# WilliamVenner/squad-mortar-helper

Measured on AMD Instinct MI355X. Metric: map frames/sec (1920x1080 full CV pipeline), whole job, higher is better.
Workload: dtype u8/f32

## Files before the change

include/smh_vision_hip_debug.h:

```cpp
#ifndef SMH_VISION_HIP_DEBUG_H
#define SMH_VISION_HIP_DEBUG_H

#include "smh_vision_hip.h"

#ifdef __cplusplus
extern "C" {
#endif

SMHV_API int smhv_debug_lsd_classic(int on);
SMHV_API int smhv_debug_lsd_tile_cap(uint32_t cap);
SMHV_API int smhv_debug_lsd_threads(uint32_t threads);
SMHV_API int smhv_debug_pattern_copy(smhv_batch *b, const void *d_frames, uint32_t n, uint32_t rows_in_flight, void *stream);
SMHV_API int smhv_debug_heightmap_color_map_device(smhv_heightmap *hm, void *d_rgba, float *ms);
SMHV_API int smhv_debug_skip_line_search(int on);
SMHV_API int smhv_debug_lsd_spin_limit(uint32_t polls);
SMHV_API int smhv_debug_no_host_atomics(int on);
SMHV_API int smhv_debug_side_kernel(smhv_ctx *ctx, uint32_t workgroups, void *stream);

SMHV_API int smhv_debug_pipeline_stats(smhv_pipeline *p, uint64_t out[32]);
SMHV_API int smhv_debug_pipeline_peek(smhv_pipeline *p, uint64_t out[16]);

SMHV_API int smhv_debug_marker_table(smhv_ctx *ctx, uint32_t *bits);

SMHV_API int smhv_debug_crc32_host_level(const void *data, uint64_t nbytes, int level, uint32_t *crc);
SMHV_API int smhv_debug_band_rows(uint32_t frame_w, uint32_t frame_h, uint32_t n, int fused, uint32_t *rows, uint32_t *bands, int *tiles);
SMHV_API int smhv_debug_map_band_rows(uint32_t rows);
SMHV_API int smhv_debug_render_form(uint32_t form);
SMHV_API int smhv_debug_render_rule(uint32_t map_w, uint32_t map_h, float sw, float sh, uint32_t hm_w, uint32_t hm_h, float *ratio, float *switch_ratio,
                                    uint32_t *lds_texels, uint32_t *form);
SMHV_API int smhv_debug_feed_rows(uint32_t rows);
SMHV_API int smhv_debug_feed_gray_form(uint32_t form);
SMHV_API int smhv_debug_batch_mask_state(smhv_batch *b, uint32_t *stale_frames, int *eager);
SMHV_API int smhv_debug_batch_ui_state(smhv_batch *b, uint32_t *stale_frames, int *eager);
SMHV_API int smhv_debug_batch_materialize_ui(smhv_batch *b, void *stream);
SMHV_API int smhv_debug_mask_expand(smhv_batch *b, uint32_t n, void *stream);
SMHV_API int smhv_debug_ingest_feed(smhv_ingest *q, uint32_t n, uint32_t *counter);
SMHV_API int smhv_debug_ingest_feed_pixels(smhv_ingest *q, uint32_t n, uint32_t *counter, uint32_t pixels);

#ifdef __cplusplus
}
#endif

#endif
```

squad-mortar-helper_amd/_lib.py:

```python
import ctypes as C
import os

_HERE = os.path.dirname(os.path.abspath(__file__))
LIB_PATH = os.environ.get("SMH_VISION_HIP_LIB") or os.path.join(_HERE, "libsmh_vision_hip.so")

MAX_LINES = 32
MAX_SCALES = 3

STAGE_MARKERS, STAGE_UI_MAP, STAGE_OCR, STAGE_SCALES, STAGE_ALL = 0x1, 0x2, 0x4, 0x8, 0xF
STAGE_MINIMAP = 0x10
STAGE_EXACT_STATS = 0x20
STAGE_LSD_HELPERS = 0x40
STAGE_FIRING = 0x80
STAGE_HEIGHTMAP_OVERLAY = 0x100
FIRING_BOUNDS_OFFSET = 1
FIRING_NONE, FIRING_SCALES, FIRING_HEIGHTMAP = 0, 1, 2
VIEW_NONE, VIEW_OCR_INPUT, VIEW_FIND_SCALES_INPUT, VIEW_LSD_PREPROCESS, VIEW_LSD_INPUT, VIEW_CROPPED_BRQ = range(6)
IMAGE_UI_MAP = 100
IMAGE_HEIGHTMAP_OVERLAY = 101
RENDER_HEIGHTMAP, RENDER_MARKERS, RENDER_BOUNDS_OFFSET = 1, 2, 4
RENDER_MAX_LINES = 256
PRIM_LINE, PRIM_RECT, PRIM_FOREGROUND, PRIM_SHIFT1 = 0, 1, 0x100, 0x200
RENDER_MAX_PRIMS = 256
LAYER_MINIMAP_BOUNDS = 1
# ... 288 lines not shown
    "smhv_lsd_stats": (C.c_int, [C.c_void_p, C.c_uint32, C.c_int, C.POINTER(C.c_uint32), C.POINTER(C.c_uint64)]),
    "smhv_calc_meters_to_px_ratio": (C.c_int, [C.c_void_p, C.POINTER(C.c_uint32), C.c_uint32, C.POINTER(C.c_double), C.POINTER(C.c_int), C.POINTER(C.c_uint32)]),
    "smhv_find_minimap": (C.c_int, [C.c_void_p, C.POINTER(C.c_uint32), C.POINTER(C.c_int)]),
    "smhv_get_debug_view": (C.c_int, [C.c_void_p, C.c_int, C.c_void_p, C.POINTER(C.c_uint32), C.POINTER(C.c_uint32)]),
    "smhv_batch_create": (C.c_int, [C.c_void_p, C.c_uint32, C.c_uint32, C.c_uint32, C.POINTER(C.c_void_p)]),
    "smhv_batch_destroy": (None, [C.c_void_p]),
    "smhv_batch_layout_get": (C.c_int, [C.c_void_p, C.POINTER(BatchLayout)]),
    "smhv_batch_run": (C.c_int, [C.c_void_p, C.c_void_p, C.c_uint32, C.c_uint32, C.c_int, C.c_uint32, C.c_void_p, C.c_void_p]),
    "smhv_batch_device_ptrs": (C.c_int, [C.c_void_p] + [C.POINTER(C.c_void_p)] * 6),
    "smhv_batch_tile_mask": (C.c_int, [C.c_void_p, C.POINTER(C.c_void_p), C.POINTER(C.c_void_p), C.POINTER(C.c_uint32)]),
    "smhv_batch_read_tile_mask": (C.c_int, [C.c_void_p, C.c_uint32, C.c_void_p, C.c_void_p, C.c_void_p, C.POINTER(C.c_int)]),
    "smhv_batch_read_results": (C.c_int, [C.c_void_p, C.c_uint32, C.c_uint32, C.POINTER(FrameResult)]),
    "smhv_batch_read_image": (C.c_int, [C.c_void_p, C.c_int, C.c_uint32, C.c_void_p]),
    "smhv_batch_set_scales_stream": (C.c_int, [C.c_void_p, C.c_void_p]),
    "smhv_batch_wait_map_pass": (C.c_int, [C.c_void_p, C.c_void_p]),
    "smhv_batch_enable_timing": (C.c_int, [C.c_void_p, C.c_int]),
    "smhv_batch_lsd_coop_stats": (C.c_int, [C.c_void_p, C.c_uint32, C.c_uint32, C.POINTER(C.c_uint32)]),
    "smhv_batch_stage_ms": (C.c_int, [C.c_void_p, C.POINTER(C.c_float)]),
    "smhv_pipeline_create": (C.c_int, [C.c_void_p, C.c_uint32, C.c_uint32, C.c_uint32, C.c_uint32, C.POINTER(C.c_void_p)]),
    "smhv_pipeline_create_ex": (C.c_int, [C.c_void_p, C.c_uint32, C.c_uint32, C.c_uint32, C.c_uint32, C.c_void_p, C.POINTER(C.c_void_p)]),
    "smhv_pipeline_hold": (C.c_int, [C.c_void_p, C.c_uint32, C.c_void_p]),
    "smhv_debug_pipeline_stats": (C.c_int, [C.c_void_p, C.POINTER(C.c_uint64)]),
    "smhv_debug_pipeline_peek": (C.c_int, [C.c_void_p, C.POINTER(C.c_uint64)]),
    "smhv_pipeline_destroy": (None, [C.c_void_p]),
    "smhv_pipeline_submit": (C.c_int, [C.c_void_p, C.c_void_p, C.c_uint32, C.c_uint32, C.c_int, C.c_uint32, C.c_void_p, C.c_void_p, C.POINTER(C.c_uint32)]),
    "smhv_pipeline_wait": (C.c_int, [C.c_void_p, C.c_uint32]),
    "smhv_pipeline_wait_all": (C.c_int, [C.c_void_p]),
    "smhv_pipeline_slot": (C.c_int, [C.c_void_p, C.c_uint32, C.POINTER(C.c_void_p), C.POINTER(C.c_void_p)]),
    "smhv_shard_range": (None, [C.c_uint64, C.c_uint32, C.c_uint32, C.POINTER(C.c_uint64), C.POINTER(C.c_uint64)]),
    "smhv_node_create": (C.c_int, [C.POINTER(C.c_int), C.c_uint32, C.c_uint32, C.c_uint32, C.c_uint32, C.c_uint32, LOG_FN, C.POINTER(C.c_void_p)]),
    "smhv_node_destroy": (None, [C.c_void_p]),
    "smhv_node_ctx": (C.c_int, [C.c_void_p, C.c_uint32, C.POINTER(C.c_void_p), C.POINTER(C.c_void_p)]),
    "smhv_node_run": (C.c_int, [C.c_void_p, C.POINTER(C.c_void_p), C.POINTER(C.c_uint32), C.c_uint32, C.c_int, C.c_uint32, C.POINTER(C.c_void_p)]),
    "smhv_node_gather": (C.c_int, [C.c_void_p, C.POINTER(FrameResult), C.POINTER(C.c_uint32)]),
    "smhv_debug_lsd_classic": (C.c_int, [C.c_int]),
    "smhv_debug_lsd_tile_cap": (C.c_int, [C.c_uint32]),
    "smhv_debug_lsd_spin_limit": (C.c_int, [C.c_uint32]),
    "smhv_debug_lsd_threads": (C.c_int, [C.c_uint32]),
    "smhv_debug_skip_line_search": (C.c_int, [C.c_int]),
    "smhv_debug_no_host_atomics": (C.c_int, [C.c_int]),
    "smhv_debug_side_kernel": (C.c_int, [C.c_void_p, C.c_uint32, C.c_void_p]),
    "smhv_trait_times": (C.c_int, [C.c_void_p, C.POINTER(C.c_uint64), C.POINTER(C.c_uint64), C.c_int]),
    "smhv_ui_map": (C.c_int, [C.c_void_p, C.POINTER(C.c_void_p), C.POINTER(C.c_uint32), C.POINTER(C.c_uint32)]),
    "smhv_debug_pattern_copy": (C.c_int, [C.c_void_p, C.c_void_p, C.c_uint32, C.c_uint32, C.c_void_p]),
    "smhv_debug_batch_mask_state": (C.c_int, [C.c_void_p, C.POINTER(C.c_uint32), C.POINTER(C.c_int)]),
    "smhv_debug_batch_ui_state": (C.c_int, [C.c_void_p, C.POINTER(C.c_uint32), C.POINTER(C.c_int)]),
    "smhv_debug_batch_materialize_ui": (C.c_int, [C.c_void_p, C.c_void_p]),
    "smhv_debug_mask_expand": (C.c_int, [C.c_void_p, C.c_uint32, C.c_void_p]),
    "smhv_debug_marker_table": (C.c_int, [C.c_void_p, C.c_void_p]),
    "smhv_ingest_create": (C.c_int, [C.c_void_p, C.c_uint32, C.c_uint32, C.c_uint32, C.c_uint32, C.POINTER(C.c_void_p)]),
    "smhv_ingest_create_ex": (C.c_int, [C.c_void_p, C.c_uint32, C.c_uint32, C.c_uint32, C.c_uint32, C.c_uint32, C.POINTER(C.c_void_p)]),
    "smhv_crc32_host": (C.c_uint32, [C.c_void_p, C.c_uint64]),
    "smhv_debug_map_band_rows": (C.c_int, [C.c_uint32]),
    "smhv_debug_band_rows": (C.c_int, [C.c_uint32, C.c_uint32, C.c_uint32, C.c_int, C.POINTER(C.c_uint32), C.POINTER(C.c_uint32), C.POINTER(C.c_int)]),
    "smhv_debug_ingest_feed": (C.c_int, [C.c_void_p, C.c_uint32, C.POINTER(C.c_uint32)]),
    "smhv_debug_ingest_feed_pixels": (C.c_int, [C.c_void_p, C.c_uint32, C.POINTER(C.c_uint32), C.c_uint32]),
    "smhv_debug_crc32_host_level": (C.c_int, [C.c_void_p, C.c_uint64, C.c_int, C.POINTER(C.c_uint32)]),
    "smhv_ingest_destroy": (None, [C.c_void_p]),
    "smhv_ingest_local_cpus": (C.c_int, [C.c_void_p, C.c_char_p, C.c_size_t]),
    "smhv_ingest_bind_thread": (C.c_int, [C.c_void_p]),
    "smhv_ingest_acquire": (C.c_int, [C.c_void_p, C.POINTER(C.c_void_p)]),
    "smhv_ingest_commit": (C.c_int, [C.c_void_p]),
    "smhv_ingest_push": (C.c_int, [C.c_void_p, C.c_void_p]),
    "smhv_ingest_commit_pixels": (C.c_int, [C.c_void_p, C.c_uint32]),
    "smhv_ingest_push_pixels": (C.c_int, [C.c_void_p, C.c_void_p, C.c_uint32]),
    "smhv_ingest_staging_bytes": (C.c_uint64, [C.c_uint32, C.c_uint32, C.c_uint32]),
    "smhv_yuv_to_bgra_device": (C.c_int, [C.c_void_p, C.c_void_p, C.POINTER(YuvLayout), C.c_uint32, C.c_uint32, C.c_uint32, C.c_uint32, C.c_void_p, C.c_uint64,
                                          C.c_uint32, C.c_void_p]),
    "smhv_bgra_to_yuv_device": (C.c_int, [C.c_void_p, C.c_void_p, C.c_uint64, C.c_uint64, C.c_uint32, C.c_uint32, C.c_uint32, C.c_uint32, C.c_uint32, C.c_void_p,
                                          C.POINTER(YuvLayout), C.c_void_p]),
    "smhv_batch_video": (C.c_int, [C.c_void_p, C.c_uint32, C.c_uint32, C.c_uint32, C.c_uint32, C.c_void_p, C.POINTER(YuvLayout), C.c_void_p]),
    "smhv_video_bytes": (C.c_uint64, [C.c_uint32, C.c_uint32, C.c_uint32]),
    "smhv_ingest_batch": (C.c_int, [C.c_void_p, C.POINTER(C.c_void_p), C.POINTER(C.c_uint32), C.POINTER(C.c_uint32)]),
    "smhv_ingest_reset": (C.c_int, [C.c_void_p]),
    "smhv_ingest_counts": (C.c_int, [C.c_void_p, C.POINTER(C.c_uint64), C.POINTER(C.c_uint64)]),
    "smhv_crc32_device": (C.c_int, [C.c_void_p, C.c_void_p, C.c_uint64, C.POINTER(C.c_uint32)]),
    "smhv_heightmap_create": (C.c_int, [C.c_void_p, C.c_void_p, C.c_uint32, C.c_uint32, C.POINTER(C.c_int32), C.POINTER(C.c_float), C.POINTER(C.c_void_p)]),
    "smhv_heightmap_destroy": (None, [C.c_void_p]),
    "smhv_heightmap_color_map": (C.c_int, [C.c_void_p, C.c_void_p]),
    "smhv_debug_heightmap_color_map_device": (C.c_int, [C.c_void_p, C.c_void_p, C.POINTER(C.c_float)]),
    "smhv_batch_set_firing": (C.c_int, [C.c_void_p, C.c_void_p, C.POINTER(FiringOptions)]),
    "smhv_pipeline_set_firing": (C.c_int, [C.c_void_p, C.c_void_p, C.POINTER(FiringOptions)]),
    "smhv_batch_read_firing": (C.c_int, [C.c_void_p, C.c_uint32, C.c_uint32, C.POINTER(FiringResult)]),
    "smhv_batch_firing_ptr": (C.c_int, [C.c_void_p, C.POINTER(C.c_void_p)]),
    "smhv_firing_solutions": (C.c_int, [C.c_void_p, C.c_void_p, C.c_uint32, C.POINTER(C.c_double), C.POINTER(C.c_uint32), C.c_void_p,
                                        C.POINTER(FiringOptions), C.POINTER(Firing)]),
    "smhv_batch_overlay_ptr": (C.c_int, [C.c_void_p, C.POINTER(C.c_void_p)]),
    "smhv_heightmap_overlay": (C.c_int, [C.c_void_p, C.c_void_p, C.POINTER(FiringOptions), C.c_void_p]),
    "smhv_map_viewport_calc": (C.c_int, [C.c_float, C.c_float, C.c_float, C.c_float, C.c_uint32, C.POINTER(C.c_float), C.POINTER(C.c_float),
                                         C.POINTER(RenderOptions)]),
    "smhv_batch_render": (C.c_int, [C.c_void_p, C.c_uint32, C.c_uint32, C.c_void_p, C.POINTER(RenderOptions), C.c_void_p]),
    "smhv_batch_render_ptr": (C.c_int, [C.c_void_p, C.POINTER(C.c_void_p), C.POINTER(C.c_uint64)]),
    "smhv_batch_render_size": (C.c_int, [C.c_void_p, C.POINTER(C.c_uint32), C.POINTER(C.c_uint32)]),
    "smhv_batch_read_render": (C.c_int, [C.c_void_p, C.c_uint32, C.c_void_p]),
    "smhv_batch_render_layers": (C.c_int, [C.c_void_p, C.c_uint32, C.c_uint32, C.c_void_p, C.POINTER(RenderOptions), C.POINTER(RenderLayersStruct), C.c_void_p]),
    "smhv_render_map_layers": (C.c_int, [C.c_void_p, C.c_void_p, C.POINTER(RenderOptions), C.POINTER(RenderLayersStruct), C.c_void_p, C.c_uint32, C.c_void_p]),
    "smhv_render_map": (C.c_int, [C.c_void_p, C.c_void_p, C.POINTER(RenderOptions), C.c_void_p, C.c_uint32, C.c_void_p]),
    "smhv_label_font": (C.c_int, [C.c_uint8, C.POINTER(C.c_uint8)]),
    "smhv_batch_render_labels": (C.c_int, [C.c_void_p, C.c_uint32, C.c_uint32, C.c_void_p, C.POINTER(RenderOptions), C.POINTER(LabelOptionsStruct), C.c_void_p]),
    "smhv_batch_read_labels": (C.c_int, [C.c_void_p, C.c_uint32, C.c_uint32, C.POINTER(LabelResult)]),
    "smhv_batch_labels_ptr": (C.c_int, [C.c_void_p, C.POINTER(C.c_void_p)]),
    "smhv_render_map_labeled": (C.c_int, [C.c_void_p, C.c_void_p, C.POINTER(RenderOptions), C.POINTER(RenderLayersStruct), C.c_void_p, C.c_uint32,
                                          C.POINTER(LabelOptionsStruct), C.c_void_p, C.POINTER(LabelResult)]),
    "smhv_text_font": (C.c_int, [C.c_uint8, C.POINTER(C.c_uint8)]),
    "smhv_probe_text": (C.c_int, [C.POINTER(Probe), C.c_char_p, C.c_size_t]),
    "smhv_batch_probe": (C.c_int, [C.c_void_p, C.c_uint32, C.c_uint32, C.POINTER(RenderOptions), C.POINTER(ProbePoint), C.c_uint32, C.c_void_p]),
# ... 62 lines not shown
    "smhv_relief_map": (C.c_int, [C.c_void_p, C.c_void_p, C.POINTER(RenderOptions), C.POINTER(ReliefOptionsStruct), C.POINTER(C.c_uint32), C.c_void_p,
                                  C.c_void_p, C.c_void_p, C.c_void_p, C.POINTER(ReliefResult)]),
    "smhv_batch_scale_labels": (C.c_int, [C.c_void_p, C.c_void_p, C.c_uint32, C.c_void_p]),
    "smhv_batch_read_scale_labels": (C.c_int, [C.c_void_p, C.c_uint32, C.c_uint32, C.POINTER(ScaleLabelFrame), C.c_void_p]),
    "smhv_batch_scale_labels_ptr": (C.c_int, [C.c_void_p, C.POINTER(C.c_void_p), C.POINTER(C.c_void_p)]),
    "smhv_scale_labels": (C.c_int, [C.c_void_p, C.POINTER(ScaleLabelFrame), C.c_void_p]),
    "smhv_glyph_templates_check": (C.c_int, [C.POINTER(GlyphTemplate), C.c_uint32]),
    "smhv_glyph_templates_from_label": (C.c_int, [C.c_void_p, C.POINTER(ScaleLabel), C.c_char_p, C.POINTER(GlyphTemplate), C.POINTER(C.c_uint32)]),
    "smhv_glyph_atlas_create": (C.c_int, [C.c_void_p, C.POINTER(GlyphTemplate), C.c_uint32, C.POINTER(GlyphAtlasOptions), C.POINTER(C.c_void_p)]),
    "smhv_glyph_atlas_destroy": (None, [C.c_void_p]),
    "smhv_batch_label_text": (C.c_int, [C.c_void_p, C.c_void_p, C.c_uint32, C.c_void_p]),
    "smhv_batch_read_label_text": (C.c_int, [C.c_void_p, C.c_uint32, C.c_uint32, C.POINTER(LabelTextFrame)]),
    "smhv_batch_label_text_ptr": (C.c_int, [C.c_void_p, C.POINTER(C.c_void_p), C.POINTER(C.c_void_p)]),
    "smhv_label_text": (C.c_int, [C.c_void_p, C.c_void_p, C.POINTER(LabelTextFrame)]),
    "smhv_batch_run_label_anchors": (C.c_int, [C.c_void_p, C.c_void_p, C.c_uint32, C.c_uint32, C.c_int, C.c_uint32, C.c_void_p]),
    "smhv_scale_labels_anchors": (C.c_int, [C.POINTER(ScaleLabel), C.c_uint32, C.POINTER(C.c_uint32), C.POINTER(Anchors), C.POINTER(C.c_double),
                                            C.POINTER(C.c_int)]),
    "smhv_debug_render_form": (C.c_int, [C.c_uint32]),
    "smhv_debug_render_rule": (C.c_int, [C.c_uint32, C.c_uint32, C.c_float, C.c_float, C.c_uint32, C.c_uint32, C.POINTER(C.c_float), C.POINTER(C.c_float),
                                         C.POINTER(C.c_uint32), C.POINTER(C.c_uint32)]),
}


def firing_options(fit_to_minimap=True, viewport=None):
    o = FiringOptions()
    o.size = C.sizeof(FiringOptions)
    o.flags = 0 if fit_to_minimap else FIRING_BOUNDS_OFFSET
    if viewport is not None:
        sw, sh, tx, ty = viewport
        o.viewport_scale[0], o.viewport_scale[1] = sw, sh
        o.viewport_top_left[0], o.viewport_top_left[1] = tx, ty
    return o


FIRING_DTYPE = None


def firing_dtype():
    import numpy as np
    global FIRING_DTYPE
    if FIRING_DTYPE is None:
        FIRING_DTYPE = np.dtype([("meters", "<f8"), ("alt_delta", "<f8"), ("mils", "<f8", (2,)), ("bearing", "<f4", (2,)),
                                 ("source", "<u4"), ("reserved", "<u4")], align=True)
        assert FIRING_DTYPE.itemsize == C.sizeof(Firing)
    return FIRING_DTYPE


class PipelineOptions(C.Structure):
    _fields_ = [("size", C.c_uint32), ("search", C.c_uint32), ("streams", C.c_uint32), ("idle_close_us", C.c_uint32), ("occupancy_policy", C.c_uint32),
                ("late_helpers", C.c_uint32), ("service_workgroups", C.c_uint32), ("flags", C.c_uint32), ("remote_after", C.c_uint32), ("remote_tickets", C.c_uint32), ("remote_last", C.c_uint32), ("room_for_others", C.c_uint32)]


SEARCH_AUTO, SEARCH_BATCH, SEARCH_FRAME = 0, 1, 2
PIPE_NO_TEAM_HELP, PIPE_NO_STREAM_PRIORITY, PIPE_NO_PROLOGUE, PIPE_NO_REMOTE_HELP, PIPE_HELP_FIRST, PIPE_WALK_BIT_ROWS, PIPE_THREE_LOAD_SETS = 1, 2, 4, 8, 16, 32, 64


class VisionError(RuntimeError):

    def __init__(self, code, msg):
        super().__init__("smh_vision_hip error %d: %s" % (code, msg))
        self.code = code
        self.records = None


_lib = None


def load():
    global _lib
    if _lib is None:
        if not os.path.exists(LIB_PATH):
            raise ImportError(
                "%s not found: the HIP extension is not built (run __graft_entry__.build() or "
                "`make -C squad-mortar-helper_amd/csrc`). There is no CPU fallback." % LIB_PATH)
        try:
            import torch
        except ImportError:
            pass
        lib = C.CDLL(LIB_PATH)
        for name, (res, args) in SIGNATURES.items():
            fn = getattr(lib, name)
            fn.restype = res
            fn.argtypes = args
        _lib = lib
    return _lib


def _hm(heightmap):
    return heightmap._hm if heightmap is not None else None


def check(rc):
    if rc != 0:
        raise VisionError(rc, load().smhv_last_error().decode("utf-8", "replace"))
```

squad-mortar-helper_amd/batch.py:

```python
import ctypes as C
from collections.abc import Mapping

import numpy as np

from . import _lib as L

STAGE_NAMES = ("button", "map_pass", "brq_pass", "lsd", "scale_ratio")


def make_anchors(per_frame):
    arr = (L.Anchors * len(per_frame))()
    for i, (start_y, scales) in enumerate(per_frame):
        arr[i].n = min(len(scales), L.MAX_SCALES)
        arr[i].scales_start_y = start_y
        for j, (m, x, y) in enumerate(scales[:L.MAX_SCALES]):
            arr[i].scales[j][0], arr[i].scales[j][1], arr[i].scales[j][2] = m, x, y
    return arr


def results_to_dicts(recs):
    out = []
    for r in recs:
        n = r.n_lines
        out.append(dict(
# ... 428 lines not shown
        for i in range(depth):
            b = C.c_void_p()
            L.check(self._lib.smhv_pipeline_slot(self._p, i, C.byref(b), None))
            self.slots.append(FrameBatch(vision, frame_w, frame_h, max_frames, _handle=b))

    def stream_of(self, slot):
        st = C.c_void_p()
        L.check(self._lib.smhv_pipeline_slot(self._p, slot, None, C.byref(st)))
        return st.value or 0

    def hold(self, slot, stream):
        L.check(self._lib.smhv_pipeline_hold(self._p, slot, C.c_void_p(stream)))

    def submit(self, frames_ptr, n, stages=L.STAGE_ALL, grayscale=True, max_gap=15, anchors=None, after_stream=0):
        if anchors is not None and len(anchors) < n:
            raise ValueError("anchors holds %d entries, the submission covers %d frames" % (len(anchors), n))
        a = C.cast(anchors, C.c_void_p) if anchors is not None else None
        slot = C.c_uint32(0)
        L.check(self._lib.smhv_pipeline_submit(self._p, C.c_void_p(frames_ptr), n, stages, int(bool(grayscale)), max_gap, a, C.c_void_p(after_stream), C.byref(slot)))
        return int(slot.value)

    def set_firing(self, heightmap=None, fit_to_minimap=True, viewport=None):
        opt = L.firing_options(fit_to_minimap, viewport)
        L.check(self._lib.smhv_pipeline_set_firing(self._p, L._hm(heightmap), C.byref(opt)))

    def search_stats(self):
        out = (C.c_uint64 * 32)()
        L.check(self._lib.smhv_debug_pipeline_stats(self._p, out))
        if not out[0]:
            return None
        keys = ("launches", "frames", "waves", "busy_cycles", "resident_cycles", "waves_per_launch", "submissions")
        d = dict(zip(keys, [int(v) for v in out[1:8]]))
        d["cycles_per_frame_by_phase"] = dict(zip(("acquire", "search", "record", "release"), [int(v) / max(d["frames"], 1) for v in out[8:12]]))
        d["help_cycles_per_frame"] = int(out[12]) / max(d["frames"], 1)
        d["remote_help"] = {"requests": int(out[16]), "helpers_attached": int(out[17]), "candidates_cast": int(out[18]), "tickets_left": int(out[19]) - (1 << 64) if int(out[19]) >= (1 << 63) else int(out[19])}
        d["cycles_per_frame"] = d["busy_cycles"] / max(d["frames"], 1)
        d["busy_fraction"] = d["busy_cycles"] / max(d["resident_cycles"], 1)
        d["remote_help"].update({"polls": int(out[23]), "polls_empty": int(out[24]), "claims_lost": int(out[25]), "exits_idle": int(out[26]), "exits_closed": int(out[27]),
                                 "cycles_attached_per_helper": int(out[28]) / max(int(out[17]), 1), "cast_fraction_of_attached": int(out[29]) / max(int(out[28]), 1)})
        d["timeline_ms"] = {"frame_wait": int(out[20]) / max(d["frames"], 1) / 1e5, "submission_search": int(out[21]) / max(d["submissions"], 1) / 1e5,
                            "last_frame_at_work": int(out[22]) / max(d["submissions"], 1) / 1e5}
        d["adaptive"] = bool(int(out[13]) & 2)
        d["settled"] = bool(int(out[13]) & 4) or not d["adaptive"]
        d["mode"] = "frame-granular" if int(out[13]) & 1 else "batch-granular"
        d["measured_frames_per_s"] = {"frame-granular": int(out[14]), "batch-granular": int(out[15])}
        return d

    def peek(self):
        out = (C.c_uint64 * 16)()
        L.check(self._lib.smhv_debug_pipeline_peek(self._p, out))
        keys = ("submissions", "alive_epoch", "launches", "last_seq", "avail", "head", "reserved", "closing_epoch", "completed", "busy")
        d = dict(zip(keys, [int(v) for v in out[:10]]))
        d["avail"] = d["avail"] - (1 << 64) if d["avail"] >= (1 << 63) else d["avail"]
        d["slots"] = [(int(v) >> 32, int(v) & 0xFFFFFFFF) for v in out[10:14]]
        d["service_workgroups"], d["waves_per_workgroup"] = int(out[14]) >> 32, int(out[14]) & 0xFFFFFFFF
        d["lds_words_per_wave"], d["lds_bytes_dynamic"] = int(out[15]) >> 32, int(out[15]) & 0xFFFFFFFF
        return d

    def wait(self, slot=None):
        if slot is None:
            L.check(self._lib.smhv_pipeline_wait_all(self._p))
        else:
            L.check(self._lib.smhv_pipeline_wait(self._p, slot))

    def close(self):
        if self._p:
            for b in self.slots:
                b.close()
            self._lib.smhv_pipeline_destroy(self._p)
            self._p = None

    def __del__(self):
        try:
            self.close()
        except Exception:
            pass
```

squad-mortar-helper_amd/csrc/smh_kernels.h:

```cpp
#pragma once
#include <hip/hip_runtime.h>
#include <stdint.h>

#include "../../include/smh_vision_hip.h"
#include "../../include/smh_vision_hip_debug.h"

namespace smh {

struct Geom {
	uint32_t W, H;
	uint32_t rx, ry, rw, rh;
	uint32_t bx, by, bw, bh;
	uint32_t qx, qy, qw, qh;
	uint32_t m_ax, m_xoff, m_quads, m_block;
	uint32_t q_ax, q_xoff, q_quads, q_block;
	uint64_t frame_bytes;
	uint64_t ui_pitch, ui_stride;
	uint64_t mask_pitch, mask_stride;
	uint32_t bits_pitch_w; uint64_t bits_stride_w;
	uint64_t ocr_pitch, ocr_stride;
};

struct FrameAux {
	uint32_t open;
// ... 332 lines not shown
	uint32_t closing;
	int32_t help_avail;
	uint32_t help_head, help_reserve;
	uint32_t stat_remote;
	uint32_t head;
	uint32_t reserve;
	uint32_t completed;
	uint32_t busy;
	uint32_t stat_items, stat_waves;
	unsigned long long stat_busy, stat_life;
	unsigned long long stat_phase[4];
	unsigned long long stat_help;
	uint32_t stat_requests, stat_attached;
	unsigned long long stat_t_wait, stat_t_sub, stat_t_last;
	uint32_t stat_h_polls, stat_h_empty, stat_h_lost, stat_h_idle_exit, stat_h_closed_exit, stat_h_pad;
	unsigned long long stat_h_cycles, stat_h_cast_cycles;
	unsigned long long help_ring[SVC_HELP_RING];
};
struct SvcHost {
	unsigned long long state;
	uint32_t launches;
	uint32_t pad0;
	uint32_t done_seq[SVC_MAX_SLOTS];
	uint32_t pad[12];
};
struct SvcParams {
	SvcCtl *ctl;
	unsigned long long *ring;
	SvcSlot *slots;
	SvcHost *host;
	const uint32_t *cull_tab;
	const float *ray_off;
	float max_gap;
	uint32_t tile_cap, list_cap;
	uint32_t part_words;
	uint32_t ring_log2;
	uint32_t epoch;
	uint32_t idle_short, idle_long;
	uint32_t flags;
	SvcRemote *remote;
	uint32_t *remote_store;
	uint32_t remote_store_words;
	uint32_t remote_after;
	uint32_t remote_tickets;
	uint32_t remote_last_div;
	uint32_t compact;
};
uint32_t svc_waves_for(const Geom &g, uint32_t tile_limit, uint32_t *part_words, uint32_t *tile_cap, uint32_t *list_cap, uint32_t *lds_bytes, uint32_t *compact = nullptr);
uint32_t svc_store_words_for(const Geom &g, uint32_t tile_cap, uint32_t compact);
hipError_t svc_probe_host_atomics(SvcHost *h, SvcHost *d_h, bool *ok);
hipError_t launch_svc_publish(SvcCtl *ctl, unsigned long long *ring, SvcSlot *slots, uint32_t slot, const Buffers &b, uint32_t n, uint32_t seq, uint32_t ring_log2, hipStream_t s);
hipError_t launch_lsd_service(const Geom &g, const SvcParams &p, uint32_t workgroups, uint32_t waves, uint32_t lds_bytes, hipStream_t s);

enum : uint32_t { MAP_UI = 1u, MAP_MASK = 2u, MAP_BYTES = 4u, MAP_PRIO = 0x100u, MAP_BAND_MAJOR = 0x200u };
enum : uint32_t { BRQ_OCR = 1u, BRQ_SCALES = 2u };

enum : uint32_t { UI_FORM_RGBA = 0u, UI_FORM_LUMA = 1u, UI_FORM_KEEP = 2u };
hipError_t launch_button(const Geom &g, const Buffers &b, uint32_t n, int force_open, hipStream_t s, uint8_t *ui_form = nullptr, uint32_t ui_luma = UI_FORM_KEEP);
hipError_t launch_ui_expand(const Geom &g, const uint8_t *d_luma, uint8_t *d_ui, uint8_t *ui_form, uint32_t n, hipStream_t s);
hipError_t launch_map_pass(const Geom &g, const Buffers &b, uint32_t n, uint32_t flags, int grayscale, hipStream_t s, bool tiles_wanted = false, bool overlapped = false);
struct LaunchTuning {
	uint32_t map_lds_total;
	uint32_t map_grid_cap;
	uint32_t lsd_tile_limit;
	uint32_t map_prio;
	uint32_t map_deep;
	uint32_t map_overlapped;
};
uint32_t map_brq_lds_bytes(const Geom &g);
uint32_t lsd_tile_lds_bytes(const Geom &g, uint32_t tile_limit);
hipError_t launch_map_brq_pass(const Geom &g, const Buffers &b, uint32_t n, uint32_t flags, uint32_t qflags, int grayscale, uint32_t fixed_start_y, int use_anchor_start, hipStream_t s,
                               const LaunchTuning *tune = nullptr);
hipError_t launch_pattern_copy(const Geom &g, const Buffers &b, uint32_t n, uint32_t rows_in_flight, hipStream_t s);
void map_band_rows(uint32_t rh, uint32_t n, int fused, uint32_t *rows, int *tiles);
hipError_t launch_brq_pass(const Geom &g, const Buffers &b, uint32_t n, uint32_t flags, uint32_t fixed_start_y, int use_anchor_start, hipStream_t s);
struct LsdFork { hipStream_t s1, s2; hipEvent_t fork, join1, join2; };
bool lsd_rows_only(const Geom &g);
hipError_t launch_lsd(const Geom &g, const Buffers &b, uint32_t n, float max_gap, int mode, float px, float py, hipStream_t s, const LsdFork *fk, uint32_t tile_bs = 0,
                      bool prefer_classic = false, uint32_t tile_limit = 0, bool *record_fused = nullptr);
size_t lsd_coop_ctl_bytes(uint32_t n);
hipError_t launch_scale_ratio(const Geom &g, const Buffers &b, uint32_t n, uint32_t *d_bars, hipStream_t s);
hipError_t launch_find_minimap(const Geom &g, const Buffers &b, uint32_t n, hipStream_t s);
hipError_t launch_finalize(const Geom &g, const Buffers &b, uint32_t n, uint32_t stages, hipStream_t s);
hipError_t launch_scales_finalize(const Geom &g, const Buffers &b, uint32_t n, uint32_t stages, uint32_t *d_bars, hipStream_t s);
hipError_t launch_firing_lines(const FiringRun &r, const smhv_line *lines, uint32_t n, uint32_t has_mpx, double mpx, uint32_t has_minimap,
                               const uint32_t minimap[4], smhv_firing *out, hipStream_t s);
hipError_t launch_heightmap_color_map(const uint16_t *hm, uint64_t n, uint32_t *mm, uint32_t *rgba, hipStream_t s);
#define SMH_HM_LUT_ENTRIES 65536u
hipError_t launch_heightmap_lut(const uint16_t *hm, uint64_t n, uint32_t *mm, uint32_t *lut, hipStream_t s);
hipError_t launch_hm_overlay(const Geom &g, const OverlayRun &r, uint32_t n, hipStream_t s);
hipError_t launch_render_map(const Geom &g, const RenderRun &r, uint32_t n, hipStream_t s);
hipError_t launch_render_map_layers(const Geom &g, const RenderRun &r, const RenderLayersRun &y, uint32_t n, hipStream_t s);
hipError_t launch_heightmap_lut16(const uint32_t *lut, uint16_t *lut16, uint32_t *vr, hipStream_t s);
#define SMH_HM_LUT_WORDS (SMH_HM_LUT_ENTRIES + 4u + SMH_HM_LUT_ENTRIES / 2u)
hipError_t launch_labels(const LabelRun &r, uint32_t n, hipStream_t s);
hipError_t launch_reach(const ReachRun &r, uint32_t n, bool paint, bool classes, hipStream_t s);
hipError_t launch_relief(const ReliefRun &r, uint32_t n, bool paint, hipStream_t s);
hipError_t launch_clear_lines(const ClearLinesRun &r, uint32_t n, hipStream_t s);
hipError_t launch_clear_map(const ClearMapRun &r, uint32_t n, bool paint, bool bytes, hipStream_t s);
hipError_t launch_scale_labels(const ScaleLabelsRun &r, uint32_t n, hipStream_t s);
uint32_t scale_labels_gap(uint32_t qw);
hipError_t launch_label_text(const LabelTextRun &r, uint32_t n, hipStream_t s);
hipError_t launch_debug_text(const Geom &g, const DebugRun &r, uint32_t n, hipStream_t s);
void render_set_form(uint32_t form);
uint32_t render_rule(const Geom &g, const RenderRun &r, uint32_t *texels, float *ratio);
float render_switch_ratio();
hipError_t launch_debug_view(const Geom &g, const Buffers &b, uint32_t frame, int which, int isolated, uint8_t *d_rgba, hipStream_t s);
hipError_t launch_marker_table(uint32_t *d_bits, hipStream_t s);
hipError_t launch_mask_expand(const Geom &g, const uint32_t *d_bits, uint8_t *d_mask, uint32_t n, hipStream_t s);
hipError_t launch_pack_rows(const void *d_src, uint32_t src_pitch_bytes, void *d_dst, uint32_t row_bytes, uint32_t rows, hipStream_t s);
hipError_t launch_side_probe(uint32_t *d_out, uint32_t workgroups, uint32_t spin, hipStream_t s);
hipError_t launch_build_sector_table(unsigned long long *d_tab, uint32_t T, hipStream_t s);
hipError_t launch_build_ray_offsets(float *d_off, hipStream_t s);
size_t lsd_lds_bytes();
void lsd_set_classic(bool on);
void lsd_set_tile_cap(uint32_t cap);
void lsd_set_threads(uint32_t threads);
void lsd_set_spin_limit(uint32_t polls);
hipError_t set_ray_table(const float *dx, const float *dy);
#define SMH_CRC_BS 1024
// ... 86 lines not shown
```

squad-mortar-helper_amd/csrc/smh_lsd_seq.inc:

```

template <int MODE>
__device__ __forceinline__ uint32_t seq_build_list(const Win &m, WShared &ws, uint32_t *list, uint32_t *survw, uint32_t list_cap, uint32_t wy0, uint32_t wrows, uint32_t wwords, uint32_t wi_min,
                                                   uint32_t WT, uint32_t *wi_next) {
	const uint32_t lane = threadIdx.x & 63u;
	uint32_t o = 0, next = WT;
	auto append = [&](uint32_t w, uint32_t wi) {
		const unsigned long long nz = __ballot(w != 0u);
		if (!nz) return;
		const uint32_t pos = o + (uint32_t)__popcll(nz & ((1ull << lane) - 1ull));
		if (w != 0u && pos < list_cap) { list[pos] = wi; survw[pos] = w; ws.stag[pos] = 0; }
		const uint32_t cnt = (uint32_t)__popcll(nz);
		if (o + cnt > list_cap) {
			unsigned long long rest = nz;
			for (uint32_t k = o; k < list_cap; ++k) rest &= rest - 1ull;
			next = (uint32_t)__builtin_amdgcn_readlane((int)wi, (int)__builtin_ctzll(rest));
			o = list_cap;
		} else o += cnt;
	};
	if constexpr (MODE == LSD_MODE_TILE || MODE == LSD_MODE_TILEC) {
		auto tile_at = [&](uint32_t ty, uint32_t c) -> uint32_t {
			if constexpr (MODE == LSD_MODE_TILEC) return tilec_number(m, (int)c, (int)ty);
			else return (uint32_t)m.t_idx[__mul24((int)ty, (int)m.t_pitch) + (int)c];
		};
		const bool two = wwords <= 32u;
// ... 150 lines not shown
		const rem_u32x4 z = {0u, 0u, 0u, 0u};
		g_st64(&r->ring[lane].post, 0ull); g_st64(&r->ring[lane].claim, 0ull); g_st128(r->ring[lane].res_a, z); g_st128(r->ring[lane].res_b, z);
	}
	if (lane == 0) g_st64(&r->info, (unsigned long long)ntiles);
	asm volatile("s_waitcnt vmcnt(0)" ::: "memory");
	__builtin_amdgcn_fence(__ATOMIC_RELEASE, "agent");
	asm volatile("s_waitcnt vmcnt(0)" ::: "memory");
	uint32_t gen = st_hi + 1u;
	if ((gen & 0xFFFFu) == 0u) ++gen;
	if (lane == 0) {
		g_st64(&r->state, ((unsigned long long)gen << 32) | SVC_REMOTE_OPEN);
		__hip_atomic_fetch_add(&ctl->stat_requests, 1u, __ATOMIC_RELAXED, __HIP_MEMORY_SCOPE_AGENT);
		ws.rem_open = 1u; ws.rem_gen = gen; ws.rem_k = 0u; ws.rem_nr = 0u;
	}
	wave_lds_sync();
	(void)remote_issue_tickets(ws, ctl, gen, tickets);
	return true;
}

__device__ __forceinline__ void tile_win(Win &m, uint32_t rw, uint32_t rh, uint32_t *smem, uint32_t tile_cap) {
	const uint32_t TWP = tile_idx_pitch(rw);
	m.w = rw; m.h = rh; m.wf = (float)rw; m.hf = (float)rh;
	m.p = smem; m.pitch4 = 0u; m.y_lo = 0; m.xbias = 0; m.rows_hi = 0u; m.cols_hi = 0u;
	m.rows0 = nullptr; m.ylo_f = 0.0f; m.yhi_f = 0.0f;
	m.c_p = (const LdsWord *)smem; m.c_y0 = 0u; m.c_rows = 0u; m.c_pitch4 = 0u;
	m.t_idx = (const LdsU16 *)(smem + (tile_cap + 1u) * 8u) + TWP + 2u; m.t_tiles = (const LdsWord *)smem; m.t_pitch = TWP; m.tiled = true;
	m.tc_rows = nullptr; m.tc_groups = 0u; m.compact = false;
	m.w2 = nullptr;
}

__device__ __forceinline__ void tilec_win(Win &m, uint32_t rw, uint32_t rh, uint32_t *smem, uint32_t tile_cap) {
	tile_win(m, rw, rh, smem, tile_cap);
	const uint32_t G = tilec_groups(rw);
	m.t_idx = nullptr;
	m.tc_rows = (const LdsWord *)(smem + (tile_cap + 1u) * 8u + G * 4u); m.tc_groups = G; m.compact = true;
}

#ifndef SVC_WIN_EXTRA
#define SVC_WIN_EXTRA 24u
#endif
#ifdef SMH_NO_WINDOW_REUSE
#define SVC_WIN_REUSE(compact) false
#else
#define SVC_WIN_REUSE(compact) (!(compact))
#endif
#define SVC_WIN_ROWS(compact) (SVC_WIN_REUSE(compact) ? W_WIN_ROWS + SVC_WIN_EXTRA : W_WIN_ROWS)
#define SVC_WIN_STRIDE(compact) (SVC_WIN_ROWS(compact) * LSD_W2_PITCH + 2u)
#ifdef SMH_NO_LEAN_SAMPLER
#define SVC_LEAN_SAMPLER(compact) false
#else
#define SVC_LEAN_SAMPLER(compact) (!(compact))
#endif

template <int MODE, bool REUSE = false, bool LEAN = false>
__device__ __forceinline__ void seq_cast_candidate(const Win &m, uint32_t *wwin, WinTag *tag, const uint32_t *cull_tab, uint32_t cull, const RayDir *dirs, const float *ray_off, float max_gap,
                                                   uint32_t px, uint32_t py, float &xs, float &ys, unsigned long long &wkey, float &ex0, float &ey0, uint32_t &steps_sum
#ifdef SMH_LSD_WDEBUG
                                                   , unsigned long long *sprof, unsigned long long &slast, unsigned long long *uprof, uint32_t &n_units
#endif
                                                   ) {
	const uint32_t lane = opaque_lane();
	unsigned long long live;
#ifdef SMH_LSD_WDEBUG
	cand_setup<MODE == LSD_MODE_TILEC, (REUSE ? W_WIN_ROWS + SVC_WIN_EXTRA : W_WIN_ROWS), REUSE>(m, wwin, cull_tab, cull, px, py, xs, ys, live, tag, uprof);
	{ const unsigned long long _n = __builtin_amdgcn_s_memtime(); sprof[2] += _n - slast; slast = _n; }
#else
	cand_setup<MODE == LSD_MODE_TILEC, (REUSE ? W_WIN_ROWS + SVC_WIN_EXTRA : W_WIN_ROWS), REUSE>(m, wwin, cull_tab, cull, px, py, xs, ys, live, tag);
#endif
	unsigned long long bkey = 0ull;
	float bxe = xs, bye = ys;
	uint32_t st = 0;
	auto unit_dirs_lds = [&](uint32_t u) -> RayDir { return dirs[min(u * 64u + lane, (uint32_t)SMH_LSD_RAYS - 1u)]; };
	RayDir dn = unit_dirs_lds(live ? (uint32_t)__builtin_ctzll(live) : 0u);
	for (unsigned long long todo = live; todo; todo &= todo - 1ull) {
		const uint32_t u = (uint32_t)__builtin_ctzll(todo);
		const RayDir d = dn;
		const unsigned long long rest = todo & (todo - 1ull);
		if (rest) dn = unit_dirs_lds((uint32_t)__builtin_ctzll(rest));
		unsigned long long key;
		float xe, ye;
#ifdef SMH_LSD_WDEBUG
		unit_rays<MODE, (MODE == LSD_MODE_TILEC ? SEQ_RAY_GROUP_C : SEQ_RAY_GROUP), REUSE, LEAN>(m, wwin, ray_off, px, py, xs, ys, u, d, max_gap, key, xe, ye, st, uprof, tag);
		++n_units;
#else
		unit_rays<MODE, (MODE == LSD_MODE_TILEC ? SEQ_RAY_GROUP_C : SEQ_RAY_GROUP), REUSE, LEAN>(m, wwin, ray_off, px, py, xs, ys, u, d, max_gap, key, xe, ye, st, tag);
#endif
		if (key > bkey) { bkey = key; bxe = xe; bye = ye; }
	}
	steps_sum = wave_sum32_dpp(st);
	wkey = 0ull; ex0 = xs; ey0 = ys;
	if (__any(bkey != 0ull)) {
		const uint32_t hi = (uint32_t)(bkey >> 32), lo = (uint32_t)bkey;
		const uint32_t mhi = wave_max32_dpp(hi);
		const uint32_t mlo = wave_max32_dpp(hi == mhi ? lo : 0u);
		wkey = ((unsigned long long)mhi << 32) | mlo;
		if (wkey != 0ull) {
			const uint32_t src = (uint32_t)__builtin_ctzll(__ballot(bkey == wkey));
			ex0 = bcast_f(bxe, src); ey0 = bcast_f(bye, src);
		}
	}
#ifdef SMH_LSD_WDEBUG
	{ const unsigned long long _n = __builtin_amdgcn_s_memtime(); sprof[3] += _n - slast; slast = _n; }
#endif
}

__device__ __forceinline__ bool desk_take(WShared &ws, uint32_t px, uint32_t py, float &xs, float &ys, unsigned long long &wkey, float &ex0, float &ey0, uint32_t &steps_sum) {
	const uint32_t lane = opaque_lane();
	bool match = false;
	if (lane < SEQ_DESK_ENTRIES) {
		const uint32_t st = W_LD_ACQ(&ws.rob[lane].state);
		match = st != (uint32_t)H_FREE && st != (uint32_t)H_RZOMBIE && ws.rob[lane].px == px && ws.rob[lane].py == py;
	}
	const unsigned long long hit = __ballot(match);
	if (!hit) return false;
	const uint32_t e = (uint32_t)__builtin_ctzll(hit);
	WSlot &sl = ws.rob[e];
	if (e >= SEQ_HELP_SLOTS) {
		if (uniform_u32(sl.state) == (uint32_t)H_RPOSTED) remote_harvest(ws);
		WDBG(0, 1u);
		if (uniform_u32(sl.state) == (uint32_t)H_RPOSTED) {
			const uint32_t k = uniform_u32(sl.lines_seen);
			uint32_t old = 0;
			if (lane == 0) old = (uint32_t)__hip_atomic_fetch_max(&rem_of(ws)->ring[e - SEQ_HELP_SLOTS].claim, (unsigned long long)k, __ATOMIC_RELAXED, __HIP_MEMORY_SCOPE_AGENT);
			if (uniform_u32(old) < k) {
				if (lane == 0) sl.state = H_FREE;
				wave_lds_sync();
				WDBG(1, 1u);
				return false;
			}
			WDBG(2, 1u);
#ifdef SMH_LSD_WDEBUG
			const unsigned long long t_w = __builtin_amdgcn_s_memtime();
#endif
			while (uniform_u32(sl.state) != (uint32_t)H_DONE) { __builtin_amdgcn_s_sleep(16); remote_harvest(ws); }
#ifdef SMH_LSD_WDEBUG
			if (lane == 0) ws.prof[0] += __builtin_amdgcn_s_memtime() - t_w;
#endif
		}
		xs = sl.ptx; ys = sl.pty; wkey = sl.best; ex0 = sl.ex; ey0 = sl.ey; steps_sum = sl.steps;
		__builtin_amdgcn_wave_barrier();
		if (lane == 0) sl.state = H_FREE;
		wave_lds_sync();
		return true;
	}
	if (uniform_u32(W_LD_ACQ(&sl.state)) == (uint32_t)H_POSTED) {
		uint32_t ok = 0;
		if (lane == 0) { uint32_t expect = H_POSTED; ok = __hip_atomic_compare_exchange_strong(&sl.state, &expect, (uint32_t)H_FREE, __ATOMIC_ACQ_REL, __ATOMIC_RELAXED, __HIP_MEMORY_SCOPE_WORKGROUP) ? 1u : 0u; }
		if (uniform_u32(ok)) return false;
	}
	while (uniform_u32(W_LD_ACQ(&sl.state)) != (uint32_t)H_DONE) __builtin_amdgcn_s_sleep(2);
	xs = sl.ptx; ys = sl.pty; wkey = sl.best; ex0 = sl.ex; ey0 = sl.ey; steps_sum = sl.steps;
	__builtin_amdgcn_wave_barrier();
	if (lane == 0) W_ST_REL(&sl.state, (uint32_t)H_FREE);
	return true;
}

__device__ __forceinline__ uint32_t disp_entry(WShared &ws, const uint32_t *list, uint32_t *survw, uint32_t e, uint32_t first, uint32_t end, uint32_t n_lines, uint32_t wy0, uint32_t wwords,
                                               int xorg, float &fpx0, float &fpy) {
	uint32_t w = 0;
	fpx0 = 0.0f; fpy = 0.0f;
	if (e < end && e >= first) {
		w = survw[e];
		const uint32_t wi = list[e], r = wi / wwords, c = wi - r * wwords;
		fpy = (float)(wy0 + r); fpx0 = (float)(xorg + (int)(c * 32u));
		const uint32_t tag = ws.stag[e];
		if (w && tag < n_lines) {
			for (uint32_t l = tag; l < n_lines && w; ++l) {
				ProxLine L;
				L.x0 = ws.lines[l][0]; L.y0 = ws.lines[l][1]; L.x1 = ws.lines[l][2]; L.y1 = ws.lines[l][3];
				L.a = ws.prox_a[l]; L.dxl = ws.prox_d[l][0]; L.dyl = ws.prox_d[l][1];
				L.degenerate = L.dxl == 0.0 && L.dyl == 0.0;
				w = prox_filter_word(w, fpx0, fpy, L);
			}
			survw[e] = w;
			ws.stag[e] = (unsigned char)n_lines;
		}
	}
	return w;
}

__device__ __forceinline__ void desk_post_remote(WShared &ws, uint32_t slot, uint32_t qx, uint32_t qy, uint32_t &st, uint32_t &spx, uint32_t &spy) {
	const uint32_t k = uniform_u32(ws.rem_k) + 1u;
	if (opaque_lane() == slot) {
		ws.rob[slot].px = qx; ws.rob[slot].py = qy; ws.rob[slot].lines_seen = k; ws.rob[slot].state = H_RPOSTED;
		ws.rem_k = k;
		g_st64(&rem_of(ws)->ring[slot - SEQ_HELP_SLOTS].post, ((unsigned long long)k << 32) | ((qy & 0xFFFFu) << 16) | (qx & 0xFFFFu));
		st = H_RPOSTED; spx = qx; spy = qy;
	}
	RDBG(0, 1ull);
	wave_lds_sync();
}
__device__ __forceinline__ void desk_refresh(WShared &ws, const uint32_t *list, uint32_t *survw, uint32_t wy0, uint32_t wwords, int xorg, uint32_t cap_local, uint32_t cap_remote, uint32_t &post_seq,
                                             uint32_t &cur_e, int &cur_bit, uint32_t &ahead) {
	const uint32_t lane = opaque_lane();
	const uint32_t n_lines = W_LD(&ws.n_lines), end = ws.disp_end, first = W_LD(&ws.disp_e);
	const uint32_t want = 1u + cap_local + cap_remote;
	cur_e = end; cur_bit = -1;
	uint32_t mpx = 0xFFFFFFFFu, mpy = 0xFFFFFFFFu, np = 0;
	for (uint32_t e0 = first & ~63u; e0 < end && np < want; e0 += 64u) {
		float fpx0, fpy;
		const uint32_t w = disp_entry(ws, list, survw, e0 + lane, first, end, n_lines, wy0, wwords, xorg, fpx0, fpy);
		unsigned long long any = __ballot(w != 0u);
		while (any && np < want) {
// ... 89 lines not shown
		const uint32_t ww = (uint32_t)__builtin_amdgcn_readlane((int)w, (int)src);
		const uint32_t bit = (uint32_t)__builtin_ctz(ww);
		const uint32_t ppx = (uint32_t)((int)bcast_f(fpx0, src) + (int)bit), ppy = (uint32_t)bcast_f(fpy, src);
		cur_e = e0 + src; cur_bit = (int)bit;
		if (ahead++ == 0u) continue;
		if (room_l) {
			const uint32_t slot = (uint32_t)__builtin_ctzll(free_l);
			free_l &= free_l - 1ull;
			if (lane == slot) {
				ws.rob[slot].px = ppx; ws.rob[slot].py = ppy; ws.rob[slot].lines_seen = post_seq;
				W_ST_REL(&ws.rob[slot].state, (uint32_t)H_POSTED);
			}
			++post_seq; ++busy_l;
		} else {
			uint32_t d0 = 0, d1 = 0, d2 = 0;
			desk_post_remote(ws, (uint32_t)__builtin_ctzll(free_r), ppx, ppy, d0, d1, d2);
			free_r &= free_r - 1ull;
			++busy_r;
		}
		room_l = busy_l < cap_local && free_l; room_r = busy_r < cap_remote && free_r;
	}
}

template <int MODE, bool WAVE = false, bool TEAM = false, bool REUSE = false, bool LEAN = false>
__device__ void lsd_frame_seq(const Geom &g, const Buffers &b, uint32_t f, float max_gap, const FrameAux &aux, uint32_t *smem, WShared &ws, const uint32_t *cull_tab, const RayDir *dirs,
                              uint32_t win_cap, uint32_t list_cap, const FrameView *tile_view = nullptr) {
	static_assert(!TEAM || (WAVE && (MODE == LSD_MODE_TILE || MODE == LSD_MODE_TILEC)), "helpers read the owner's tile store in LDS");
	const uint32_t lane = threadIdx.x & 63u;
	FrameView v;
	if constexpr (MODE == LSD_MODE_TILE || MODE == LSD_MODE_TILEC) v = *tile_view;
	else frame_setup<MODE, WAVE>(g, b, f, aux, smem, v);
	const Win &m = v.m;
	uint32_t *list = smem + win_cap, *survw = list + list_cap, *wwin = survw + list_cap;
	const uint32_t wy0 = v.wy0, wrows = v.wrows, wwords = v.wwords;
	const int xorg = v.xorg;
	const uint32_t WT = wrows * wwords;
	const uint32_t cull = cull_mode_for(b.cull_tab, max_gap);
	if (lane == 0) { ws.n_lines = 0u; ws.rounds = 0u; ws.steps = 0ull; }
	if (TEAM && lane < SEQ_DESK_ENTRIES) ws.rob[lane].state = H_FREE;
	if (TEAM && lane == 0) { ws.rem_open = 0u; ws.rem_nr = 0u; if (REUSE) ws.frame_no += 1u; }
#ifdef SMH_LSD_WDEBUG
	if (lane < 8u) ws.dbg[lane] = 0u;
	if (lane < 10u) ws.rdbg[lane] = 0ull;
	if (lane == 0) ws.prof[0] = 0ull;
#endif
	const bool remote_ok = TEAM && ws.rem_r != 0ull;
	bool rem_open = false;
	uint32_t rem_nr = 0, rem_asked = 0;
	uint32_t rounds = 0, n_lines = 0, post_seq = 0;
	uint32_t seg_start = 0, cur_e = 0, ahead = 0;
	int cur_bit = -1;
	bool done = false, want = false, desk_valid = false;
	WinTag wtag = {0, 0, false};
#ifdef SMH_LSD_WDEBUG
	unsigned long long sprof[8] = {0, 0, 0, 0, 0, 0, 0, 0}, slast = __builtin_amdgcn_s_memtime(), uprof[12] = {0, 0, 0, 0, 0, 0, 0, 0, 0, 0, 0, 0};
	uint32_t n_units = 0, n_taken = 0;
#define SPROF(i) do { const unsigned long long _n = __builtin_amdgcn_s_memtime(); sprof[i] += _n - slast; slast = _n; } while (0)
#else
#define SPROF(i)
#endif
	while (!done) {
		uint32_t segnext;
		const uint32_t n_list = seq_build_list<MODE>(m, ws, list, survw, list_cap, wy0, wrows, wwords, seg_start, WT, &segnext);
		if (lane == 0) { ws.disp_e = 0u; ws.disp_end = n_list; }
		desk_valid = false;
		__builtin_amdgcn_fence(__ATOMIC_RELEASE, "workgroup");
		__builtin_amdgcn_wave_barrier();
		__builtin_amdgcn_fence(__ATOMIC_ACQUIRE, "workgroup");
		SPROF(0);
		while (true) {
			uint32_t px = 0, py = 0;
			if (!wave_dispatch(ws, list, survw, wy0, wwords, xorg, px, py)) break;
			__builtin_amdgcn_fence(__ATOMIC_RELEASE, "workgroup");
			__builtin_amdgcn_wave_barrier();
			SPROF(1);
			float xs = 0.0f, ys = 0.0f, ex0 = 0.0f, ey0 = 0.0f;
			unsigned long long wkey = 0ull;
			uint32_t st_sum = 0u;
			++rounds;
			if (ahead) --ahead;
			bool have = false;
#ifdef SMH_LSD_WDEBUG
			const unsigned long long t_tk = __builtin_amdgcn_s_memtime();
#endif
			if (TEAM && want) have = desk_take(ws, px, py, xs, ys, wkey, ex0, ey0, st_sum);
#ifdef SMH_LSD_WDEBUG
			if (rem_open) RDBG(7, __builtin_amdgcn_s_memtime() - t_tk);
#endif
#ifdef SMH_LSD_WDEBUG
			if (have) ++n_taken;
			if (!have) seq_cast_candidate<MODE, REUSE, LEAN>(m, wwin, &wtag, cull_tab, cull, dirs, b.ray_off, max_gap, px, py, xs, ys, wkey, ex0, ey0, st_sum, sprof, slast, uprof, n_units);
#else
			if (!have) seq_cast_candidate<MODE, REUSE, LEAN>(m, wwin, &wtag, cull_tab, cull, dirs, b.ray_off, max_gap, px, py, xs, ys, wkey, ex0, ey0, st_sum);
#endif
			if (lane == 0) ws.steps += st_sum;
			if (wkey != 0ull && __uint_as_float((uint32_t)(wkey >> 32)) > SMH_LSD_ACCEPT_LEN_SQ) {
				float ex, ey;
				get_centre(m, ex0, ey0, ex, ey);
				if (lane == 0) {
					ws.lines[n_lines][0] = xs; ws.lines[n_lines][1] = ys; ws.lines[n_lines][2] = ex; ws.lines[n_lines][3] = ey;
					const ProxLine pl = prox_line(xs, ys, ex, ey);
					ws.prox_a[n_lines] = pl.a; ws.prox_d[n_lines][0] = pl.dxl; ws.prox_d[n_lines][1] = pl.dyl;
					W_ST_REL(&ws.n_lines, n_lines + 1u);
				}
				++n_lines;
				desk_valid = false;
				__builtin_amdgcn_fence(__ATOMIC_RELEASE, "workgroup");
				__builtin_amdgcn_wave_barrier();
				__builtin_amdgcn_fence(__ATOMIC_ACQUIRE, "workgroup");
				if (n_lines == SMH_LSD_MAX_LINES) { done = true; break; }
			}
			if (TEAM) {
				if (!want && rounds >= SEQ_HELP_AFTER) {
					want = true;
					if (lane == 0) W_ST_REL(&ws.want_set, 1u);
				}
				if (want) {
					if (remote_ok && (rounds & (rem_open ? 7u : 1u)) == 0u) {
						if (rem_open) {
							rem_nr = remote_helpers(ws);
							const uint32_t want_h = uniform_u32(ws.rem_tickets);
							if (rem_nr * 2u < want_h && rounds - rem_asked >= 8u) {
								if ((ws.rem_flags & 1u) || (int32_t)uniform_u32((uint32_t)__hip_atomic_load(&rem_ctl_of(ws)->avail, __ATOMIC_RELAXED, __HIP_MEMORY_SCOPE_AGENT)) <= 0)
									(void)remote_issue_tickets(ws, rem_ctl_of(ws), uniform_u32(ws.rem_gen), want_h - rem_nr);
								rem_asked = rounds;
							}
						}
						else if (rounds >= uniform_u32(ws.rem_after) && ws.disp_end - min(W_LD(&ws.disp_e), ws.disp_end) >= SEQ_REMOTE_MIN_LEFT) {
							const uint32_t *dp = (const uint32_t *)(uintptr_t)(((unsigned long long)uniform_u32((uint32_t)(ws.rem_done >> 32)) << 32) | uniform_u32((uint32_t)ws.rem_done));
							const uint32_t n_sub = uniform_u32(ws.rem_n), fin = uniform_u32(__hip_atomic_load(dp, __ATOMIC_RELAXED, __HIP_MEMORY_SCOPE_AGENT));
							const bool free_waves = (ws.rem_flags & 1u) || (int32_t)uniform_u32((uint32_t)__hip_atomic_load(&rem_ctl_of(ws)->avail, __ATOMIC_RELAXED, __HIP_MEMORY_SCOPE_AGENT)) <= 0;
							if (free_waves && (n_sub - min(fin, n_sub)) * uniform_u32(ws.rem_last_div) <= n_sub) rem_asked = rounds;
#ifdef SMH_LSD_WDEBUG
							if (rem_asked == rounds && lane == 0) { ws.dbg[3] += 1u; if (ws.dbg[4] == 0u) ws.dbg[4] = rounds; }
#endif
							if (rem_asked == rounds)
								rem_open = remote_open<MODE == LSD_MODE_TILEC>((uint32_t)(uintptr_t)(const LdsByte *)&ws, (uint32_t)(uintptr_t)(const LdsByte *)smem, MODE == LSD_MODE_TILEC ? tilec_idx_words(g.rw, g.rh) : tile_idx_words(g.rw, g.rh));
						}
					}
					const uint32_t nh = uniform_u32(W_LD(&ws.late));
					const uint32_t cap_l = min(nh, SEQ_HELP_SLOTS - 1u), cap_r = rem_open ? min(2u + 2u * rem_nr, SVC_REMOTE_RING) : 0u;
					if (!cap_l && !cap_r) desk_valid = false;
					else if (!desk_valid) {
#ifdef SMH_LSD_WDEBUG
						const unsigned long long t_r = __builtin_amdgcn_s_memtime();
#endif
						desk_refresh(ws, list, survw, wy0, wwords, xorg, cap_l, cap_r, post_seq, cur_e, cur_bit, ahead);
						desk_valid = true;
#ifdef SMH_LSD_WDEBUG
						if (rem_open) { RDBG(3, 1ull); RDBG(5, __builtin_amdgcn_s_memtime() - t_r); }
#endif
					} else {
#ifdef SMH_LSD_WDEBUG
						const unsigned long long t_r = __builtin_amdgcn_s_memtime();
#endif
						desk_post_more(ws, list, survw, wy0, wwords, xorg, cap_l, cap_r, post_seq, cur_e, cur_bit, ahead);
#ifdef SMH_LSD_WDEBUG
						if (rem_open) RDBG(6, __builtin_amdgcn_s_memtime() - t_r);
#endif
					}
#ifdef SMH_LSD_WDEBUG
					if (rem_open) { RDBG(8, 1ull); if (lane == 0 && ws.rdbg[9] == 0ull) ws.rdbg[9] = __builtin_amdgcn_s_memtime(); }
#endif
				}
			}
			SPROF(4);
		}
		if (segnext >= WT) break;
		seg_start = segnext;
	}
	if (TEAM) {
		if (lane == 0) W_ST_REL(&ws.want_set, 0u);
		if (rem_open) remote_close(ws);
		while (uniform_u32(W_LD_ACQ(&ws.late)) != 0u) __builtin_amdgcn_s_sleep(2);
	}
	smhv_frame_result *res = &b.results[f];
	if (lane < n_lines) {
		res->lines[lane].x0 = ws.lines[lane][0]; res->lines[lane].y0 = ws.lines[lane][1];
		res->lines[lane].x1 = ws.lines[lane][2]; res->lines[lane].y1 = ws.lines[lane][3];
	}
	if (lane == 0) { res->n_lines = n_lines; res->rounds = rounds; res->ray_steps = ws.steps; res->status = SMHV_FRAME_OK; }
#ifdef SMH_LSD_WDEBUG
	if (lane == 0) {
		for (int k = 0; k < 5; ++k) res->meters[20 + k] = (double)sprof[k];
		for (int k = 0; k < 3; ++k) res->meters[25 + k] = (double)uprof[8 + k];
		res->meters[30] = (double)uprof[0]; res->meters[31] = (double)uprof[1];
		res->length_px[28] = (double)uprof[2];
		res->meters[28] = (double)n_units;
		res->meters[29] = (double)n_taken;
		res->length_px[22] = (double)ws.dbg[0]; res->length_px[23] = (double)ws.dbg[1]; res->length_px[24] = (double)ws.dbg[2]; res->length_px[25] = (double)ws.prof[0];
		res->length_px[26] = (double)ws.dbg[3]; res->length_px[27] = (double)ws.dbg[4];
		for (int k = 0; k < 9; ++k) res->angle[16 + k] = (float)ws.rdbg[k];
		res->angle[25] = ws.rdbg[9] ? (float)(__builtin_amdgcn_s_memtime() - ws.rdbg[9]) : 0.0f;
	}
#endif
}
```

squad-mortar-helper_amd/csrc/smh_map_pass.inc:

```
	const uint32_t f = blockIdx.y;
	if (!b.aux[f].open) return;
	const uint32_t q = threadIdx.x, lane = q & 63u, wave = q >> 6, nwave = blockDim.x >> 6;
	const int r0 = (int)(blockIdx.x * RB);
	const int r1 = min(r0 + (int)RB, (int)g.rh);
	const bool qact = q < g.m_quads;
	uint32_t vmask = 0;
#pragma unroll
	for (int c = 0; c < 4; ++c)
		if ((uint32_t)(4 * q + c - g.m_xoff) < g.rw) vmask |= 1u << c;
	if (!qact) vmask = 0;

	const uint8_t *fp = b.frames + (size_t)f * g.frame_bytes + ((size_t)g.ry * g.W + g.m_ax + 4 * q) * 4;
	uint8_t *uip = GRAYF == 2 ? b.ui + (size_t)f * (g.ui_stride >> 2) + (size_t)q * 4 : b.ui + (size_t)f * g.ui_stride + (size_t)q * 16;
	const size_t row_bytes = (size_t)g.W * 4;

	uint64_t P[4] = {0, 0, 0, 0};
	const int rs = max(r0 - 1, 0), re = min(r1, (int)g.rh - 1);
	const bool do_ui = (flags & MAP_UI) != 0, do_mask = (flags & MAP_MASK) != 0;

	const uint8_t *lp = qact ? fp : fp - (size_t)q * 16;
	uint4 nx[4];
#pragma unroll
	for (int k = 0; k < 4; ++k) nx[k] = *(const uint4 *)(lp + (size_t)min(rs + k, re) * row_bytes);
	extern __shared__ __attribute__((aligned(16))) uint32_t s_hits[];
	for (int r = rs; r <= re; r += 4) {
		uint4 px[4];
		uint32_t prehits = 0;
#pragma unroll
		for (int k = 0; k < 4; ++k) px[k] = nx[k];
		if (r + 4 <= re) {
#pragma unroll
			for (int k = 0; k < 4; ++k) nx[k] = *(const uint4 *)(lp + (size_t)min(r + 4 + k, re) * row_bytes);
		}
#pragma unroll
		for (int k = 0; k < 4; ++k) {
			const int row = r + k;
			if (row > re) break;
			const uint32_t pv[4] = {px[k].x, px[k].y, px[k].z, px[k].w};
			if (do_ui && row >= r0 && row < r1 && qact) {
				uint32_t ov[4];
#pragma unroll
				for (int c = 0; c < 4; ++c) {
					const uint32_t p = pv[c], bb = p & 255u, gg = (p >> 8) & 255u, rr8 = (p >> 16) & 255u;
					if (GRAYF == 2) ov[c] = luma8(rr8, gg, bb);
					else if (GRAYF) ov[c] = luma8(rr8, gg, bb) * 0x00010101u | 0xFF000000u;
					else ov[c] = rr8 | (gg << 8) | (bb << 16) | 0xFF000000u;
				}
				if constexpr (GRAYF == 2) *(uint32_t *)(uip + (size_t)row * (g.ui_pitch >> 2)) = ov[0] | (ov[1] << 8) | (ov[2] << 16) | (ov[3] << 24);
				else {
					uint4 o;
					o.x = ov[0]; o.y = ov[1]; o.z = ov[2]; o.w = ov[3];
					*(uint4 *)(uip + (size_t)row * g.ui_pitch) = o;
				}
			}
			if (do_mask) {
				uint32_t pre = 0;
#pragma unroll
				for (int c = 0; c < 4; ++c) pre |= marker_prefilter(pv[c]) ? (1u << c) : 0u;
				prehits |= (pre & vmask) << (4 * k);
			}
		}
		if (do_mask && __any(prehits != 0u)) {
			uint32_t *hpx = s_hits + wave * 160u;
			uint32_t *hres = hpx + 64;
			unsigned short *hid = (unsigned short *)(hres + 64);
			const uint32_t cnt = (uint32_t)__popc(prehits);
			uint32_t incl = cnt;
			for (int o = 1; o < 64; o <<= 1) { const uint32_t t = __shfl_up(incl, o); if (lane >= (uint32_t)o) incl += t; }
			const uint32_t total = __shfl(incl, 63);
			const uint32_t off = incl - cnt;
			hres[lane] = 0u;
			for (uint32_t base = 0; base < total; base += 64u) {
				uint32_t o = off - base;
#pragma unroll
				for (int k = 0; k < 4; ++k) {
					const uint32_t pk[4] = {px[k].x, px[k].y, px[k].z, px[k].w};
#pragma unroll
					for (int c = 0; c < 4; ++c)
						if ((prehits >> (4 * k + c)) & 1u) {
							if (o < 64u) { hpx[o] = pk[c]; hid[o] = (unsigned short)((lane << 4) | (uint32_t)(4 * k + c)); }
							++o;
						}
				}
				__builtin_amdgcn_wave_barrier();
				const uint32_t e = base + lane;
				if (e < total) {
					const uint32_t p = hpx[lane];
					if (marker_exact((p >> 16) & 255u, (p >> 8) & 255u, p & 255u)) {
						const uint32_t id = hid[lane];
						atomicOr(&hres[id >> 4], 1u << (id & 15u));
					}
				}
				__builtin_amdgcn_wave_barrier();
			}
			const uint32_t res = hres[lane];
			if (res) {
				const int sh = r - (r0 - 1);
#pragma unroll
				for (int c = 0; c < 4; ++c) {
					uint32_t y = (res >> c) & 0x1111u;
					y = (y | (y >> 3) | (y >> 6) | (y >> 9)) & 0xFu;
					P[c] |= (uint64_t)y << sh;
				}
			}
		}
	}
	if (!do_mask) return;

	__shared__ uint64_t s_edge_first[16], s_edge_last[16];
	if (lane == 0) s_edge_first[wave] = P[0];
	if (lane == 63) s_edge_last[wave] = P[3];
	__syncthreads();
	uint64_t left = __shfl_up(P[3], 1), right = __shfl_down(P[0], 1);
	if (lane == 0) left = wave > 0 ? s_edge_last[wave - 1] : 0ull;
	if (lane == 63) right = wave + 1 < nwave ? s_edge_first[wave + 1] : 0ull;
	const int nrows = r1 - r0;
	const uint64_t rowmask = ((nrows >= 63 ? ~0ull : ((1ull << nrows) - 1ull)) << 1);
	uint64_t D[4];
#define SMH_VERT(p) ((p) | ((p) << 1) | ((p) >> 1))
	D[0] = SMH_VERT(P[0]) | left | P[1];
	D[1] = SMH_VERT(P[1]) | P[0] | P[2];
	D[2] = SMH_VERT(P[2]) | P[1] | P[3];
	D[3] = SMH_VERT(P[3]) | P[2] | right;
#undef SMH_VERT
#pragma unroll
	for (int c = 0; c < 4; ++c) D[c] = ((vmask >> c) & 1u) ? (D[c] & rowmask) : 0ull;

	const bool do_bytes = (flags & MAP_BYTES) != 0;
	const uint32_t quads_padded = (g.m_quads + 15u) & ~15u;
	const uint64_t any = D[0] | D[1] | D[2] | D[3];
	const uint64_t lanes_set = __ballot(any != 0ull);
	uint32_t occ7 = 0;
	if constexpr (TILES) {
		const uint32_t ntr = ((uint32_t)nrows + 7u) >> 3, op = occ_pitch(g);
		uint8_t *occp = b.occ + (size_t)f * occ_stride(g) + (size_t)((uint32_t)r0 >> 3) * op + wave;
		if (lanes_set) occ7 = tile_occupancy(any >> 1, lane, ntr, occp, op);
		else if (lane < ntr) occp[(size_t)lane * op] = 0;
		if (blockIdx.x == 0 && q == 0) b.aux[f].tiles = 1u;
	}
	if (q < quads_padded) {
		uint8_t *mp = b.mask + (size_t)f * g.mask_stride + (size_t)q * 4;
		uint32_t *bp = b.bits + (size_t)f * g.bits_stride_w + (q >> 3);
		uint32_t *tp = nullptr;
		if constexpr (TILES) tp = b.tiled + (size_t)f * tiled_stride_w(g) + ((size_t)((uint32_t)r0 >> 3) * g.bits_pitch_w + (q >> 3)) * 8u;
		for (int row = r0; row < r1; ++row) {
			const int bit = row - r0 + 1;
			const uint32_t nib = (uint32_t)((D[0] >> bit) & 1ull) | ((uint32_t)((D[1] >> bit) & 1ull) << 1) |
			                     ((uint32_t)((D[2] >> bit) & 1ull) << 2) | ((uint32_t)((D[3] >> bit) & 1ull) << 3);
			if (do_bytes) *(uint32_t *)(mp + (size_t)row * g.mask_pitch) = ((nib * 0x00204081u) & 0x01010101u) * 0xFFu;
			uint32_t v = nib;
			v |= __shfl_down(v, 1) << 4;
			v |= __shfl_down(v, 2) << 8;
			v |= __shfl_down(v, 4) << 16;
			if ((lane & 7u) == 0) bp[(size_t)row * g.bits_pitch_w] = v;
			if constexpr (TILES) {
				const uint32_t i = (uint32_t)(row - r0);
				if ((occ7 >> (i >> 3)) & 1u) tp[(size_t)(i >> 3) * g.bits_pitch_w * 8u + (i & 7u)] = v;
			}
		}
	}
	if (lanes_set) {
		const uint64_t rows_set = wave_or64(any);
		const uint32_t cnt = wave_sum32(__popcll(D[0]) + __popcll(D[1]) + __popcll(D[2]) + __popcll(D[3]));
		if (lane == 0) {
			FrameAux *a = &b.aux[f];
			atomicMin(&a->y_min, (uint32_t)(r0 - 1 + __builtin_ctzll(rows_set)));
			atomicMax(&a->y_max, (uint32_t)(r0 - 1 + 63 - __builtin_clzll(rows_set)));
			atomicMin(&a->w_min, (wave * 64u + (uint32_t)__builtin_ctzll(lanes_set)) >> 3);
			atomicMax(&a->w_max, (wave * 64u + 63u - (uint32_t)__builtin_clzll(lanes_set)) >> 3);
			atomicAdd(&a->n_mask_px, cnt);
		}
	}
```

squad-mortar-helper_amd/csrc/smh_runtime.cpp:

```cpp
#include <hip/hip_runtime.h>

#include <atomic>
#include <condition_variable>
#include <deque>
#include <thread>
#include <cmath>
#include <cstdarg>
#include <cstdio>
#include <cstdlib>
#include <cstring>
#include <ctime>
#include <initializer_list>
#include <sched.h>
#include <pthread.h>
#include <cctype>
#include <mutex>
#include <vector>
#include <new>
#include <string>

#include "smh_consts.h"
#include "smh_kernels.h"
#include "smh_glyph_rule.h"
#include "smh_grid.h"
// ... 995 lines not shown
		if (rc) return rc;
	}
	const bool scales = (stages & SMHV_STAGE_SCALES) && (anchors || d_anchors_src);
	const hipStream_t sb = (svc && svc->s_pro) ? svc->s_pro : s;
	if (scales && d_anchors_src) HIPCHK(hipMemcpyAsync(b->d_anchors, d_anchors_src, sizeof(smhv_anchors) * n, hipMemcpyDeviceToDevice, sb));
	else if (scales) {
		smhv_batch::AnchorStage *st = nullptr;
		for (auto &a : b->anchor_stage)
			if (hipEventQuery(a.done) == hipSuccess) { st = &a; break; }
		if (!st) {
			smhv_batch::AnchorStage a;
			hipError_t e = hipHostMalloc((void **)&a.h, sizeof(smhv_anchors) * b->max_frames);
			if (e == hipSuccess) e = hipEventCreateWithFlags(&a.done, hipEventDisableTiming);
			if (e != hipSuccess) { if (a.h) (void)hipHostFree(a.h); return fail(SMHV_E_HIP, "anchor staging: %s", hipGetErrorString(e)); }
			b->anchor_stage.push_back(a);
			st = &b->anchor_stage.back();
		}
		memcpy(st->h, anchors, sizeof(smhv_anchors) * n);
		HIPCHK(hipMemcpyAsync(b->d_anchors, st->h, sizeof(smhv_anchors) * n, hipMemcpyHostToDevice, sb));
		HIPCHK(hipEventRecord(st->done, sb));
	}
	if (stages & SMHV_STAGE_FIRING) {
		int rc = firing_upload(b, sb);
		if (rc) return rc;
		bf.firing = b->d_fire_run;
	}
	const bool t = b->timing;
	hipEvent_t *ev = t ? b->ev[b->timed_runs % smhv_batch::TIMING_RING] : nullptr;
#define STAGE_BEGIN(i, st) do { if (t) HIPCHK(hipEventRecord(ev[2 * (i)], (st))); } while (0)
#define STAGE_END(i, st) do { if (t) HIPCHK(hipEventRecord(ev[2 * (i) + 1], (st))); } while (0)
	const bool ui_stage = (stages & SMHV_STAGE_UI_MAP) != 0u;
	bool ui_lazy = false;
	if (ui_stage) {
		std::lock_guard<std::mutex> lk(b->ui_mu);
		ui_lazy = grayscale && !(stages & SMHV_STAGE_HEIGHTMAP_OVERLAY) && !b->ui_eager;
		if (ui_lazy) { b->ui_stale = std::max(b->ui_stale, n); bf.ui = b->d_ui_luma; }
	}
	const int pass_gray = ui_lazy ? 2 : (grayscale ? 1 : 0);
	STAGE_BEGIN(0, sb);
	HIPCHK(launch_button(g, bf, n, 0, sb, b->d_ui_form, ui_stage ? (ui_lazy ? UI_FORM_LUMA : UI_FORM_RGBA) : UI_FORM_KEEP));
	STAGE_END(0, sb);
	if (sb != s) {
		HIPCHK(hipEventRecord(svc->ev_pro, sb));
		HIPCHK(hipStreamWaitEvent(s, svc->ev_pro, 0));
	}
	uint32_t mflags = 0, qflags = 0;
	if (stages & SMHV_STAGE_MARKERS) mflags |= MAP_MASK;
	if (stages & SMHV_STAGE_UI_MAP) mflags |= MAP_UI;
	if (stages & SMHV_STAGE_OCR) qflags |= BRQ_OCR;
	if (scales) qflags |= BRQ_SCALES;
	if (b->probe) HIPCHK(hipEventRecord(b->ev_probe[0], s));
	STAGE_BEGIN(1, s);
	if (mflags && qflags) HIPCHK(launch_map_brq_pass(g, bf, n, mflags, qflags, pass_gray, 0, 1, s, &b->tune));
	else if (mflags) HIPCHK(launch_map_pass(g, bf, n, mflags, pass_gray, s, true, b->tune.map_overlapped != 0u));
	if (mflags & MAP_MASK) {
		std::lock_guard<std::mutex> lk(b->mask_mu);
		if (b->mask_eager) HIPCHK(launch_mask_expand(g, b->d_bits, b->d_mask, n, s));
		else b->mask_stale = std::max(b->mask_stale, n);
	}
	STAGE_END(1, s);
	if (mflags & MAP_UI) { b->ui_written = true; b->ui_gray = grayscale != 0; }
	if (mflags & MAP_MASK) b->mask_written = true;
	if (qflags & BRQ_OCR) b->ocr_written = true;
	if (qflags & BRQ_SCALES) b->scales_written = true;
	b->run_stages = stages; b->run_n = n;
	STAGE_BEGIN(2, s);
	if (qflags && !mflags) HIPCHK(launch_brq_pass(g, bf, n, qflags, 0, 1, s));
	STAGE_END(2, s);
	if (!svc) HIPCHK(hipEventRecord(b->ev_map_done, s));
	if (b->probe) HIPCHK(hipEventRecord(b->ev_probe[1], s));
	if (sl != s) HIPCHK(hipStreamWaitEvent(sl, b->ev_map_done, 0));
	const bool skip_lsd = g_skip_lsd.load(std::memory_order_relaxed);
	if (svc) {
		if (stages & SMHV_STAGE_MINIMAP) HIPCHK(launch_find_minimap(g, bf, n, s));
		if (stages & SMHV_STAGE_HEIGHTMAP_OVERLAY) HIPCHK(launch_hm_overlay(g, orun, n, s));
		bf.rec_stages = SMH_REC_ON | (scales ? stages : (stages & ~SMHV_STAGE_SCALES));
		bf.rec_bars = b->d_bars;
		STAGE_BEGIN(3, s);
		HIPCHK(launch_svc_publish(svc->ctl, svc->ring, svc->slots, svc->slot, bf, n, svc->seq, svc->ring_log2, s));
		if (svc->published) *svc->published = true;
		STAGE_END(3, s);
		STAGE_BEGIN(4, s);
		STAGE_END(4, s);
		if (t) b->timed_runs++;
		return SMHV_OK;
	}
	STAGE_BEGIN(3, sl);
	const uint32_t late_kc = b->lsd_late_kc;
	if (late_kc > 0u) { bf.lsd_flags |= SMH_LSD_LATE_HELP; bf.lsd_late_kc = late_kc; }
	bool record_fused = false;
	if (!(stages & SMHV_STAGE_MINIMAP)) {
		bf.rec_stages = SMH_REC_ON | (scales ? stages : (stages & ~SMHV_STAGE_SCALES));
		bf.rec_bars = b->d_bars;
	}
	if ((stages & SMHV_STAGE_MARKERS) && !skip_lsd) HIPCHK(launch_lsd(g, bf, n, (float)max_gap, 0, 0.0f, 0.0f, sl, b->lsd_fork.s1 ? &b->lsd_fork : nullptr, b->lsd_bs, b->lsd_prefer_classic,
	                                                      (mflags && qflags) ? b->tune.lsd_tile_limit : 0u,
	                                                      &record_fused));
	STAGE_END(3, sl);
	if (b->probe) { HIPCHK(hipEventRecord(b->ev_probe[2], sl)); b->probe_valid = (stages & SMHV_STAGE_MARKERS) && mflags; }
	if (stages & SMHV_STAGE_MINIMAP) HIPCHK(launch_find_minimap(g, bf, n, sl));
	if (stages & SMHV_STAGE_HEIGHTMAP_OVERLAY) HIPCHK(launch_hm_overlay(g, orun, n, sl));
	STAGE_BEGIN(4, sl);
	if (record_fused) {  }
	else if (scales) HIPCHK(launch_scales_finalize(g, bf, n, stages, b->d_bars, sl));
	else HIPCHK(launch_finalize(g, bf, n, stages & ~SMHV_STAGE_SCALES, sl));
	STAGE_END(4, sl);
#undef STAGE_BEGIN
// ... 139 lines not shown
	const Geom &g = b->g;
	HIPCHK(hipSetDevice(b->ctx->device));
	HIPCHK(hipDeviceSynchronize());
	if (which == SMHV_IMAGE_HEIGHTMAP_OVERLAY && !b->d_overlay) return fail(SMHV_E_STATE, "batch_read_image: no run of this batch had SMHV_STAGE_HEIGHTMAP_OVERLAY");
	switch (which) {
	case 100:
	case SMHV_IMAGE_HEIGHTMAP_OVERLAY:
		{
			int rc = batch_materialize_ui(b, b->ctx->s_main);
			if (rc) return rc;
			HIPCHK(wait_stream(b->ctx->s_main));
		}
		HIPCHK(hipMemcpy2D(out, (size_t)g.rw * 4, (which == 100 ? b->d_ui : b->d_overlay) + frame * g.ui_stride + (size_t)g.m_xoff * 4, g.ui_pitch, (size_t)g.rw * 4,
		                   g.rh, hipMemcpyDeviceToHost));
		break;
	case SMHV_VIEW_LSD_INPUT: {
		std::lock_guard<std::mutex> lk(b->ctx->mu);
		int rc = batch_materialize_mask(b, b->ctx->s_main);
		if (rc) return rc;
		return copy_image_d2h(b->ctx, 2, out, b->d_mask + frame * g.mask_stride, g.mask_pitch, g.m_xoff, g.rw, g.rh, b->ctx->s_main);
	}
	case SMHV_VIEW_OCR_INPUT: {
		std::lock_guard<std::mutex> lk(b->ctx->mu);
		return copy_image_d2h(b->ctx, 2, out, b->d_ocr + frame * g.ocr_stride, g.ocr_pitch, g.q_xoff, g.qw, g.qh, b->ctx->s_main);
	}
	case SMHV_VIEW_FIND_SCALES_INPUT: {
		std::lock_guard<std::mutex> lk(b->ctx->mu);
		return copy_image_d2h(b->ctx, 2, out, b->d_scales + frame * g.ocr_stride, g.ocr_pitch, g.q_xoff, g.qw, g.qh, b->ctx->s_main);
	}
	default:
		return fail(SMHV_E_INVALID, "unsupported image id %d", which);
	}
	return SMHV_OK;
}

static std::atomic<int> g_own_queues[64];
struct smhv_pipeline {
	smhv_ctx *ctx = nullptr;
	uint32_t depth = 0;
	smhv_pipeline_options opt{};
	std::vector<smhv_batch *> batch;
	std::vector<hipStream_t> stream;
	std::vector<hipEvent_t> done;
	std::vector<hipEvent_t> hold;
	std::vector<char> held;
	std::vector<hipStream_t> last_sl;
	hipEvent_t ev_after = nullptr;
	LaunchTuning tuning{0u, 0u, 0u, 0u};
	bool adapt = false, tune_on = true;
	float ratio_ema = 0.0f;
	uint64_t submitted = 0;
	uint64_t round_start = 0;
	bool svc = false;
	uint32_t svc_compact = 0;
	uint32_t svc_streams = 0, svc_waves = 0, svc_part_words = 0, svc_tile_cap = 0, svc_list_cap = 0, svc_lds = 0, svc_wgs = 0, svc_ring_log2 = 0;
	SvcCtl *d_svc_ctl = nullptr;
	unsigned long long *d_svc_ring = nullptr;
	SvcSlot *d_svc_slots = nullptr;
	SvcHost *h_svc = nullptr, *d_svc_host = nullptr;
	SvcRemote *d_svc_remote = nullptr;
	uint32_t *d_svc_store = nullptr;
	uint32_t svc_store_words = 0;
	hipStream_t s_search = nullptr, s_pro = nullptr;
	std::mutex peek_mu;
	hipStream_t s_peek = nullptr;
	SvcCtl *h_peek = nullptr;
	smhv_heightmap *fire_hm = nullptr;
	smhv_firing_options fire_opt{};
	std::vector<hipEvent_t> ev_pub;
	std::vector<hipEvent_t> ev_pro;
	std::vector<uint32_t> seq;
	std::vector<hipStream_t> slot_st;
	uint32_t seq_counter = 0, svc_epoch = 0;
	bool svc_key_valid = false;
	const uint32_t *svc_cull = nullptr;
	uint32_t svc_max_gap = 0;
	std::vector<hipStream_t> svc_stream;
	std::vector<uint8_t> slot_frame;
	bool adaptive = false, mode_frame = false;
	uint32_t own_queues = 0;
	struct ModeCtl {
		uint32_t phase = 0, count = 0, settle = 0, key_n = 0, key_stages = 0, key_gap = 0, decisions = 0;
		uint32_t cand_n = 0, cand_stages = 0, cand_gap = 0, cand_count = 0;
		uint32_t remeasured = 0;
		bool window_mixed = false;
		uint64_t frames = 0;
		struct timespec t0{};
		double rate[2] = {0.0, 0.0};
	} mc;
};
static int svc_wait_slot(smhv_pipeline *p, uint32_t slot);
static int slot_wait(smhv_pipeline *p, uint32_t slot) {
	if (p->svc && p->slot_frame[slot]) return svc_wait_slot(p, slot);
	HIPCHK(wait_event(p->done[slot]));
	return SMHV_OK;
}
static int svc_launch(smhv_pipeline *p, uint32_t slot);
static int svc_submit(smhv_pipeline *p, uint32_t slot, const void *d_frames, uint32_t n, uint32_t stages, int grayscale, uint32_t max_gap,
                      const smhv_anchors *anchors, void *after_stream, uint32_t *slot_out);

extern "C" SMHV_API void smhv_pipeline_destroy(smhv_pipeline *p) {
	if (!p) return;
	if (p->ctx) (void)hipSetDevice(p->ctx->device);
	if (p->svc) for (uint32_t i = 0; i < p->depth && i < p->slot_frame.size(); ++i) if (p->slot_frame[i]) (void)svc_wait_slot(p, i);
	(void)hipDeviceSynchronize();
	for (auto b : p->batch) if (b) smhv_batch_destroy(b);
	for (auto e : p->done) if (e) (void)hipEventDestroy(e);
	for (auto e : p->hold) if (e) (void)hipEventDestroy(e);
	if (p->ev_after) (void)hipEventDestroy(p->ev_after);
	for (auto st : p->stream) if (st) (void)hipStreamDestroy(st);
	for (auto st : p->svc_stream) if (st) (void)hipStreamDestroy(st);
	if (p->ctx) g_own_queues[(uint32_t)p->ctx->device & 63u].fetch_sub((int)p->own_queues, std::memory_order_relaxed);
	if (p->s_search) (void)hipStreamDestroy(p->s_search);
	if (p->s_pro) (void)hipStreamDestroy(p->s_pro);
	if (p->s_peek) (void)hipStreamDestroy(p->s_peek);
	if (p->h_peek) (void)hipHostFree(p->h_peek);
	for (auto e : p->ev_pub) if (e) (void)hipEventDestroy(e);
	for (auto e : p->ev_pro) if (e) (void)hipEventDestroy(e);
	if (p->d_svc_ctl) (void)hipFree(p->d_svc_ctl);
	if (p->d_svc_ring) (void)hipFree(p->d_svc_ring);
	if (p->d_svc_slots) (void)hipFree(p->d_svc_slots);
	if (p->d_svc_remote) (void)hipFree(p->d_svc_remote);
	if (p->d_svc_store) (void)hipFree(p->d_svc_store);
	if (p->h_svc) (void)hipHostFree(p->h_svc);
	hm_release(p->fire_hm);
	ctx_release(p->ctx);
	delete p;
}

#define SMH_PIPE_TILE_LIMIT(g) ((g).rh > 900u ? 320u : 200u)
#define SMH_SVC_TILE_LIMIT(g) ((g).rh > 900u ? 272u : 200u)
#define SMH_PIPE_MAP_GRID 1024u
#define SMH_LDS_PER_CU 163840u
#define SMH_ADAPT_OFF 3.5f
#define SMH_ADAPT_ON 1.6f
#define SMH_LATE_KC_SEARCH_BOUND 400u
static LaunchTuning pipeline_tuning(const Geom &g) {
	LaunchTuning t{0u, 0u, 0u, 0u, 0u};
	const uint32_t lsd = (lsd_tile_lds_bytes(g, SMH_PIPE_TILE_LIMIT(g)) + 1023u) & ~1023u;
	if (lsd + 2048u >= SMH_LDS_PER_CU) return t;
	const uint32_t r = ((SMH_LDS_PER_CU - lsd - 2048u) / 2u) & ~1023u;
	if (4u * r <= SMH_LDS_PER_CU || r <= map_brq_lds_bytes(g)) return t;
	t.map_lds_total = r; t.map_grid_cap = SMH_PIPE_MAP_GRID; t.lsd_tile_limit = SMH_PIPE_TILE_LIMIT(g);
	return t;
}

#define SMH_SVC_AUTO_DEPTH 6u
#define SMH_OWN_QUEUES 16u
#define SMH_OWN_QUEUES_PROCESS 20u
static int pipeline_create_impl(smhv_ctx *c, uint32_t W, uint32_t H, uint32_t max_frames, uint32_t depth, const smhv_pipeline_options *opt_in, smhv_pipeline **out) {
	if (!c || !out || max_frames == 0 || depth == 0 || depth > SVC_MAX_SLOTS) return fail(SMHV_E_INVALID, "pipeline_create: bad arguments (depth 1..%u)", SVC_MAX_SLOTS);
	*out = nullptr;
	smhv_pipeline_options opt;
	memset(&opt, 0, sizeof opt);
	if (opt_in) {
		if (opt_in->size < 2 * sizeof(uint32_t) || opt_in->size > 4096u) return fail(SMHV_E_INVALID, "pipeline_create_ex: options.size is not set");
		memcpy(&opt, opt_in, opt_in->size < sizeof opt ? opt_in->size : sizeof opt);
	}
	if (opt.search > SMHV_SEARCH_FRAME || opt.occupancy_policy > 2u || opt.late_helpers > 2u || opt.streams > 8u || opt.room_for_others > 2u)
		return fail(SMHV_E_INVALID, "pipeline_create_ex: bad option value");
	CTX_OPEN(c);
	HIPCHK(hipSetDevice(c->device));
	Geom g0;
	{ int rc = compute_geom(W, H, &g0); if (rc) return rc; }
	smhv_pipeline *p = new (std::nothrow) smhv_pipeline();
	if (!p) return fail(SMHV_E_INVALID, "out of host memory");
	c->refs.fetch_add(1, std::memory_order_relaxed);
	p->ctx = c; p->depth = depth; p->opt = opt;
	if (opt.search != SMHV_SEARCH_BATCH && depth >= 3 && (opt.search == SMHV_SEARCH_FRAME || depth >= SMH_SVC_AUTO_DEPTH) && max_frames < (1u << 24)) {
		p->svc_waves = svc_waves_for(g0, SMH_SVC_TILE_LIMIT(g0), &p->svc_part_words, &p->svc_tile_cap, &p->svc_list_cap, &p->svc_lds, &p->svc_compact);
		p->svc = p->svc_waves > 0u;
	}
	if (opt.search == SMHV_SEARCH_FRAME && !p->svc) {
		ctx_release(c);
		delete p;
		return fail(SMHV_E_INVALID, "pipeline_create_ex: the frame-granular search needs depth >= 3 and a frame size whose mask tiles fit the LDS beside the streaming pass (%ux%u, depth %u)", W, H, depth);
	}
	if (p->svc) {
		bool atomics_ok = false;
		int native = 0;
		hipError_t ea = hipHostMalloc((void **)&p->h_svc, sizeof(SvcHost), hipHostMallocMapped | hipHostMallocCoherent);
		if (ea == hipSuccess) { memset(p->h_svc, 0, sizeof(SvcHost)); ea = hipHostGetDevicePointer((void **)&p->d_svc_host, p->h_svc, 0); }
		if (ea == hipSuccess && hipDeviceGetAttribute(&native, hipDeviceAttributeHostNativeAtomicSupported, c->device) != hipSuccess) { native = -1; (void)hipGetLastError(); }
		if (ea == hipSuccess) ea = svc_probe_host_atomics(p->h_svc, p->d_svc_host, &atomics_ok);
		if (g_no_host_atomics.load(std::memory_order_relaxed)) atomics_ok = false;
		if (ea != hipSuccess || !atomics_ok) {
			(void)hipGetLastError();
			logf(c, 2, "pipeline: device-side atomics on mapped host memory %s (hipDeviceAttributeHostNativeAtomicSupported = %d): no frame-granular search",
			     ea != hipSuccess ? hipGetErrorString(ea) : "do not take effect", native);
// ... 12 lines not shown
		p->svc_streams = p->svc ? std::min<uint32_t>(depth, opt.streams ? opt.streams : 2u) : 0u;
		p->adaptive = p->svc && opt.search == SMHV_SEARCH_AUTO;
		p->mode_frame = p->svc;
		p->slot_frame.assign(depth, 0);
		const uint32_t ns = (!p->svc || p->adaptive) ? depth : 0u;
		const uint32_t full[8] = {~0u, ~0u, ~0u, ~0u, ~0u, ~0u, ~0u, ~0u};
		p->stream.assign(ns, nullptr);
		auto own_queue = [p]() {
			if (p->own_queues >= SMH_OWN_QUEUES) return false;
			std::atomic<int> &cnt = g_own_queues[(uint32_t)p->ctx->device & 63u];
			if (cnt.fetch_add(1, std::memory_order_relaxed) >= (int)SMH_OWN_QUEUES_PROCESS) { cnt.fetch_sub(1, std::memory_order_relaxed); return false; }
			p->own_queues++;
			return true;
		};
		if (p->svc) {
			p->svc_stream.assign(p->svc_streams, nullptr);
			(void)own_queue();
			e = create_stream(&p->s_search, full);
			for (uint32_t i = 0; i < p->svc_streams && e == hipSuccess; ++i) e = create_stream(&p->svc_stream[i], own_queue() ? full : nullptr);
			if (e == hipSuccess && !(opt.flags & SMHV_PIPE_NO_PROLOGUE)) e = create_stream(&p->s_pro, own_queue() ? full : nullptr);
		}
		for (uint32_t i = 0; i < ns && e == hipSuccess; ++i) e = create_stream(&p->stream[i], own_queue() ? full : nullptr);
	}
	if (e == hipSuccess) e = hipEventCreateWithFlags(&p->ev_after, hipEventDisableTiming);
	for (uint32_t i = 0; i < depth && e == hipSuccess; ++i) e = hipEventCreateWithFlags(&p->done[i], hipEventDisableTiming);
	for (uint32_t i = 0; i < depth && e == hipSuccess; ++i) e = hipEventCreateWithFlags(&p->hold[i], hipEventDisableTiming);
	if (p->svc && e == hipSuccess) {
		p->ev_pub.assign(depth, nullptr); p->ev_pro.assign(depth, nullptr); p->seq.assign(depth, 0u); p->slot_st.assign(depth, nullptr);
		for (uint32_t i = 0; i < depth && e == hipSuccess; ++i) e = hipEventCreateWithFlags(&p->ev_pub[i], hipEventDisableTiming);
		for (uint32_t i = 0; i < depth && e == hipSuccess; ++i) e = hipEventCreateWithFlags(&p->ev_pro[i], hipEventDisableTiming);
		uint32_t lg = 8;
		while ((1ull << lg) < (uint64_t)depth * max_frames) ++lg;
		p->svc_ring_log2 = lg;
		int cus = 0;
		if (e == hipSuccess) e = hipDeviceGetAttribute(&cus, hipDeviceAttributeMultiprocessorCount, c->device);
		const int svc_cus = opt.room_for_others == 1u ? cus - std::max(cus / 8, 1) : cus;
		const bool every_cu = p->svc_waves >= 4u && !p->svc_compact;
		p->svc_wgs = opt.service_workgroups ? opt.service_workgroups : (uint32_t)std::max(every_cu ? svc_cus : std::min(cus * 9 / 16, svc_cus), 1);
		if (e == hipSuccess) e = hipMalloc((void **)&p->d_svc_ctl, sizeof(SvcCtl));
		if (e == hipSuccess) e = hipMemset(p->d_svc_ctl, 0, sizeof(SvcCtl));
		if (e == hipSuccess) e = hipMalloc((void **)&p->d_svc_ring, sizeof(unsigned long long) << lg);
		if (e == hipSuccess) e = hipMemset(p->d_svc_ring, 0, sizeof(unsigned long long) << lg);
		if (e == hipSuccess) e = hipMalloc((void **)&p->d_svc_slots, sizeof(SvcSlot) * depth);
		if (e == hipSuccess) e = hipMemset(p->d_svc_slots, 0, sizeof(SvcSlot) * depth);
		if (!(opt.flags & (SMHV_PIPE_NO_REMOTE_HELP | SMHV_PIPE_NO_TEAM_HELP)) && (uint64_t)p->svc_wgs * p->svc_waves <= 0xFFFFu) {
			const size_t owners = (size_t)p->svc_wgs * p->svc_waves;
			p->svc_store_words = svc_store_words_for(g0, p->svc_tile_cap, p->svc_compact);
			if (e == hipSuccess) e = hipMalloc((void **)&p->d_svc_remote, sizeof(SvcRemote) * owners);
			if (e == hipSuccess) e = hipMemset(p->d_svc_remote, 0, sizeof(SvcRemote) * owners);
			if (e == hipSuccess) e = hipMalloc((void **)&p->d_svc_store, sizeof(uint32_t) * owners * p->svc_store_words);
		}
	}
	if (e != hipSuccess) { smhv_pipeline_destroy(p); return fail(SMHV_E_HIP, "pipeline streams / events: %s", hipGetErrorString(e)); }
	for (uint32_t i = 0; i < depth; ++i) {
		int rc = smhv_batch_create(c, W, H, max_frames, &p->batch[i]);
		if (rc) { smhv_pipeline_destroy(p); return rc; }
		p->batch[i]->lsd_bs = depth >= 2 ? 512u : 1024u;
		p->batch[i]->lsd_prefer_classic = depth == 2 && lsd_rows_only(p->batch[i]->g);
		if (p->svc && !p->adaptive) {
			p->batch[i]->tune.map_prio = (opt.flags & SMHV_PIPE_NO_STREAM_PRIORITY) ? 0u : 1u;
			p->batch[i]->tune.map_deep = (opt.flags & SMHV_PIPE_THREE_LOAD_SETS) ? 1u : 0u;
			p->batch[i]->tune.map_overlapped = 1u;
		} else if (depth >= 3) {
			if (opt.occupancy_policy != 2u) p->tuning = pipeline_tuning(p->batch[i]->g);
			p->batch[i]->tune = p->tuning;
			p->batch[i]->tune.map_overlapped = 1u;
			if (opt.late_helpers == 1u) p->batch[i]->lsd_late_kc = 20u;
			if (opt.occupancy_policy == 0u) {
				p->adapt = true;
				hipError_t e2 = hipSuccess;
				for (int k = 0; k < 3 && e2 == hipSuccess; ++k) e2 = hipEventCreate(&p->batch[i]->ev_probe[k]);
				if (e2 != hipSuccess) { smhv_pipeline_destroy(p); return fail(SMHV_E_HIP, "pipeline probe events: %s", hipGetErrorString(e2)); }
				p->batch[i]->probe = true;
			}
		}
	}
	*out = p;
	return SMHV_OK;
}

extern "C" SMHV_API int smhv_pipeline_create(smhv_ctx *c, uint32_t W, uint32_t H, uint32_t max_frames, uint32_t depth, smhv_pipeline **out) {
	return pipeline_create_impl(c, W, H, max_frames, depth, nullptr, out);
}

extern "C" SMHV_API int smhv_pipeline_create_ex(smhv_ctx *c, uint32_t W, uint32_t H, uint32_t max_frames, uint32_t depth, const smhv_pipeline_options *opt, smhv_pipeline **out) {
	return pipeline_create_impl(c, W, H, max_frames, depth, opt, out);
}

static inline bool svc_alive(smhv_pipeline *p) { return (uint32_t)__atomic_load_n(&p->h_svc->state, __ATOMIC_ACQUIRE) != 0u; }

static int svc_launch(smhv_pipeline *p, uint32_t slot) {
	SvcParams sp;
	sp.ctl = p->d_svc_ctl; sp.ring = p->d_svc_ring; sp.slots = p->d_svc_slots; sp.host = p->d_svc_host;
	sp.cull_tab = p->svc_cull; sp.ray_off = p->ctx->d_ray_off; sp.max_gap = (float)p->svc_max_gap;
	sp.tile_cap = p->svc_tile_cap; sp.list_cap = p->svc_list_cap; sp.part_words = p->svc_part_words; sp.ring_log2 = p->svc_ring_log2;
	sp.epoch = ++p->svc_epoch;
	if (sp.epoch == 0u) sp.epoch = ++p->svc_epoch;
	sp.idle_short = p->opt.idle_close_us ? p->opt.idle_close_us * 2u : 100u;
	sp.flags = (p->opt.flags & SMHV_PIPE_NO_TEAM_HELP) ? 8u : 0u;
	sp.idle_long = 50000u;
	if (p->opt.flags & SMHV_PIPE_HELP_FIRST) sp.flags |= 16u;
	if (p->opt.flags & SMHV_PIPE_WALK_BIT_ROWS) sp.flags |= 32u;

	sp.remote = p->d_svc_remote; sp.remote_store = p->d_svc_store; sp.remote_store_words = p->svc_store_words;
	sp.remote_after = p->opt.remote_after ? p->opt.remote_after : 24u;
	sp.remote_tickets = std::min<uint32_t>(p->opt.remote_tickets ? p->opt.remote_tickets : 3u, 16u);
	sp.remote_last_div = p->opt.remote_last ? p->opt.remote_last : 6u;
	sp.compact = p->svc_compact;
	__atomic_fetch_or(&p->h_svc->state, (unsigned long long)sp.epoch, __ATOMIC_ACQ_REL);
	hipError_t e = hipStreamWaitEvent(p->s_search, p->ev_pub[slot], 0);
	if (e == hipSuccess) e = launch_lsd_service(p->batch[slot]->g, sp, p->svc_wgs, p->svc_waves, p->svc_lds, p->s_search);
	if (e != hipSuccess) {
		__atomic_fetch_and(&p->h_svc->state, 0xFFFFFFFF00000000ull, __ATOMIC_ACQ_REL);
		return fail(SMHV_E_HIP, "launching the line-search service: %s", hipGetErrorString(e));
	}
	p->h_svc->launches++;
	return SMHV_OK;
}

static int svc_wait_slot(smhv_pipeline *p, uint32_t slot) {
	const uint32_t target = p->seq[slot];
	if (target == 0u) return SMHV_OK;
	volatile uint32_t *flag = &p->h_svc->done_seq[slot];
	uint64_t spins = 0;
	struct timespec t0;
	clock_gettime(CLOCK_MONOTONIC, &t0);
	auto reached = [flag, target]() { return (int32_t)(__atomic_load_n(flag, __ATOMIC_ACQUIRE) - target) >= 0; };
	while (!reached()) {
		if (!svc_alive(p)) {
			if (reached()) break;
			int rc = svc_launch(p, slot);
			if (rc) return rc;
		}
		if (++spins < 4000u) { __builtin_ia32_pause(); continue; }
		struct timespec ts = {0, 20000};
		nanosleep(&ts, nullptr);
		if ((spins & 1023u) == 0u) {
			struct timespec t1;
			clock_gettime(CLOCK_MONOTONIC, &t1);
			if (t1.tv_sec - t0.tv_sec > 60) {
				const unsigned long long st = __atomic_load_n(&p->h_svc->state, __ATOMIC_ACQUIRE);
				return fail(SMHV_E_STATE, "pipeline_wait: slot %u (sequence %u, last completed %u) did not complete within 60 s: line-search service stalled "
				            "(submissions %u, launch alive %u, launches %u)", slot, target, *flag, (uint32_t)(st >> 32), (uint32_t)st, p->h_svc->launches);
			}
		}
	}
	return SMHV_OK;
}

static int svc_submit(smhv_pipeline *p, uint32_t slot, const void *d_frames, uint32_t n, uint32_t stages, int grayscale, uint32_t max_gap,
                      const smhv_anchors *anchors, void *after_stream, uint32_t *slot_out) {
	smhv_batch *b = p->batch[slot];
	if (!d_frames || n == 0 || n > b->max_frames) return fail(SMHV_E_INVALID, "bad arguments (n=%u, capacity %u)", n, b->max_frames);
	int rc = slot_wait(p, slot);
	if (rc) return rc;
	if (batch_check_errors(b, "pipeline_submit (the slot's previous submission, never waited for)") != SMHV_OK) logf(p->ctx, 2, "%s", t_last_error.c_str());
	hipStream_t st = p->svc_stream[p->submitted % p->svc_streams];
	if (p->adaptive) { b->tune = LaunchTuning{0u, 0u, 0u, (p->opt.flags & SMHV_PIPE_NO_STREAM_PRIORITY) ? 0u : 1u, (p->opt.flags & SMHV_PIPE_THREE_LOAD_SETS) ? 1u : 0u, 1u}; b->probe = false; b->lsd_late_kc = 0u; }
	Buffers probe{};
	const bool want_cull = (stages & SMHV_STAGE_MARKERS) && !(stages & SMHV_STAGE_EXACT_STATS);
	if (want_cull) { rc = sector_table_for(p->ctx, max_gap, st, &probe); if (rc) return rc; }
	if (!p->svc_key_valid || p->svc_cull != probe.cull_tab || p->svc_max_gap != max_gap) {
		for (uint32_t i = 0; i < p->depth; ++i) { rc = svc_wait_slot(p, i); if (rc) return rc; }
		struct timespec td0;
		clock_gettime(CLOCK_MONOTONIC, &td0);
		for (uint64_t spins = 0; svc_alive(p); ++spins) {
			struct timespec ts = {0, 20000}, td1;
			nanosleep(&ts, nullptr);
			if ((spins & 1023u) == 1023u) {
				clock_gettime(CLOCK_MONOTONIC, &td1);
				if (td1.tv_sec - td0.tv_sec > 60) {
					const unsigned long long stw = __atomic_load_n(&p->h_svc->state, __ATOMIC_ACQUIRE);
					return fail(SMHV_E_STATE, "pipeline_submit: the line-search service did not close within 60 s of its last submission (another gap threshold needs a new launch; "
					            "submissions %u, launch alive %u, launches %u)", (uint32_t)(stw >> 32), (uint32_t)stw, p->h_svc->launches);
				}
			}
		}
		p->svc_key_valid = true; p->svc_cull = probe.cull_tab; p->svc_max_gap = max_gap;
	}
	const hipStream_t s_first = p->s_pro ? p->s_pro : st;
	if (after_stream) {
		HIPCHK(hipEventRecord(p->ev_after, (hipStream_t)after_stream));
		HIPCHK(hipStreamWaitEvent(s_first, p->ev_after, 0));
	}
	if (p->held[slot]) {
		HIPCHK(hipStreamWaitEvent(s_first, p->hold[slot], 0));
		p->held[slot] = 0;
	}
	uint32_t seq = ++p->seq_counter;
	if (seq == 0u) seq = ++p->seq_counter;
	bool published = false;
	SvcPublish pub{p->d_svc_ctl, p->d_svc_ring, p->d_svc_slots, slot, seq, p->svc_ring_log2, probe.cull_tab, true, p->s_pro, p->ev_pro[slot], &published};
	__atomic_fetch_add(&p->h_svc->state, 1ull << 32, __ATOMIC_ACQ_REL);
	rc = batch_run_impl(b, d_frames, n, stages, grayscale, max_gap, anchors, st, st, &pub);
	if (rc && !published) {
		__atomic_fetch_sub(&p->h_svc->state, 1ull << 32, __ATOMIC_ACQ_REL);
		return rc;
	}
	const int rc_late = rc;
	p->seq[slot] = seq;
	p->slot_st[slot] = st;
	p->last_sl[slot] = st;
	p->slot_frame[slot] = 1;
	if (!svc_alive(p)) {
		HIPCHK(hipEventRecord(p->ev_pub[slot], st));
		rc = svc_launch(p, slot);
		if (rc) return rc;
	}
	p->submitted++;
	if (slot_out) *slot_out = slot;
	return rc_late;
// ... 136 lines not shown
	p->slot_frame[slot] = 0;
	p->submitted++;
	if (p->adaptive) { p->mc.count++; p->mc.frames += n; }
	if (slot_out) *slot_out = slot;
	return SMHV_OK;
}

extern "C" SMHV_API int smhv_pipeline_wait(smhv_pipeline *p, uint32_t slot) {
	if (!p || slot >= p->depth) return fail(SMHV_E_INVALID, "pipeline_wait: bad arguments");
	HIPCHK(hipSetDevice(p->ctx->device));
	{ int rc = slot_wait(p, slot); if (rc) return rc; }
	return batch_check_errors(p->batch[slot], "pipeline_wait");
}

extern "C" SMHV_API int smhv_pipeline_wait_all(smhv_pipeline *p) {
	if (!p) return fail(SMHV_E_INVALID, "null pipeline");
	HIPCHK(hipSetDevice(p->ctx->device));
	for (uint32_t i = 0; i < p->depth; ++i) { int r = slot_wait(p, i); if (r) return r; }
	int rc = SMHV_OK;
	for (uint32_t i = 0; i < p->depth; ++i) {
		std::string keep = t_last_error;
		const int r = batch_check_errors(p->batch[i], "pipeline_wait_all");
		if (r && !rc) rc = r;
		else if (r) t_last_error = keep;
	}
	return rc;
}

extern "C" SMHV_API int smhv_debug_pipeline_stats(smhv_pipeline *p, uint64_t out[32]) {
	if (!p || !out) return fail(SMHV_E_INVALID, "bad arguments");
	memset(out, 0, sizeof(uint64_t) * 32);
	if (!p->svc) return SMHV_OK;
	HIPCHK(hipSetDevice(p->ctx->device));
	HIPCHK(hipDeviceSynchronize());
	SvcCtl c;
	HIPCHK(hipMemcpy(&c, p->d_svc_ctl, sizeof c, hipMemcpyDeviceToHost));
	out[0] = 1u; out[1] = p->h_svc->launches; out[2] = c.stat_items; out[3] = c.stat_waves; out[4] = c.stat_busy; out[5] = c.stat_life;
	out[6] = (uint64_t)p->svc_wgs * p->svc_waves; out[7] = c.completed;
	for (int k = 0; k < 4; ++k) out[8 + k] = c.stat_phase[k];
	out[12] = c.stat_help;
	out[16] = c.stat_requests; out[17] = c.stat_attached; out[18] = c.stat_remote; out[19] = (uint64_t)(int64_t)c.help_avail;
	out[20] = c.stat_t_wait; out[21] = c.stat_t_sub; out[22] = c.stat_t_last;
	out[23] = c.stat_h_polls; out[24] = c.stat_h_empty; out[25] = c.stat_h_lost; out[26] = c.stat_h_idle_exit; out[27] = c.stat_h_closed_exit; out[28] = c.stat_h_cycles; out[29] = c.stat_h_cast_cycles;
	out[13] = (p->adaptive ? 2u : 0u) | (p->mode_frame ? 1u : 0u) | (p->mc.phase == 4u ? 4u : 0u); out[14] = (uint64_t)p->mc.rate[1]; out[15] = (uint64_t)p->mc.rate[0];
	return SMHV_OK;
}

extern "C" SMHV_API int smhv_debug_pipeline_peek(smhv_pipeline *p, uint64_t out[16]) {
	if (!p || !out) return fail(SMHV_E_INVALID, "bad arguments");
	memset(out, 0, sizeof(uint64_t) * 16);
	if (!p->svc) return SMHV_OK;
	HIPCHK(hipSetDevice(p->ctx->device));
	const unsigned long long st = __atomic_load_n(&p->h_svc->state, __ATOMIC_ACQUIRE);
	out[0] = st >> 32; out[1] = (uint32_t)st; out[2] = p->h_svc->launches; out[3] = p->seq_counter;
	out[14] = ((uint64_t)p->svc_wgs << 32) | p->svc_waves; out[15] = ((uint64_t)p->svc_part_words << 32) | p->svc_lds;
	std::lock_guard<std::mutex> lk(p->peek_mu);
	if (!p->s_peek) HIPCHK(hipStreamCreateWithFlags(&p->s_peek, hipStreamNonBlocking));
	if (!p->h_peek) HIPCHK(hipHostMalloc((void **)&p->h_peek, sizeof(SvcCtl)));
	SvcCtl *h_ctl = p->h_peek;
	HIPCHK(hipMemcpyAsync(h_ctl, p->d_svc_ctl, sizeof(SvcCtl), hipMemcpyDeviceToHost, p->s_peek));
	HIPCHK(hipStreamSynchronize(p->s_peek));
	out[4] = (uint64_t)(int64_t)h_ctl->avail; out[5] = h_ctl->head; out[6] = h_ctl->reserve; out[7] = h_ctl->closing; out[8] = h_ctl->completed; out[9] = h_ctl->busy;
	for (uint32_t i = 0; i < 4 && i < p->depth; ++i) out[10 + i] = ((uint64_t)p->seq[i] << 32) | __atomic_load_n(&p->h_svc->done_seq[i], __ATOMIC_ACQUIRE);
	return SMHV_OK;
}

extern "C" SMHV_API int smhv_pipeline_hold(smhv_pipeline *p, uint32_t slot, void *stream) {
	if (!p || slot >= p->depth) return fail(SMHV_E_INVALID, "pipeline_hold: bad arguments");
	HIPCHK(hipSetDevice(p->ctx->device));
	HIPCHK(hipEventRecord(p->hold[slot], (hipStream_t)stream));
	p->held[slot] = 1;
	return SMHV_OK;
}

extern "C" SMHV_API int smhv_pipeline_slot(smhv_pipeline *p, uint32_t slot, smhv_batch **batch, void **stream) {
	if (!p || slot >= p->depth) return fail(SMHV_E_INVALID, "pipeline_slot: bad arguments");
	if (batch) *batch = p->batch[slot];
	if (stream && p->svc && (p->slot_frame[slot] || p->stream.empty())) {
		HIPCHK(hipSetDevice(p->ctx->device));
		int rc = svc_wait_slot(p, slot);
		if (rc) return rc;
		*stream = (void *)(p->slot_st[slot] ? p->slot_st[slot] : p->svc_stream[0]);
		return SMHV_OK;
	}
	if (stream) *stream = (void *)(p->last_sl[slot] ? p->last_sl[slot] : p->stream[slot]);
	return SMHV_OK;
}

static int ensure_frame_buffers(smhv_ctx *c, uint32_t w, uint32_t h) {
	if (c->fb && c->W == w && c->H == h) return SMHV_OK;
	std::lock_guard<std::mutex> lk(c->mu);
	Geom g;
	int rc = compute_geom(w, h, &g);
	if (rc) return rc;
	HIPCHK(hipDeviceSynchronize());
	if (c->fb) { smhv_batch_destroy(c->fb); c->fb = nullptr; }
	if (c->h_ocr) { (void)hipHostFree(c->h_ocr); c->h_ocr = nullptr; }
	if (c->h_scales) { (void)hipHostFree(c->h_scales); c->h_scales = nullptr; }
	rc = smhv_batch_create(c, w, h, 1, &c->fb);
	if (rc) return rc;
	HIPCHK(hipHostMalloc((void **)&c->h_ocr, (size_t)g.qw * g.qh));
	HIPCHK(hipHostMalloc((void **)&c->h_scales, (size_t)g.qw * g.qh));
	memset(c->h_scales, 0, (size_t)g.qw * g.qh);
	memset(c->h_ocr, 0, (size_t)g.qw * g.qh);
	c->W = w; c->H = h;
	logf(c, 3, "allocated buffers for %ux%u frames (map ROI %u,%u %ux%u)", w, h, g.rx, g.ry, g.rw, g.rh);
	return SMHV_OK;
// ... 833 lines not shown
		}
		q->cv_job.notify_one();
		q->head++;
		q->acquired = false;
		return SMHV_OK;
	}
	if (layout == SMHV_PIXELS_BGRA8) {
		HIPCHK(hipMemcpyAsync(q->d_stage[slot], q->h_stage[slot], q->frame_bytes, hipMemcpyHostToDevice, q->s));
	} else if (yuv) {
		if (!q->d_raw[slot]) HIPCHK(hipMalloc((void **)&q->d_raw[slot], q->frame_bytes));
		HIPCHK(hipMemcpyAsync(q->d_raw[slot], q->h_stage[slot], yuv_tight_bytes(q->W, q->H), hipMemcpyHostToDevice, q->s));
		YuvRun run{};
		run.src = q->d_raw[slot]; run.dst = q->d_stage[slot]; run.W = q->W; run.H = q->H; run.n = 1; run.k = yuv_coef(yd);
		run.r[0] = yuv_tight_rect(q->W, q->H, yd.layout);
		HIPCHK(launch_yuv_to_bgra(run, 1, yd.layout, yd.bilinear, q->s));
	} else {
		if (!q->d_raw[slot]) HIPCHK(hipMalloc((void **)&q->d_raw[slot], q->frame_bytes));
		HIPCHK(hipMemcpyAsync(q->d_raw[slot], q->h_stage[slot], q->frame_bytes / 4 * bpp, hipMemcpyHostToDevice, q->s));
		HIPCHK(launch_to_bgra(q->d_raw[slot], q->d_stage[slot], (uint64_t)q->W * q->H, layout, q->s));
	}
	HIPCHK(hipMemsetAsync(q->d_acc + slot, 0, sizeof(uint32_t), q->s));
	HIPCHK(launch_crc32(q->d_stage[slot], q->frame_bytes / 4, q->wgs, q->rounds, q->x_skip, q->d_x_local, q->d_x_wg, q->d_acc + slot, q->s));
	HIPCHK(hipMemcpyAsync(q->h_acc + slot, q->d_acc + slot, sizeof(uint32_t), hipMemcpyDeviceToHost, q->s));
	HIPCHK(hipEventRecord(q->done[slot], q->s));
	q->head++;
	q->acquired = false;
	return SMHV_OK;
}

extern "C" SMHV_API int smhv_ingest_commit(smhv_ingest *q) { return smhv_ingest_commit_pixels(q, SMHV_PIXELS_BGRA8); }

extern "C" SMHV_API int smhv_ingest_push_pixels(smhv_ingest *q, const uint8_t *pixels, uint32_t layout) {
	if (!q || !pixels) return fail(SMHV_E_INVALID, "ingest_push: null argument");
	const uint32_t bpp = pixel_layout_bytes(layout);
	YuvDesc yd;
	if (!bpp && !yuv_decode(layout, &yd)) return fail(SMHV_E_INVALID, "ingest_push_pixels: unknown pixel layout 0x%x", layout);
	if (q->roi && bpp && layout != SMHV_PIXELS_BGRA8) return fail(SMHV_E_INVALID, "ingest_push_pixels: a queue created with SMHV_INGEST_ROI_UPLOAD takes BGRA8, NV12 and I420 frames only");
	uint8_t *dst = nullptr;
	int rc = smhv_ingest_acquire(q, &dst);
	if (rc) return rc;
	memcpy(dst, pixels, bpp ? q->frame_bytes / 4 * bpp : (size_t)yuv_tight_bytes(q->W, q->H));
	return smhv_ingest_commit_pixels(q, layout);
}

namespace smh { extern std::atomic<uint32_t> g_map_band_rows, g_map_band_major; }
extern "C" SMHV_API int smhv_debug_map_band_rows(uint32_t rows) {
	g_map_band_major.store((rows >> 31) ? 1u : ((rows >> 30) & 1u) ? 2u : 0u, std::memory_order_relaxed);
	rows &= 0x3FFFFFFFu;
	if (rows & 7u) return fail(SMHV_E_INVALID, "debug_map_band_rows: a multiple of 8 (0: the library's rule)");
	g_map_band_rows.store(rows, std::memory_order_relaxed);
	return SMHV_OK;
}

extern "C" SMHV_API int smhv_debug_band_rows(uint32_t frame_w, uint32_t frame_h, uint32_t n, int fused, uint32_t *rows, uint32_t *bands, int *tiles) {
	Geom g;
	int rc = compute_geom(frame_w, frame_h, &g);
	if (rc) return rc;
	uint32_t rb = 0;
	map_band_rows(g.rh, n ? n : 1u, fused, &rb, tiles);
	if (rows) *rows = rb;
	if (bands) *bands = (g.rh + rb - 1) / rb;
	return SMHV_OK;
}

extern "C" SMHV_API int smhv_debug_batch_mask_state(smhv_batch *b, uint32_t *stale_frames, int *eager) {
	if (!b) return fail(SMHV_E_INVALID, "null batch");
	std::lock_guard<std::mutex> lk(b->mask_mu);
	if (stale_frames) *stale_frames = b->mask_stale;
	if (eager) *eager = b->mask_eager ? 1 : 0;
	return SMHV_OK;
}

extern "C" SMHV_API int smhv_debug_batch_ui_state(smhv_batch *b, uint32_t *stale_frames, int *eager) {
	if (!b) return fail(SMHV_E_INVALID, "null batch");
	std::lock_guard<std::mutex> lk(b->ui_mu);
	if (stale_frames) *stale_frames = b->ui_stale;
	if (eager) *eager = b->ui_eager ? 1 : 0;
	return SMHV_OK;
}

extern "C" SMHV_API int smhv_debug_batch_materialize_ui(smhv_batch *b, void *stream) {
	if (!b) return fail(SMHV_E_INVALID, "null batch");
	CTX_OPEN(b->ctx);
	HIPCHK(hipSetDevice(b->ctx->device));
	return batch_materialize_ui(b, (hipStream_t)stream);
}

extern "C" SMHV_API int smhv_debug_mask_expand(smhv_batch *b, uint32_t n, void *stream) {
	if (!b || n == 0 || n > b->max_frames) return fail(SMHV_E_INVALID, "debug_mask_expand: bad arguments");
	CTX_OPEN(b->ctx);
	HIPCHK(hipSetDevice(b->ctx->device));
	HIPCHK(launch_mask_expand(b->g, b->d_bits, b->d_mask, n, (hipStream_t)stream));
	return SMHV_OK;
}

extern "C" SMHV_API int smhv_debug_ingest_feed(smhv_ingest *q, uint32_t n, uint32_t *counter) { return smhv_debug_ingest_feed_pixels(q, n, counter, SMHV_PIXELS_BGRA8); }

extern "C" SMHV_API int smhv_debug_ingest_feed_pixels(smhv_ingest *q, uint32_t n, uint32_t *counter, uint32_t pixels) {
	if (!q || !counter) return fail(SMHV_E_INVALID, "ingest_feed: null argument");
	for (uint32_t i = 0; i < n; ++i) {
		uint8_t *buf = nullptr;
		int rc = smhv_ingest_acquire(q, &buf);
		if (rc) return rc;
		const uint32_t c = (*counter)++;
		buf[0] = (uint8_t)c; buf[1] = (uint8_t)(c >> 8); buf[2] = (uint8_t)(c >> 16); buf[3] = 255;
		rc = smhv_ingest_commit_pixels(q, pixels);
// ... 204 lines not shown
```

squad-mortar-helper_amd/csrc/smh_service.inc:

```
#pragma once

struct SvcKernelArgs { Geom g; SvcParams p; };
#ifdef __HIP_DEVICE_COMPILE__
typedef const __attribute__((address_space(4))) SvcSlot *SvcSlotPtr;
typedef const __attribute__((address_space(4))) SvcKernelArgs *SvcKernelArgsPtr;
#else
typedef const SvcSlot *SvcSlotPtr;
typedef const SvcKernelArgs *SvcKernelArgsPtr;
#endif
__device__ __forceinline__ SvcKernelArgsPtr svc_args(const void *ka) {
	const unsigned long long v = (unsigned long long)(uintptr_t)ka;
	const uint32_t lo = (uint32_t)__builtin_amdgcn_readfirstlane((int)(uint32_t)v), hi = (uint32_t)__builtin_amdgcn_readfirstlane((int)(uint32_t)(v >> 32));
	return (SvcKernelArgsPtr)(uintptr_t)(((unsigned long long)hi << 32) | lo);
}

#define SVC_WS_WORDS ((uint32_t)((sizeof(WShared) + 15u) / 16u * 4u))
#define SVC_POLL_SLEEP 64

__device__ __forceinline__ uint32_t svc_ld(const uint32_t *p) { return __hip_atomic_load(p, __ATOMIC_RELAXED, __HIP_MEMORY_SCOPE_AGENT); }

__device__ __forceinline__ uint32_t *lds_ptr(uint32_t byte_off) { return (uint32_t *)(LdsWord *)(uintptr_t)uniform_u32(byte_off); }
__device__ __forceinline__ uint32_t lds_off(const void *p) { return (uint32_t)(uintptr_t)(const LdsByte *)p; }

template <bool COMPACT>
__device__ __attribute__((noinline)) void svc_frame_global(const void *kargs, uint32_t slot, uint32_t f, uint32_t part_off, uint32_t cull_off, uint32_t dirs_off) {
	SvcKernelArgsPtr ka = svc_args(kargs);
	slot = uniform_u32(slot); f = uniform_u32(f);
	uint32_t *part = lds_ptr(part_off);
	const Geom g = ka->g;
	const Buffers b = ((SvcSlotPtr)(ka->p.slots + slot))->b;
	const FrameAux aux = b.aux[f];
	lsd_frame_seq<LSD_MODE_GLOBAL, true, false, SVC_WIN_REUSE(COMPACT), SVC_LEAN_SAMPLER(COMPACT)>(g, b, f, ka->p.max_gap, aux, part + SVC_WS_WORDS, *(WShared *)part, lds_ptr(cull_off), (const RayDir *)lds_ptr(dirs_off), 0u, ka->p.list_cap);
}

template <bool COMPACT>
__device__ __attribute__((noinline)) unsigned long long svc_frame(const void *kargs, uint32_t slot, uint32_t f, uint32_t part_off, uint32_t cull_off, uint32_t dirs_off) {
	SvcKernelArgsPtr ka = svc_args(kargs);
	slot = uniform_u32(slot); f = uniform_u32(f);
	uint32_t *part = lds_ptr(part_off);
	const Geom g = ka->g;
	const Buffers b = ((SvcSlotPtr)(ka->p.slots + slot))->b;
	const FrameAux aux = b.aux[f];
	WShared &ws = *(WShared *)part;
	uint32_t *smem = part + SVC_WS_WORDS;
	if (!aux.open || aux.n_mask_px == 0) {
		if ((threadIdx.x & 63u) == 0) { b.results[f].n_lines = 0; b.results[f].rounds = 0; b.results[f].ray_steps = 0; b.results[f].status = SMHV_FRAME_OK; }
	} else {
		const uint32_t tile_cap = ka->p.tile_cap;
		if ((threadIdx.x & 63u) == 0) {
			SvcSlot *sl = ka->p.slots + slot;
			ws.rem_done = (unsigned long long)(uintptr_t)&sl->done;
			ws.rem_n = __hip_atomic_load(&sl->n, __ATOMIC_RELAXED, __HIP_MEMORY_SCOPE_AGENT);
		}
		FrameView v;
		bool fits;
		if constexpr (COMPACT) {
			uint32_t rc = 2u;
			if (b.tiled && aux.tiles && !(ka->p.flags & 32u)) rc = frame_setup_tilec_occ(g, b, f, aux, smem, tile_cap, &ws.ntiles, v, smem + tilec_mask_words(g.rw, g.rh, tile_cap), 2u * ka->p.list_cap + SVC_WIN_STRIDE(true));
			fits = rc == 2u ? frame_setup_tilec(g, b, f, aux, smem, tile_cap, &ws.ntiles, v) : rc == 0u;
		} else {
			uint32_t rc = 2u;
			if (b.tiled && aux.tiles && !(ka->p.flags & 32u)) rc = frame_setup_tile_occ(g, b, f, aux, smem, tile_cap, &ws.ntiles, v, smem + tile_mask_words(g.rw, g.rh, tile_cap), 2u * ka->p.list_cap + SVC_WIN_STRIDE(false));
			fits = rc == 2u ? frame_setup_tile<true>(g, b, f, aux, smem, tile_cap, &ws.ntiles, v) : rc == 0u;
		}
		if (fits) {
			if constexpr (COMPACT) lsd_frame_seq<LSD_MODE_TILEC, true, true, SVC_WIN_REUSE(true)>(g, b, f, ka->p.max_gap, aux, smem, ws, lds_ptr(cull_off), (const RayDir *)lds_ptr(dirs_off), tilec_mask_words(g.rw, g.rh, tile_cap), ka->p.list_cap, &v);
			else lsd_frame_seq<LSD_MODE_TILE, true, true, SVC_WIN_REUSE(false), SVC_LEAN_SAMPLER(false)>(g, b, f, ka->p.max_gap, aux, smem, ws, lds_ptr(cull_off), (const RayDir *)lds_ptr(dirs_off), tile_mask_words(g.rw, g.rh, tile_cap), ka->p.list_cap, &v);
		} else svc_frame_global<COMPACT>(kargs, slot, f, part_off, cull_off, dirs_off);
	}
	const unsigned long long t_search_end = __builtin_amdgcn_s_memtime();
	if (b.rec_stages & SMH_REC_ON) frame_record_tail_wave(&((const SvcKernelArgs *)kargs)->g, &((const SvcSlot *)(ka->p.slots + slot))->b, f);
	return t_search_end;
}

#define SVC_HELP_IDLE_POLLS 160u
template <bool COMPACT>
__device__ __attribute__((noinline)) void svc_help(const void *kargs, uint32_t owner_off, uint32_t my_off, uint32_t cull_off, uint32_t dirs_off) {
	SvcKernelArgsPtr ka = svc_args(kargs);
	uint32_t *opart = lds_ptr(owner_off), *mpart = lds_ptr(my_off);
	WShared &wo = *(WShared *)opart;
	const uint32_t lane = threadIdx.x & 63u;
	uint32_t ok = 0;
	if (lane == 0 && W_LD_ACQ(&wo.want_set) && W_LD(&wo.late) < SEQ_MAX_HELPERS) {
		const uint32_t prev = __hip_atomic_fetch_add(&wo.late, 1u, __ATOMIC_ACQ_REL, __HIP_MEMORY_SCOPE_WORKGROUP);
		if (prev < SEQ_MAX_HELPERS && W_LD_ACQ(&wo.want_set)) ok = 1u;
		else __hip_atomic_fetch_sub(&wo.late, 1u, __ATOMIC_RELEASE, __HIP_MEMORY_SCOPE_WORKGROUP);
	}
	if (!uniform_u32(ok)) return;
	const uint32_t rw = ka->g.rw, rh = ka->g.rh, tile_cap = ka->p.tile_cap, list_cap = ka->p.list_cap;
	const float max_gap = ka->p.max_gap;
	const uint32_t cull = cull_mode_for(ka->p.cull_tab, max_gap);
	const float *ray_off = ka->p.ray_off;
	Win m;
	if constexpr (COMPACT) tilec_win(m, rw, rh, opart + SVC_WS_WORDS, tile_cap); else tile_win(m, rw, rh, opart + SVC_WS_WORDS, tile_cap);
	uint32_t *wwin = mpart + SVC_WS_WORDS + (COMPACT ? tilec_mask_words(rw, rh, tile_cap) : tile_mask_words(rw, rh, tile_cap)) + 2u * list_cap;
	const uint32_t *cull_tab = lds_ptr(cull_off);
	const RayDir *dirs = (const RayDir *)lds_ptr(dirs_off);
	uint32_t idle = 0;
	WinTag wtag = {0, 0, false};
	uint32_t wframe = 0u;
	while (uniform_u32(W_LD_ACQ(&wo.want_set))) {
		uint32_t key = 0u;
		if (lane < SEQ_HELP_SLOTS && W_LD_ACQ(&wo.rob[lane].state) == (uint32_t)H_POSTED) key = ~((wo.rob[lane].lines_seen << 2) | lane);
		key = wave_max32_dpp(key);
		if (!key) {
			if (++idle > SVC_HELP_IDLE_POLLS) break;
			__builtin_amdgcn_s_sleep(8);
			continue;
		}
		WSlot &sl = wo.rob[~key & 3u];
		uint32_t got = 0;
		if (lane == 0) { uint32_t expect = H_POSTED; got = __hip_atomic_compare_exchange_strong(&sl.state, &expect, (uint32_t)H_TAKEN, __ATOMIC_ACQ_REL, __ATOMIC_RELAXED, __HIP_MEMORY_SCOPE_WORKGROUP) ? 1u : 0u; }
		if (!uniform_u32(got)) continue;
		idle = 0;
		const uint32_t px = uniform_u32(sl.px), py = uniform_u32(sl.py);
		if (SVC_WIN_REUSE(COMPACT)) {
			const uint32_t oframe = uniform_u32(W_LD(&wo.frame_no));
			if (oframe != wframe) { wframe = oframe; wtag.valid = false; }
		}
		float xs, ys, ex0, ey0;
		unsigned long long wkey;
		uint32_t st_sum;
#ifdef SMH_LSD_WDEBUG
		unsigned long long sprof[8] = {0, 0, 0, 0, 0, 0, 0, 0}, slast = __builtin_amdgcn_s_memtime(), uprof[12] = {0, 0, 0, 0, 0, 0, 0, 0, 0, 0, 0, 0};
		uint32_t n_units = 0;
		seq_cast_candidate<COMPACT ? LSD_MODE_TILEC : LSD_MODE_TILE, SVC_WIN_REUSE(COMPACT), SVC_LEAN_SAMPLER(COMPACT)>(m, wwin, &wtag, cull_tab, cull, dirs, ray_off, max_gap, px, py, xs, ys, wkey, ex0, ey0, st_sum, sprof, slast, uprof, n_units);
#else
		seq_cast_candidate<COMPACT ? LSD_MODE_TILEC : LSD_MODE_TILE, SVC_WIN_REUSE(COMPACT), SVC_LEAN_SAMPLER(COMPACT)>(m, wwin, &wtag, cull_tab, cull, dirs, ray_off, max_gap, px, py, xs, ys, wkey, ex0, ey0, st_sum);
#endif
		if (lane == 0) {
			sl.ptx = xs; sl.pty = ys; sl.best = wkey; sl.ex = ex0; sl.ey = ey0; sl.steps = st_sum;
			W_ST_REL(&sl.state, (uint32_t)H_DONE);
		}
	}
	if (lane == 0) __hip_atomic_fetch_sub(&wo.late, 1u, __ATOMIC_RELEASE, __HIP_MEMORY_SCOPE_WORKGROUP);
}

#define SVC_REMOTE_IDLE_POLLS 12u
#define SVC_REMOTE_IDLE_POLLS_FREE 600u
#define SVC_REMOTE_MAX_HELPERS 12u
template <bool COMPACT>
__device__ __attribute__((noinline)) void svc_help_remote(const void *kargs, uint32_t ticket, uint32_t my_off, uint32_t cull_off, uint32_t dirs_off) {
	SvcKernelArgsPtr ka = svc_args(kargs);
	ticket = uniform_u32(ticket);
	const uint32_t owner = ticket & 0xFFFFu, gen16 = ticket >> 16;
	SvcRemote *r = ka->p.remote + owner;
	const uint32_t lane = threadIdx.x & 63u;
	uint32_t ok = 0, gen = 0;
	if (lane == 0) {
		unsigned long long st = g_ld64(&r->state);
		while ((st & SVC_REMOTE_OPEN) && ((uint32_t)(st >> 32) & 0xFFFFu) == gen16 && ((uint32_t)st & 0x7FFFFFFFu) < SVC_REMOTE_MAX_HELPERS) {
			if (__hip_atomic_compare_exchange_strong(&r->state, &st, st + 1ull, __ATOMIC_ACQ_REL, __ATOMIC_RELAXED, __HIP_MEMORY_SCOPE_AGENT)) { ok = 1u; gen = (uint32_t)(st >> 32); break; }
		}
	}
	if (!uniform_u32(ok)) return;
	gen = uniform_u32(gen);
	if (lane == 0) __hip_atomic_fetch_add(&ka->p.ctl->stat_attached, 1u, __ATOMIC_RELAXED, __HIP_MEMORY_SCOPE_AGENT);
	__builtin_amdgcn_fence(__ATOMIC_ACQUIRE, "agent");
	const uint32_t rw = ka->g.rw, rh = ka->g.rh, tile_cap = ka->p.tile_cap, list_cap = ka->p.list_cap;
	const uint32_t ntiles = min(uniform_u32((uint32_t)g_ld64(&r->info)), tile_cap);
	uint32_t *mpart = lds_ptr(my_off), *store = mpart + SVC_WS_WORDS;
	{
		const uint4 *src = (const uint4 *)(ka->p.remote_store + (size_t)owner * ka->p.remote_store_words);
		uint4 *dst = (uint4 *)store;
		for (uint32_t i = lane; i < (ntiles + 1u) * 2u; i += 64u) dst[i] = src[i];
		const uint32_t q0 = (tile_cap + 1u) * 2u, nq = ((COMPACT ? tilec_idx_words(rw, rh) : tile_idx_words(rw, rh)) + 3u) / 4u;
		for (uint32_t i = lane; i < nq; i += 64u) dst[q0 + i] = src[q0 + i];
	}
	wave_lds_sync();
	const float max_gap = ka->p.max_gap;
	const uint32_t cull = cull_mode_for(ka->p.cull_tab, max_gap);
	const float *ray_off = ka->p.ray_off;
	Win m;
	if constexpr (COMPACT) tilec_win(m, rw, rh, store, tile_cap); else tile_win(m, rw, rh, store, tile_cap);
	uint32_t *wwin = store + (COMPACT ? tilec_mask_words(rw, rh, tile_cap) : tile_mask_words(rw, rh, tile_cap)) + 2u * list_cap;
	const uint32_t *cull_tab = lds_ptr(cull_off);
	const RayDir *dirs = (const RayDir *)lds_ptr(dirs_off);
	WinTag wtag = {0, 0, false};
	uint32_t idle = 0, n_cast = 0, n_polls = 0, n_empty = 0, n_lost = 0, exit_idle = 0;
	unsigned long long t_cast = 0ull;
	const unsigned long long t_att = __builtin_amdgcn_s_memtime();
	while (true) {
		++n_polls;
		const unsigned long long st = g_ld64(&r->state);
		unsigned long long pw = 0ull, cw = 0ull;
		if (lane < SVC_REMOTE_RING) { pw = g_ld64(&r->ring[lane].post); cw = g_ld64(&r->ring[lane].claim); }
		if (!(uniform_u32((uint32_t)st) & (uint32_t)SVC_REMOTE_OPEN) || uniform_u32((uint32_t)(st >> 32)) != gen) break;
		const uint32_t pk = (uint32_t)(pw >> 32);
		const bool open_post = lane < SVC_REMOTE_RING && pk != 0u && (unsigned long long)pk > cw;
		const uint32_t key = wave_max32_dpp(open_post ? ~pk : 0u);
		if (!key) {
			const int32_t waiting = (int32_t)uniform_u32((uint32_t)__hip_atomic_load(&ka->p.ctl->avail, __ATOMIC_RELAXED, __HIP_MEMORY_SCOPE_AGENT));
			++n_empty;
			if (++idle > (waiting > 0 ? SVC_REMOTE_IDLE_POLLS : SVC_REMOTE_IDLE_POLLS_FREE)) { exit_idle = 1u; break; }
			if (idle < 4u) __builtin_amdgcn_s_sleep(24); else __builtin_amdgcn_s_sleep(72);
			continue;
		}
		const uint32_t k = ~key;
		const uint32_t e = (uint32_t)__builtin_ctzll(__ballot(open_post && pk == k));
		uint32_t mine = 0;
		if (lane == 0) mine = __hip_atomic_fetch_max(&r->ring[e].claim, (unsigned long long)k, __ATOMIC_RELAXED, __HIP_MEMORY_SCOPE_AGENT) < (unsigned long long)k ? 1u : 0u;
		if (!uniform_u32(mine)) { ++n_lost; continue; }
		idle = 0;
		const unsigned long long t_c0 = __builtin_amdgcn_s_memtime();
		const uint32_t pxy = (uint32_t)__builtin_amdgcn_readlane((int)(uint32_t)pw, (int)e);
		const uint32_t px = pxy & 0xFFFFu, py = pxy >> 16;
		float xs, ys, ex0, ey0;
		unsigned long long wkey;
		uint32_t st_sum;
#ifdef SMH_LSD_WDEBUG
		unsigned long long sprof[8] = {0, 0, 0, 0, 0, 0, 0, 0}, slast = __builtin_amdgcn_s_memtime(), uprof[12] = {0, 0, 0, 0, 0, 0, 0, 0, 0, 0, 0, 0};
		uint32_t n_units = 0;
		seq_cast_candidate<COMPACT ? LSD_MODE_TILEC : LSD_MODE_TILE, SVC_WIN_REUSE(COMPACT), SVC_LEAN_SAMPLER(COMPACT)>(m, wwin, &wtag, cull_tab, cull, dirs, ray_off, max_gap, px, py, xs, ys, wkey, ex0, ey0, st_sum, sprof, slast, uprof, n_units);
#else
		seq_cast_candidate<COMPACT ? LSD_MODE_TILEC : LSD_MODE_TILE, SVC_WIN_REUSE(COMPACT), SVC_LEAN_SAMPLER(COMPACT)>(m, wwin, &wtag, cull_tab, cull, dirs, ray_off, max_gap, px, py, xs, ys, wkey, ex0, ey0, st_sum);
#endif
		++n_cast;
		t_cast += __builtin_amdgcn_s_memtime() - t_c0;
		if (lane == 0) {
			SvcRemoteEntry *en = &r->ring[e];
			const rem_u32x4 a = {k, st_sum, (uint32_t)(wkey >> 32), (uint32_t)wkey};
			const rem_u32x4 b = {k, __float_as_uint(ex0), __float_as_uint(ey0), ((uint32_t)(ys * 2.0f) << 16) | ((uint32_t)(xs * 2.0f) & 0xFFFFu)};
			g_st128(en->res_a, a);
			g_st128(en->res_b, b);
		}
	}
	asm volatile("s_waitcnt vmcnt(0)" ::: "memory");
	if (lane == 0) {
		__hip_atomic_fetch_sub(&r->state, 1ull, __ATOMIC_RELEASE, __HIP_MEMORY_SCOPE_AGENT);
		SvcCtl *ctl = ka->p.ctl;
		__hip_atomic_fetch_add(&ctl->stat_remote, n_cast, __ATOMIC_RELAXED, __HIP_MEMORY_SCOPE_AGENT);
		__hip_atomic_fetch_add(&ctl->stat_h_polls, n_polls, __ATOMIC_RELAXED, __HIP_MEMORY_SCOPE_AGENT);
		__hip_atomic_fetch_add(&ctl->stat_h_empty, n_empty, __ATOMIC_RELAXED, __HIP_MEMORY_SCOPE_AGENT);
		__hip_atomic_fetch_add(&ctl->stat_h_lost, n_lost, __ATOMIC_RELAXED, __HIP_MEMORY_SCOPE_AGENT);
		__hip_atomic_fetch_add(exit_idle ? &ctl->stat_h_idle_exit : &ctl->stat_h_closed_exit, 1u, __ATOMIC_RELAXED, __HIP_MEMORY_SCOPE_AGENT);
		__hip_atomic_fetch_add(&ctl->stat_h_cycles, __builtin_amdgcn_s_memtime() - t_att, __ATOMIC_RELAXED, __HIP_MEMORY_SCOPE_AGENT);
		__hip_atomic_fetch_add(&ctl->stat_h_cast_cycles, t_cast, __ATOMIC_RELAXED, __HIP_MEMORY_SCOPE_AGENT);
	}
}

__device__ __forceinline__ uint32_t svc_sibling_in_need(uint32_t *smem, uint32_t part_words, uint32_t nw, uint32_t me) {
	for (uint32_t w = 0; w < nw; ++w) {
		if (w == me) continue;
		const WShared &wsib = *(const WShared *)(smem + w * part_words);
		if (uniform_u32(W_LD(&wsib.want_set)) && uniform_u32(W_LD(&wsib.late)) < SEQ_MAX_HELPERS) return lds_off(smem + w * part_words);
	}
	return 0xFFFFFFFFu;
}

__device__ __forceinline__ uint32_t svc_pop(const SvcParams &p, uint32_t *team_smem, uint32_t nw, uint32_t me, bool checker, uint32_t *help_ticket) {
	const uint32_t lane = threadIdx.x & 63u;
	SvcCtl *ctl = p.ctl;
	const unsigned long long t_idle0 = __builtin_amdgcn_s_memtime();
	uint32_t polls = 0;
	while (true) {
		const unsigned long long look = __hip_atomic_load((const unsigned long long *)&ctl->avail, __ATOMIC_RELAXED, __HIP_MEMORY_SCOPE_AGENT);
		if ((uint32_t)(look >> 32) == p.epoch) return 0xFFFFFFFFu;
		if (p.remote && ((p.flags & 16u) || (int32_t)(uint32_t)look <= 0)) {
			const unsigned long long hl = __hip_atomic_load((const unsigned long long *)&ctl->help_avail, __ATOMIC_RELAXED, __HIP_MEMORY_SCOPE_AGENT);
			if ((int32_t)(uint32_t)hl > 0) {
				uint32_t hgot = 0, ht = 0;
				if (lane == 0) {
					if (__hip_atomic_fetch_sub(&ctl->help_avail, 1, __ATOMIC_ACQUIRE, __HIP_MEMORY_SCOPE_AGENT) > 0) { ht = __hip_atomic_fetch_add(&ctl->help_head, 1u, __ATOMIC_RELAXED, __HIP_MEMORY_SCOPE_AGENT); hgot = 1u; }
					else __hip_atomic_fetch_add(&ctl->help_avail, 1, __ATOMIC_RELAXED, __HIP_MEMORY_SCOPE_AGENT);
				}
				if (uniform_u32(hgot)) {
					ht = uniform_u32(ht);
					const unsigned long long *he = &ctl->help_ring[ht & (SVC_HELP_RING - 1u)];
// ... 26 lines not shown
			if (team_smem && svc_sibling_in_need(team_smem, p.part_words, nw, me) != 0xFFFFFFFFu) return 0xFFFFFFFEu;
			if (polls < 8u) __builtin_amdgcn_s_sleep(SVC_POLL_SLEEP); else __builtin_amdgcn_s_sleep(127);
		}
		++polls;
		if (checker && polls >= 8u && (polls & 3u) == 0u) {
			const unsigned long long idle = (__builtin_amdgcn_s_memtime() - t_idle0) >> 10;
			if (idle >= p.idle_short) {
				uint32_t leave = 0;
				if (lane == 0) {
					unsigned long long st = __hip_atomic_load(&p.host->state, __ATOMIC_RELAXED, __HIP_MEMORY_SCOPE_SYSTEM);
					if ((uint32_t)st != p.epoch) {
						__hip_atomic_store(&ctl->closing, p.epoch, __ATOMIC_RELEASE, __HIP_MEMORY_SCOPE_AGENT);
						leave = 1u;
					} else {
						const uint32_t comp = __hip_atomic_load(&ctl->completed, __ATOMIC_RELAXED, __HIP_MEMORY_SCOPE_AGENT);
						const bool quiet = svc_ld(&ctl->busy) == 0u && __hip_atomic_load(&ctl->avail, __ATOMIC_RELAXED, __HIP_MEMORY_SCOPE_AGENT) <= 0;
						const bool drained = quiet && (int32_t)(comp - (uint32_t)(st >> 32)) >= 0;
						const bool stalled = quiet && idle >= p.idle_long;
						if ((drained || stalled) &&
						    __hip_atomic_compare_exchange_strong(&p.host->state, &st, st & 0xFFFFFFFF00000000ull, __ATOMIC_ACQ_REL, __ATOMIC_RELAXED, __HIP_MEMORY_SCOPE_SYSTEM)) {
							__hip_atomic_store(&ctl->closing, p.epoch, __ATOMIC_RELEASE, __HIP_MEMORY_SCOPE_AGENT);
							leave = 1u;
						}
					}
				}
				if (uniform_u32(leave)) return 0xFFFFFFFFu;
			}
		}
	}
}

#define SVC_MAX_WAVES 4
#pragma clang diagnostic push
#pragma clang diagnostic ignored "-Wpass-failed"
template <bool COMPACT>
__device__ __forceinline__ void svc_kernel_body(const Geom &g, const SvcParams &p) {
	extern __shared__ __attribute__((aligned(16))) uint32_t smem[];
	__shared__ uint32_t cull_tab[SMH_CULL_TAB_WORDS];
	__shared__ RayDir s_dirs[SMH_LSD_RAYS];
	const uint32_t lane = threadIdx.x & 63u, wave = threadIdx.x >> 6;
	if (p.cull_tab) for (uint32_t i = threadIdx.x; i < SMH_CULL_TAB_WORDS; i += blockDim.x) cull_tab[i] = p.cull_tab[i];
	for (uint32_t i = threadIdx.x; i < SMH_LSD_RAYS; i += blockDim.x) s_dirs[i] = g_ray_table[i];
	if (lane == 0) {
		WShared &w0 = *(WShared *)(smem + wave * p.part_words);
		w0.want_set = 0u; w0.late = 0u;
		if (SVC_WIN_REUSE(COMPACT)) w0.frame_no = 0u;
		const uint32_t owner = blockIdx.x * (blockDim.x >> 6) + wave;
		const bool rem = p.remote != nullptr && !(p.flags & 8u) && owner < 0x10000u;
		w0.rem_r = rem ? (unsigned long long)(uintptr_t)(p.remote + owner) : 0ull;
		w0.rem_store = (unsigned long long)(uintptr_t)(p.remote_store + (size_t)owner * p.remote_store_words);
		w0.rem_ctl = (unsigned long long)(uintptr_t)p.ctl;
		w0.rem_after = p.remote_after; w0.rem_tickets = p.remote_tickets; w0.rem_owner = owner; w0.rem_cap = p.tile_cap;
		w0.rem_open = 0u; w0.rem_gen = 0u; w0.rem_k = 0u; w0.rem_nr = 0u;
		w0.rem_last_div = p.remote_last_div; w0.rem_flags = (p.flags & 16u) ? 1u : 0u;
	}
	__syncthreads();
	uint32_t *part = smem + wave * p.part_words;
	const uint32_t nw = blockDim.x >> 6;
	const bool team = nw > 1u && !(p.flags & 8u);
	if (p.flags & 4u) __builtin_amdgcn_s_setprio(3);
	const unsigned long long t_start = __builtin_amdgcn_s_memtime();
	unsigned long long t_busy = 0ull, t_help = 0ull, t_phase[4] = {0ull, 0ull, 0ull, 0ull}, rt_wait = 0ull;
	uint32_t n_items = 0u;
	while (true) {
		if (team) {
			const uint32_t sib = svc_sibling_in_need(smem, p.part_words, nw, uniform_u32(wave));
			if (sib != 0xFFFFFFFFu) {
				const unsigned long long t_h = __builtin_amdgcn_s_memtime();
				svc_help<COMPACT>((const void *)__builtin_amdgcn_kernarg_segment_ptr(), sib, lds_off(part), lds_off(cull_tab), lds_off(s_dirs));
				t_help += __builtin_amdgcn_s_memtime() - t_h;
				continue;
			}
		}
		uint32_t help_ticket = 0;
		const uint32_t item = svc_pop(p, team ? smem : nullptr, nw, uniform_u32(wave), blockIdx.x == 0u && uniform_u32(wave) == 0u, &help_ticket);
		if (item == 0xFFFFFFFEu) continue;
		if (item == 0xFFFFFFFDu) {
			const unsigned long long t_h = __builtin_amdgcn_s_memtime();
			svc_help_remote<COMPACT>((const void *)__builtin_amdgcn_kernarg_segment_ptr(), help_ticket, lds_off(part), lds_off(cull_tab), lds_off(s_dirs));
			t_help += __builtin_amdgcn_s_memtime() - t_h;
			continue;
		}
		if (item == 0xFFFFFFFFu) break;
		const unsigned long long t_item = __builtin_amdgcn_s_memtime(), rt_item = __builtin_amdgcn_s_memrealtime();
		const uint32_t slot = item >> 24, f = item & 0xFFFFFFu;
		if (!(p.flags & 1u)) {
			__builtin_amdgcn_fence(__ATOMIC_ACQUIRE, "agent");
			__builtin_amdgcn_s_dcache_inv();
		}
		const unsigned long long t_acq = __builtin_amdgcn_s_memtime();
		const unsigned long long t_srch = svc_frame<COMPACT>((const void *)__builtin_amdgcn_kernarg_segment_ptr(), slot, f, lds_off(part), lds_off(cull_tab), lds_off(s_dirs));
		const unsigned long long t_rec = __builtin_amdgcn_s_memtime();
		if (!(p.flags & 2u)) __builtin_amdgcn_fence(__ATOMIC_RELEASE, "agent");
		if (lane == 0) {
			SvcSlot *sl = p.slots + slot;
			const uint32_t n = __hip_atomic_load(&sl->n, __ATOMIC_RELAXED, __HIP_MEMORY_SCOPE_AGENT), seq = __hip_atomic_load(&sl->seq, __ATOMIC_RELAXED, __HIP_MEMORY_SCOPE_AGENT);
			const unsigned long long t_pub = __hip_atomic_load(&sl->t_pub, __ATOMIC_RELAXED, __HIP_MEMORY_SCOPE_AGENT), rt_now = __builtin_amdgcn_s_memrealtime();
			rt_wait += rt_item - t_pub;
			__hip_atomic_fetch_sub(&p.ctl->busy, 1u, __ATOMIC_RELAXED, __HIP_MEMORY_SCOPE_AGENT);
			if (__hip_atomic_fetch_add(&sl->done, 1u, __ATOMIC_ACQ_REL, __HIP_MEMORY_SCOPE_AGENT) + 1u == n) {
				__hip_atomic_store(&p.host->done_seq[slot], seq, __ATOMIC_RELEASE, __HIP_MEMORY_SCOPE_SYSTEM);
				__hip_atomic_fetch_add(&p.ctl->stat_t_sub, rt_now - t_pub, __ATOMIC_RELAXED, __HIP_MEMORY_SCOPE_AGENT);
				__hip_atomic_fetch_add(&p.ctl->stat_t_last, rt_now - rt_item, __ATOMIC_RELAXED, __HIP_MEMORY_SCOPE_AGENT);
				__hip_atomic_fetch_add(&p.ctl->completed, 1u, __ATOMIC_RELEASE, __HIP_MEMORY_SCOPE_AGENT);
			}
		}
		const unsigned long long t_end = __builtin_amdgcn_s_memtime();
// ... 49 lines not shown
```

squad-mortar-helper_amd/csrc/smh_stream.hip:

```cpp
#include <algorithm>
#include <atomic>
#include <cstdlib>

#include "smh_device.h"

namespace smh {

__device__ __forceinline__ uint32_t tile_occupancy(uint64_t rows_any, uint32_t lane, uint32_t ntr, uint8_t *occp, uint32_t pitch) {
	uint32_t alo = (uint32_t)rows_any, ahi = (uint32_t)(rows_any >> 32);
	alo |= SMH_DPP(alo, 0x101); ahi |= SMH_DPP(ahi, 0x101);
	alo |= SMH_DPP(alo, 0x102); ahi |= SMH_DPP(ahi, 0x102);
	alo |= SMH_DPP(alo, 0x104); ahi |= SMH_DPP(ahi, 0x104);
	uint32_t occ = 0;
#pragma unroll
	for (int t = 0; t < 4; ++t) occ |= (((alo >> (8 * t)) & 255u) ? 1u : 0u) << t;
#pragma unroll
	for (int t = 0; t < 3; ++t) occ |= (((ahi >> (8 * t)) & 255u) ? 1u : 0u) << (4 + t);
	if (lane & 7u) occ = 0u;
	uint32_t mine = 0;
#pragma unroll
	for (int t = 0; t < 7; ++t) {
		const uint64_t bal = __ballot((occ >> t) & 1u) & 0x0101010101010101ull;
		const uint32_t byte = (uint32_t)((bal * 0x0102040810204080ull) >> 56);
		if (lane == (uint32_t)t) mine = byte;
// ... 295 lines not shown

	if (my_q && do_ocr && live) {
#pragma unroll
		for (int k = 0; k < 4; ++k) {
			const int row = k < 2 ? r0 - 3 + k : r1 + k - 1;
			const int qrow = row - qy0;
			if (qrow < 0 || qrow >= (int)g.qh || row < 0 || row >= (int)g.rh) continue;
			if ((uint32_t)qrow + SMH_OCR_DILATE_RADIUS > g.qh) continue;
			const uint4 v = *(const uint4 *)(fp + (size_t)row * row_bytes);
			const uint32_t pv[4] = {v.x, v.y, v.z, v.w};
#pragma unroll
			for (int c = 0; c < 4; ++c) {
				const uint32_t p = pv[c], bb = p & 255u, gg = (p >> 8) & 255u, rr8 = (p >> 16) & 255u;
				const uint32_t mx = max(rr8, max(gg, bb)), mn = min(rr8, min(gg, bb));
				const bool w = (mx == mn) && mn >= SMH_OCR_BRIGHTNESS_THRESHOLD && ((qw_ >> c) & 1u);
				or_w(c, (uint64_t)(w ? 1u : 0u) << (row - base));
			}
		}
	}

	uint32_t *s_hits = s_dyn;
	auto rare = [](bool c) -> bool { if constexpr (TILES) return __builtin_expect(c, 0); else return c; };
	auto group = [&](const u32x4 (&px)[GR], int r) {
		uint32_t prehits = 0, wrows = 0, erows = 0;
#pragma unroll
		for (int k = 0; k < GR; ++k) {
			const int row = r + k;
			if (row > re) break;
			const uint32_t pv[4] = {px[k].x, px[k].y, px[k].z, px[k].w};
			const bool out_row = row >= r0 && row < r1;
			const int qrow = row - qy0;
			const bool q_row = wave_q && qrow >= 0 && qrow < (int)g.qh;
			uint32_t wnib = 0, enib = 0;
			if (q_row) {
#pragma unroll
				for (int c = 0; c < 4; ++c) {
					const uint32_t p = pv[c], bb = p & 255u, gg = (p >> 8) & 255u, rr8 = (p >> 16) & 255u;
					const uint32_t mx = max(rr8, max(gg, bb)), mn = min(rr8, min(gg, bb));
					const bool w = (mx == mn) && mn >= SMH_OCR_BRIGHTNESS_THRESHOLD;
					const bool e = (4u * (mx - mn) <= SMH_OCR_SIMILARITY_EDGE_THRESHOLD) && mn >= SMH_OCR_BRIGHTNESS_EDGE_THRESHOLD && !w;
					wnib |= (w ? 1u : 0u) << c;
					enib |= (e ? 1u : 0u) << c;
				}
				const bool nb_row = (uint32_t)qrow + SMH_OCR_DILATE_RADIUS <= g.qh;
				if (nb_row) wrows |= (wnib & qw_) << (4 * k);
				if (out_row) erows |= (enib & qv) << (4 * k);
			}
			if (out_row) {
				uint32_t lum[4] = {0, 0, 0, 0};
				if (GRAY || q_row) {
#pragma unroll
					for (int c = 0; c < 4; ++c) lum[c] = luma_bgra(pv[c]);
				}
				if constexpr (GRAY == 2) {
					if (do_ui && qact) SMH_ST32(loff >> 2, lum[0] | (lum[1] << 8) | (lum[2] << 16) | (lum[3] << 24), uibase + (size_t)row * (g.ui_pitch >> 2));
				} else if (do_ui && qact) {
					u32x4 o;
					uint32_t ov[4];
#pragma unroll
					for (int c = 0; c < 4; ++c) {
						const uint32_t p = pv[c], bb = p & 255u, gg = (p >> 8) & 255u, rr8 = (p >> 16) & 255u;
						if (GRAY) ov[c] = __builtin_amdgcn_perm(0u, lum[c], 0x0D000000u);
						else ov[c] = rr8 | (gg << 8) | (bb << 16) | 0xFF000000u;
					}
					o.x = ov[0]; o.y = ov[1]; o.z = ov[2]; o.w = ov[3];
					SMH_ST128(loff, o, uibase + (size_t)row * g.ui_pitch);
				}
				if (q_row && in_q) {
					const uint32_t l4 = lum[0] | (lum[1] << 8) | (lum[2] << 16) | (lum[3] << 24);
					if (do_ocr) SMH_ST32(qoff, ~(l4 & nib_to_bytes(wnib & qv)), op + (size_t)qrow * g.ocr_pitch);
					if (do_scales && (uint32_t)qrow >= start_y) {
						const uint32_t nz = ((((l4 & 0x7F7F7F7Fu) + 0x7F7F7F7Fu) | l4) >> 7) & 0x01010101u;
						SMH_ST32(qoff, ones_to_bytes(nz), sp + (size_t)qrow * g.ocr_pitch);
					}
				}
			}
			if (rare(do_mask && __any(bright4(pv) != 0u))) {
				uint32_t pre = 0;
#pragma unroll
				for (int c = 0; c < 4; ++c) pre |= marker_prefilter(pv[c]) ? (1u << c) : 0u;
				prehits |= (pre & vmask) << (4 * k);
			}
		}
		if (rare(wave_q && __any((wrows | erows) != 0u))) {
			const int sh = r - base;
#pragma unroll
			for (int c = 0; c < 4; ++c) { or_w(c, (uint64_t)rows_of_col(wrows, c) << sh); or_e(c, (uint64_t)rows_of_col(erows, c) << sh); }
		}
		if (rare(do_mask && __any(prehits != 0u))) {
			uint32_t *hpx = s_hits + gwave * 160u;
			uint32_t *hres = hpx + 64;
			unsigned short *hid = (unsigned short *)(hres + 64);
			const uint32_t cnt = (uint32_t)__popc(prehits);
			uint32_t incl = cnt;
			for (int o = 1; o < 64; o <<= 1) { const uint32_t t = __shfl_up(incl, o); if (lane >= (uint32_t)o) incl += t; }
			const uint32_t total = __shfl(incl, 63);
			const uint32_t off = incl - cnt;
			hres[lane] = 0u;
			for (uint32_t hb = 0; hb < total; hb += 64u) {
				uint32_t o = off - hb;
#pragma unroll
				for (int k = 0; k < GR; ++k) {
					const uint32_t pk[4] = {px[k].x, px[k].y, px[k].z, px[k].w};
#pragma unroll
					for (int c = 0; c < 4; ++c)
						if ((prehits >> (4 * k + c)) & 1u) {
							if (o < 64u) { hpx[o] = pk[c]; hid[o] = (unsigned short)((lane << 4) | (uint32_t)(4 * k + c)); }
							++o;
						}
				}
				__builtin_amdgcn_wave_barrier();
				const uint32_t e = hb + lane;
				if (e < total) {
					const uint32_t p = hpx[lane];
					if (marker_exact((p >> 16) & 255u, (p >> 8) & 255u, p & 255u)) {
						const uint32_t id = hid[lane];
						atomicOr(&hres[id >> 4], 1u << (id & 15u));
					}
				}
				__builtin_amdgcn_wave_barrier();
			}
			const uint32_t res = hres[lane];
			if (res) {
				const int sh = r - base;
#pragma unroll
				for (int c = 0; c < 4; ++c) P[c] |= (uint64_t)rows_of_col(res, c) << sh;
			}
		}
	};

	{
		const uint8_t *dummy = (const uint8_t *)&b.aux[f];
		auto load4 = [&](u32x4 (&dst)[GR], int r) {
#pragma unroll
			for (int k = 0; k < GR; ++k) {
				const bool inside = r + k <= re;
				const uint8_t *rowp = inside ? fbase + (size_t)(r + k) * row_bytes : dummy;
				SMH_LD128(dst[k], inside ? loff : 0u, rowp);
			}
		};
		if constexpr (SETS == 2) {
			u32x4 S0[GR], S1[GR];
			load4(S0, rs);
			for (int r = rs; ; r += 8) {
				load4(S1, r + 4);
				SMH_WAIT_SET(4, S0);
				group(S0, r);
				if (r + 4 > re) break;
				load4(S0, r + 8);
				SMH_WAIT_SET(4, S1);
				group(S1, r + 4);
				if (r + 8 > re) break;
			}
			asm volatile("s_waitcnt vmcnt(0) ; smh-drain" : "+v"(S0[0]), "+v"(S0[1]), "+v"(S0[2]), "+v"(S0[3]), "+v"(S1[0]), "+v"(S1[1]), "+v"(S1[2]), "+v"(S1[3]) : : "memory");
		} else {
			u32x4 S0[GR], S1[GR], S2[GR];
			load4(S0, rs);
			load4(S1, rs + 4);
			for (int r = rs; ; r += 12) {
				load4(S2, r + 8);
				SMH_WAIT_SET(8, S0);
				group(S0, r);
				if (r + 4 > re) break;
				load4(S0, r + 12);
				SMH_WAIT_SET(8, S1);
				group(S1, r + 4);
				if (r + 8 > re) break;
				load4(S1, r + 16);
				SMH_WAIT_SET(8, S2);
				group(S2, r + 8);
				if (r + 12 > re) break;
			}
			asm volatile("s_waitcnt vmcnt(0) ; smh-drain" : "+v"(S0[0]), "+v"(S0[1]), "+v"(S0[2]), "+v"(S0[3]), "+v"(S1[0]), "+v"(S1[1]), "+v"(S1[2]), "+v"(S1[3]),
			             "+v"(S2[0]), "+v"(S2[1]), "+v"(S2[2]), "+v"(S2[3]) : : "memory");
		}
	}

	uint64_t V[4];
#pragma unroll
	for (int c = 0; c < 4; ++c) {
		const uint64_t w = get_w(c);
		V[c] = w | (w << 1) | (w << 2) | (w << 3) | (w >> 1) | (w >> 2) | (w >> 3);
	}
	__shared__ uint64_t s_edge_first[16], s_edge_last[16], s_first[16][4], s_last[16][4];
	if (lane == 0) { s_edge_first[gwave] = P[0]; s_first[gwave][0] = V[0]; s_first[gwave][1] = V[1]; s_first[gwave][2] = V[2]; s_first[gwave][3] = V[3]; }
	if (lane == 63) { s_edge_last[gwave] = P[3]; s_last[gwave][0] = V[0]; s_last[gwave][1] = V[1]; s_last[gwave][2] = V[2]; s_last[gwave][3] = V[3]; }
	__syncthreads();
	if (do_mask) {
		uint64_t left = __shfl_up(P[3], 1), right = __shfl_down(P[0], 1);
		if (lane == 0) left = wave > 0 ? s_edge_last[gwave - 1] : 0ull;
		if (lane == 63) right = wave + 1 < nwave ? s_edge_first[gwave + 1] : 0ull;
		const int nrows = r1 - r0;
		const uint64_t rowmask = ((nrows >= 61 ? ~0ull : ((1ull << nrows) - 1ull)) << 3);
		uint64_t D[4];
#define SMH_VERT(p) ((p) | ((p) << 1) | ((p) >> 1))
		D[0] = SMH_VERT(P[0]) | left | P[1];
		D[1] = SMH_VERT(P[1]) | P[0] | P[2];
		D[2] = SMH_VERT(P[2]) | P[1] | P[3];
		D[3] = SMH_VERT(P[3]) | P[2] | right;
#undef SMH_VERT
#pragma unroll
		for (int c = 0; c < 4; ++c) D[c] = ((vmask >> c) & 1u) ? (D[c] & rowmask) : 0ull;
		const uint32_t quads_padded = (g.m_quads + 15u) & ~15u;
		const uint64_t any = D[0] | D[1] | D[2] | D[3];
		const uint64_t lanes_set = __ballot(any != 0ull);
		uint32_t occ7 = 0;
		uint32_t *tiled_out = nullptr;
		if constexpr (TILES) {
			MapKernelArgsPtr kb = ka;
			asm volatile("" : "+s"(kb));
			tiled_out = kb->b.tiled;
			uint8_t *const occ_out = kb->b.occ;
			const uint32_t ntr = ((uint32_t)nrows + 7u) >> 3, opitch = occ_pitch(g);
			uint8_t *occp = occ_out + (size_t)f * occ_stride(g) + (size_t)((uint32_t)r0 >> 3) * opitch + wave;
			if (lanes_set) occ7 = tile_occupancy(any >> 3, lane, ntr, occp, opitch);
			else if (lane < ntr) occp[(size_t)lane * opitch] = 0;
			if (band == 0u && q == 0u) b.aux[f].tiles = 1u;
		}
		if (q < quads_padded && !lanes_set) {
			uint32_t *bbase = b.bits + (size_t)f * g.bits_stride_w;
			const uint32_t boff = (q >> 3) * 4u;
			const bool bit_lane = (lane & 7u) == 0;
			if (bit_lane)
				for (int row = r0; row < r1; ++row) *(uint32_t *)((uint8_t *)bbase + (size_t)row * g.bits_pitch_w * 4u + boff) = 0u;
		} else if (q < quads_padded) {
			uint32_t *bbase = b.bits + (size_t)f * g.bits_stride_w;
			const uint32_t boff = (q >> 3) * 4u;
			const bool bit_lane = (lane & 7u) == 0;
			uint32_t *tp = nullptr;
			uint32_t tpitch = 0;
			if constexpr (TILES) { tp = tiled_out + (size_t)f * tiled_stride_w(g) + ((size_t)((uint32_t)r0 >> 3) * g.bits_pitch_w + (q >> 3)) * 8u; tpitch = g.bits_pitch_w * 8u; }
#pragma unroll
			for (int half = 0; half < 2; ++half) {
				const uint32_t d0 = (uint32_t)(D[0] >> (32 * half)), d1 = (uint32_t)(D[1] >> (32 * half)), d2 = (uint32_t)(D[2] >> (32 * half)), d3 = (uint32_t)(D[3] >> (32 * half));
				const int row_lo = max(r0, base + 32 * half), row_hi = min(r1, base + 32 * half + 32);
				for (int row = row_lo; row < row_hi; ++row) {
					const uint32_t bit = (uint32_t)(row - base) & 31u;
					const uint32_t nib = ((d0 >> bit) & 1u) | (((d1 >> bit) & 1u) << 1) | (((d2 >> bit) & 1u) << 2) | (((d3 >> bit) & 1u) << 3);
					uint32_t v = nib;
					v |= SMH_DPP(v, 0x101) << 4;
					v |= SMH_DPP(v, 0x102) << 8;
					v |= SMH_DPP(v, 0x104) << 16;
					if (bit_lane) *(uint32_t *)((uint8_t *)bbase + (size_t)row * g.bits_pitch_w * 4u + boff) = v;
					if constexpr (TILES) {
						const uint32_t i = (uint32_t)(row - r0);
						if ((occ7 >> (i >> 3)) & 1u) tp[(size_t)(i >> 3) * tpitch + (i & 7u)] = v;
					}
				}
			}
		}
		if (lanes_set) {
			const uint64_t rows_set = wave_or64(any);
			const uint32_t cnt = wave_sum32(__popcll(D[0]) + __popcll(D[1]) + __popcll(D[2]) + __popcll(D[3]));
			if (lane == 0) {
				FrameAux *a = &b.aux[f];
				atomicMin(&a->y_min, (uint32_t)(base + __builtin_ctzll(rows_set)));
				atomicMax(&a->y_max, (uint32_t)(base + 63 - __builtin_clzll(rows_set)));
				atomicMin(&a->w_min, (wave * 64u + (uint32_t)__builtin_ctzll(lanes_set)) >> 3);
				atomicMax(&a->w_max, (wave * 64u + 63u - (uint32_t)__builtin_clzll(lanes_set)) >> 3);
				atomicAdd(&a->n_mask_px, cnt);
			}
		}
	}
	if (!(wave_q && do_ocr)) return;
	uint64_t X[12];
#pragma unroll
	for (int c = 0; c < 4; ++c) {
		uint64_t l = __shfl_up(V[c], 1), r = __shfl_down(V[c], 1);
		if (lane == 0) l = wave > 0 ? s_last[gwave - 1][c] : 0ull;
		if (lane == 63) r = wave + 1 < nwave ? s_first[gwave + 1][c] : 0ull;
		X[c] = l; X[4 + c] = V[c]; X[8 + c] = r;
	}
#pragma unroll
	for (int c = 0; c < 4; ++c) {
		uint64_t d = 0;
#pragma unroll
		for (int k = -3; k <= 3; ++k) d |= X[4 + c + k];
		uint64_t kk = get_e(c) & d;
		while (kk) {
			const int bit = __builtin_ctzll(kk);
			kk &= kk - 1;
			const int row = base + bit;
			const uint32_t p = *(const uint32_t *)(fp + (size_t)row * row_bytes + 4 * c);
			const uint32_t l = luma_bgra(p);
			op[(size_t)(row - qy0) * g.ocr_pitch + qoff + c] = (uint8_t)(255u - l);
		}
	}
}

template <bool GRAY, bool LOOP, int SETS, bool TILES>
__global__ void __launch_bounds__(1024) k_map_brq_pass(Geom g, Buffers b, uint32_t flags, uint32_t qflags, uint32_t RB, uint32_t fixed_start_y, int use_anchor_start,
                                                       uint32_t nbands, uint32_t items) {
#ifdef SMH_MAP_FAT
	asm volatile("; register footprint experiment" ::: SMH_MAP_FAT);
#endif
	static_assert(sizeof(MapKernelArgs) == sizeof(Geom) + sizeof(Buffers) + 7 * 4 + 4 || sizeof(MapKernelArgs) == sizeof(Geom) + sizeof(Buffers) + 7 * 4, "the kernel's parameter list");
	MapKernelArgsPtr ka = (MapKernelArgsPtr)__builtin_amdgcn_kernarg_segment_ptr();
	if (flags & MAP_PRIO) __builtin_amdgcn_s_setprio(3);
	if (LOOP) {
		for (uint32_t item = blockIdx.x; item < items; item += gridDim.x) {
			const uint32_t f = item / nbands, band = item - f * nbands;
			map_brq_item<GRAY ? 1 : 0, SETS, TILES>(ka, f, band);
			__syncthreads();
// ... 43 lines not shown
}

hipError_t launch_map_pass(const Geom &g, const Buffers &b, uint32_t n, uint32_t flags, int grayscale, hipStream_t s, bool tiles_wanted, bool overlapped) {
	const uint32_t RB = band_rows_for(g.rh, n, MAP_RB_MAX, tiles_wanted && b.tiled != nullptr, overlapped);
	const dim3 grid((g.rh + RB - 1) / RB, n);
	const unsigned lds = (g.m_block / 64u) * 640u;
	const bool tiles = tiles_wanted && b.tiled != nullptr && (RB & 7u) == 0u;
	if (grayscale == 2) {
		if (flags & MAP_BYTES) return hipErrorInvalidValue;
		if (tiles) hipLaunchKernelGGL((k_map_pass_luma<true>), grid, dim3(g.m_block), lds, s, g, b, flags, RB);
		else hipLaunchKernelGGL((k_map_pass_luma<false>), grid, dim3(g.m_block), lds, s, g, b, flags, RB);
	} else if (tiles) {
		if (grayscale) hipLaunchKernelGGL((k_map_pass<true, true>), grid, dim3(g.m_block), lds, s, g, b, flags, RB);
		else hipLaunchKernelGGL((k_map_pass<false, true>), grid, dim3(g.m_block), lds, s, g, b, flags, RB);
	} else {
		if (grayscale) hipLaunchKernelGGL((k_map_pass<true, false>), grid, dim3(g.m_block), lds, s, g, b, flags, RB);
		else hipLaunchKernelGGL((k_map_pass<false, false>), grid, dim3(g.m_block), lds, s, g, b, flags, RB);
	}
	return hipGetLastError();
}

static uint32_t map_brq_static_lds() {
	static const uint32_t v = [] { hipFuncAttributes a; return hipFuncGetAttributes(&a, (const void *)k_map_brq_pass<true, true, 2, false>) == hipSuccess ? (uint32_t)a.sharedSizeBytes : 2048u; }();
	return v;
}
uint32_t map_brq_lds_bytes(const Geom &g) { return map_brq_static_lds() + (g.m_block / 64u) * 640u; }

hipError_t launch_map_brq_pass(const Geom &g, const Buffers &b, uint32_t n, uint32_t flags, uint32_t qflags, int grayscale, uint32_t fixed_start_y, int use_anchor_start, hipStream_t s,
                               const LaunchTuning *tune) {
	const uint32_t cap0 = tune ? tune->map_grid_cap : 0u;
	const uint32_t RB0 = band_rows_for(g.rh, n, MAPQ_RB_MAX, false);
	bool no_tiles = b.tiled == nullptr || (tune && tune->map_deep) || (cap0 && cap0 < ((g.rh + RB0 - 1) / RB0) * n);
	uint32_t RB = no_tiles ? RB0 : band_rows_for(g.rh, n, MAPQ_RB_MAX, true, tune && tune->map_overlapped);
	uint32_t nbands = (g.rh + RB - 1) / RB, items = nbands * n;
	if (!no_tiles && cap0 && cap0 < items) { no_tiles = true; RB = RB0; nbands = (g.rh + RB - 1) / RB; items = nbands * n; }
	unsigned lds = (g.m_block / 64u) * 640u;
	if (tune && tune->map_lds_total > map_brq_lds_bytes(g)) lds = tune->map_lds_total - map_brq_static_lds();
	if (lds > 65536u) {
		static std::atomic<uint64_t> attr_devices{0};
		int dev = 0;
		hipError_t e = hipGetDevice(&dev);
		if (e != hipSuccess) return e;
		if (dev >= 64 || !((attr_devices.load(std::memory_order_acquire) >> dev) & 1ull)) {
			const void *fns[] = {(const void *)k_map_brq_pass<true, true, 2, false>, (const void *)k_map_brq_pass<false, true, 2, false>, (const void *)k_map_brq_pass<true, false, 2, false>,
			                     (const void *)k_map_brq_pass<false, false, 2, false>, (const void *)k_map_brq_pass<true, false, 2, true>, (const void *)k_map_brq_pass<false, false, 2, true>,
			                     (const void *)k_map_brq_pass<true, false, 3, false>, (const void *)k_map_brq_pass<false, false, 3, false>,
			                     (const void *)k_map_brq_pass_luma<true, 2, false>, (const void *)k_map_brq_pass_luma<false, 2, false>, (const void *)k_map_brq_pass_luma<false, 2, true>,
			                     (const void *)k_map_brq_pass_luma<false, 3, false>};
			for (const void *fn : fns) if (e == hipSuccess) e = hipFuncSetAttribute(fn, hipFuncAttributeMaxDynamicSharedMemorySize, 160 * 1024 - 2048);
			if (e != hipSuccess) return e;
			if (dev < 64) attr_devices.fetch_or(1ull << dev, std::memory_order_release);
		}
	}
	if (tune && tune->map_prio) flags |= MAP_PRIO;
	flags |= work_item_order(tune && tune->map_overlapped);
	const uint32_t cap = tune ? tune->map_grid_cap : 0u;
	const bool deep = tune && tune->map_deep && !(cap && cap < items);
	const bool tiles = !no_tiles && (RB & 7u) == 0u && !(cap && cap < items) && !deep;
#define SMH_LAUNCH_MAPQ(GRAYV, LOOPV, SETSV, TILESV, GRID) \
	hipLaunchKernelGGL((k_map_brq_pass<GRAYV, LOOPV, SETSV, TILESV>), GRID, dim3(g.m_block), lds, s, g, b, flags, qflags, RB, fixed_start_y, use_anchor_start, nbands, items)
#define SMH_LAUNCH_MAPQ_LUMA(LOOPV, SETSV, TILESV, GRID) \
	hipLaunchKernelGGL((k_map_brq_pass_luma<LOOPV, SETSV, TILESV>), GRID, dim3(g.m_block), lds, s, g, b, flags, qflags, RB, fixed_start_y, use_anchor_start, nbands, items)
	if (grayscale == 2) {
		if (cap && cap < items) SMH_LAUNCH_MAPQ_LUMA(true, 2, false, dim3(cap));
		else if (deep) SMH_LAUNCH_MAPQ_LUMA(false, 3, false, dim3(nbands, n));
		else if (tiles) SMH_LAUNCH_MAPQ_LUMA(false, 2, true, dim3(nbands, n));
		else SMH_LAUNCH_MAPQ_LUMA(false, 2, false, dim3(nbands, n));
	} else if (cap && cap < items) {
		if (grayscale) SMH_LAUNCH_MAPQ(true, true, 2, false, dim3(cap)); else SMH_LAUNCH_MAPQ(false, true, 2, false, dim3(cap));
	} else if (deep) {
		if (grayscale) SMH_LAUNCH_MAPQ(true, false, 3, false, dim3(nbands, n)); else SMH_LAUNCH_MAPQ(false, false, 3, false, dim3(nbands, n));
	} else if (tiles) {
		if (grayscale) SMH_LAUNCH_MAPQ(true, false, 2, true, dim3(nbands, n)); else SMH_LAUNCH_MAPQ(false, false, 2, true, dim3(nbands, n));
	} else {
		if (grayscale) SMH_LAUNCH_MAPQ(true, false, 2, false, dim3(nbands, n)); else SMH_LAUNCH_MAPQ(false, false, 2, false, dim3(nbands, n));
	}
#undef SMH_LAUNCH_MAPQ_LUMA
#undef SMH_LAUNCH_MAPQ
	return hipGetLastError();
}

template <int NR>
__global__ void __launch_bounds__(1024) k_pattern_copy(Geom g, Buffers b, uint32_t RB, uint32_t band_major) {
	uint32_t f = blockIdx.y, band = blockIdx.x;
	if (band_major) {
		const uint32_t id = blockIdx.y * gridDim.x + blockIdx.x;
		band = id / gridDim.y; f = id - band * gridDim.y;
	}
	const uint32_t q = threadIdx.x;
	const int r0 = (int)(band * RB), r1 = min(r0 + (int)RB, (int)g.rh);
	if (q >= g.m_quads) return;
	const uint8_t *fp = b.frames + (size_t)f * g.frame_bytes + ((size_t)g.ry * g.W + g.m_ax) * 4 + (size_t)q * 16;
	uint8_t *up = b.ui + (size_t)f * g.ui_stride + (size_t)q * 16;
	const int qy0 = (int)(g.qy - g.ry);
	const int qq = (int)q - (int)((g.q_ax - g.m_ax) >> 2);
	const bool in_q = qq >= 0 && (uint32_t)qq < g.q_quads;
	uint8_t *op = b.ocr + (size_t)f * g.ocr_stride + (size_t)(in_q ? qq : 0) * 4;
	uint8_t *sp = b.scales + (size_t)f * g.ocr_stride + (size_t)(in_q ? qq : 0) * 4;
	const size_t row_bytes = (size_t)g.W * 4;
	for (int r = r0; r < r1; r += NR) {
		uint4 v[NR];
#pragma unroll
		for (int k = 0; k < NR; ++k) v[k] = *(const uint4 *)(fp + (size_t)min(r + k, r1 - 1) * row_bytes);
#pragma unroll
		for (int k = 0; k < NR; ++k) {
			const int row = r + k;
			if (row >= r1) break;
// ... 38 lines not shown
```

Before: 667,400.

## Add configurable wave priority modes for map pass and LSD service kernels

Adds selectable s_setprio modes for the map pass: raise priority for the whole pass, only around global loads, or around loads and stores. It also lets the persistent LSD service raise priority for owner waves and the record tail, and drops priority while spin-waiting. The aim is to stop the co-resident map pass and service waves from starving each other on shared CUs. By default the map pass keeps its previous whole-pass priority, and the plain pass gets no priority. The service priority bit is now set by default in non-compact mode, which changes scheduling between owner and helper waves and may slow the map pass.

```diff
diff --git a/include/smh_vision_hip_debug.h b/include/smh_vision_hip_debug.h
--- a/include/smh_vision_hip_debug.h
+++ b/include/smh_vision_hip_debug.h
@@ -25,6 +25,9 @@
 SMHV_API int smhv_debug_crc32_host_level(const void *data, uint64_t nbytes, int level, uint32_t *crc);
 SMHV_API int smhv_debug_band_rows(uint32_t frame_w, uint32_t frame_h, uint32_t n, int fused, uint32_t *rows, uint32_t *bands, int *tiles);
 SMHV_API int smhv_debug_map_band_rows(uint32_t rows);
+#define SMHV_DEBUG_PRIORITY_RULE 0xFFFFFFFFu
+SMHV_API int smhv_debug_stream_priority(uint32_t pass_mode, uint32_t service_mode);
+SMHV_API int smhv_debug_stream_priority_get(uint32_t *pass_mode, uint32_t *service_mode);
 SMHV_API int smhv_debug_render_form(uint32_t form);
 SMHV_API int smhv_debug_render_rule(uint32_t map_w, uint32_t map_h, float sw, float sh, uint32_t hm_w, uint32_t hm_h, float *ratio, float *switch_ratio,
                                     uint32_t *lds_texels, uint32_t *form);
diff --git a/squad-mortar-helper_amd/_lib.py b/squad-mortar-helper_amd/_lib.py
--- a/squad-mortar-helper_amd/_lib.py
+++ b/squad-mortar-helper_amd/_lib.py
@@ -364,6 +364,8 @@
     "smhv_ingest_create_ex": (C.c_int, [C.c_void_p, C.c_uint32, C.c_uint32, C.c_uint32, C.c_uint32, C.c_uint32, C.POINTER(C.c_void_p)]),
     "smhv_crc32_host": (C.c_uint32, [C.c_void_p, C.c_uint64]),
     "smhv_debug_map_band_rows": (C.c_int, [C.c_uint32]),
+    "smhv_debug_stream_priority": (C.c_int, [C.c_uint32, C.c_uint32]),
+    "smhv_debug_stream_priority_get": (C.c_int, [C.POINTER(C.c_uint32), C.POINTER(C.c_uint32)]),
     "smhv_debug_band_rows": (C.c_int, [C.c_uint32, C.c_uint32, C.c_uint32, C.c_int, C.POINTER(C.c_uint32), C.POINTER(C.c_uint32), C.POINTER(C.c_int)]),
     "smhv_debug_ingest_feed": (C.c_int, [C.c_void_p, C.c_uint32, C.POINTER(C.c_uint32)]),
     "smhv_debug_ingest_feed_pixels": (C.c_int, [C.c_void_p, C.c_uint32, C.POINTER(C.c_uint32), C.c_uint32]),
@@ -532,6 +534,7 @@
 
 
 SEARCH_AUTO, SEARCH_BATCH, SEARCH_FRAME = 0, 1, 2
+DEBUG_PRIORITY_RULE = 0xFFFFFFFF
 PIPE_NO_TEAM_HELP, PIPE_NO_STREAM_PRIORITY, PIPE_NO_PROLOGUE, PIPE_NO_REMOTE_HELP, PIPE_HELP_FIRST, PIPE_WALK_BIT_ROWS, PIPE_THREE_LOAD_SETS = 1, 2, 4, 8, 16, 32, 64
 
 
diff --git a/squad-mortar-helper_amd/batch.py b/squad-mortar-helper_amd/batch.py
--- a/squad-mortar-helper_amd/batch.py
+++ b/squad-mortar-helper_amd/batch.py
@@ -504,6 +504,8 @@
         keys = ("submissions", "alive_epoch", "launches", "last_seq", "avail", "head", "reserved", "closing_epoch", "completed", "busy")
         d = dict(zip(keys, [int(v) for v in out[:10]]))
         d["avail"] = d["avail"] - (1 << 64) if d["avail"] >= (1 << 63) else d["avail"]
+        d["priority"] = {"pass": (d["launches"] >> 32) & 0xFF, "plain_pass": (d["launches"] >> 40) & 0xFF, "service": (d["launches"] >> 48) & 0xFF}
+        d["launches"] &= 0xFFFFFFFF
         d["slots"] = [(int(v) >> 32, int(v) & 0xFFFFFFFF) for v in out[10:14]]
         d["service_workgroups"], d["waves_per_workgroup"] = int(out[14]) >> 32, int(out[14]) & 0xFFFFFFFF
         d["lds_words_per_wave"], d["lds_bytes_dynamic"] = int(out[15]) >> 32, int(out[15]) & 0xFFFFFFFF
diff --git a/squad-mortar-helper_amd/csrc/smh_kernels.h b/squad-mortar-helper_amd/csrc/smh_kernels.h
--- a/squad-mortar-helper_amd/csrc/smh_kernels.h
+++ b/squad-mortar-helper_amd/csrc/smh_kernels.h
@@ -408,7 +408,8 @@
 hipError_t launch_svc_publish(SvcCtl *ctl, unsigned long long *ring, SvcSlot *slots, uint32_t slot, const Buffers &b, uint32_t n, uint32_t seq, uint32_t ring_log2, hipStream_t s);
 hipError_t launch_lsd_service(const Geom &g, const SvcParams &p, uint32_t workgroups, uint32_t waves, uint32_t lds_bytes, hipStream_t s);
 
-enum : uint32_t { MAP_UI = 1u, MAP_MASK = 2u, MAP_BYTES = 4u, MAP_PRIO = 0x100u, MAP_BAND_MAJOR = 0x200u };
+enum : uint32_t { MAP_UI = 1u, MAP_MASK = 2u, MAP_BYTES = 4u, MAP_PRIO = 0x100u, MAP_BAND_MAJOR = 0x200u, MAP_PRIO_LOADS = 0x400u, MAP_PRIO_MEM = 0x800u };
+inline uint32_t map_prio_flags(uint32_t mode) { return mode == 1u ? (uint32_t)MAP_PRIO : mode == 2u ? (uint32_t)MAP_PRIO_LOADS : mode == 3u ? (uint32_t)(MAP_PRIO_LOADS | MAP_PRIO_MEM) : 0u; }
 enum : uint32_t { BRQ_OCR = 1u, BRQ_SCALES = 2u };
 
 enum : uint32_t { UI_FORM_RGBA = 0u, UI_FORM_LUMA = 1u, UI_FORM_KEEP = 2u };
@@ -422,6 +423,7 @@
 	uint32_t map_prio;
 	uint32_t map_deep;
 	uint32_t map_overlapped;
+	uint32_t map_prio_plain;
 };
 uint32_t map_brq_lds_bytes(const Geom &g);
 uint32_t lsd_tile_lds_bytes(const Geom &g, uint32_t tile_limit);
diff --git a/squad-mortar-helper_amd/csrc/smh_lsd_seq.inc b/squad-mortar-helper_amd/csrc/smh_lsd_seq.inc
--- a/squad-mortar-helper_amd/csrc/smh_lsd_seq.inc
+++ b/squad-mortar-helper_amd/csrc/smh_lsd_seq.inc
@@ -226,8 +226,9 @@
 #define SVC_LEAN_SAMPLER(compact) (!(compact))
 #endif
 
+__device__ __forceinline__ bool owner_prio(const uint32_t *prio_word) { return prio_word != nullptr && (uniform_u32(W_LD(prio_word)) & 2u) != 0u; }
 template <int MODE, bool REUSE = false, bool LEAN = false>
-__device__ __forceinline__ void seq_cast_candidate(const Win &m, uint32_t *wwin, WinTag *tag, const uint32_t *cull_tab, uint32_t cull, const RayDir *dirs, const float *ray_off, float max_gap,
+__device__ __forceinline__ void seq_cast_candidate(const Win &m, uint32_t *wwin, WinTag *tag, const uint32_t *cull_tab, uint32_t cull, const RayDir *dirs, const float *ray_off, float max_gap, const uint32_t *prio_word,
                                                    uint32_t px, uint32_t py, float &xs, float &ys, unsigned long long &wkey, float &ex0, float &ey0, uint32_t &steps_sum
 #ifdef SMH_LSD_WDEBUG
                                                    , unsigned long long *sprof, unsigned long long &slast, unsigned long long *uprof, uint32_t &n_units
@@ -246,6 +247,7 @@
 	uint32_t st = 0;
 	auto unit_dirs_lds = [&](uint32_t u) -> RayDir { return dirs[min(u * 64u + lane, (uint32_t)SMH_LSD_RAYS - 1u)]; };
 	RayDir dn = unit_dirs_lds(live ? (uint32_t)__builtin_ctzll(live) : 0u);
+	if (owner_prio(prio_word)) __builtin_amdgcn_s_setprio(0);
 	for (unsigned long long todo = live; todo; todo &= todo - 1ull) {
 		const uint32_t u = (uint32_t)__builtin_ctzll(todo);
 		const RayDir d = dn;
@@ -261,6 +263,7 @@
 #endif
 		if (key > bkey) { bkey = key; bxe = xe; bye = ye; }
 	}
+	if (owner_prio(prio_word)) __builtin_amdgcn_s_setprio(3);
 	steps_sum = wave_sum32_dpp(st);
 	wkey = 0ull; ex0 = xs; ey0 = ys;
 	if (__any(bkey != 0ull)) {
@@ -306,7 +309,9 @@
 #ifdef SMH_LSD_WDEBUG
 			const unsigned long long t_w = __builtin_amdgcn_s_memtime();
 #endif
+			__builtin_amdgcn_s_setprio(0);
 			while (uniform_u32(sl.state) != (uint32_t)H_DONE) { __builtin_amdgcn_s_sleep(16); remote_harvest(ws); }
+			if (owner_prio(&ws.rem_flags)) __builtin_amdgcn_s_setprio(3);
 #ifdef SMH_LSD_WDEBUG
 			if (lane == 0) ws.prof[0] += __builtin_amdgcn_s_memtime() - t_w;
 #endif
@@ -322,7 +327,9 @@
 		if (lane == 0) { uint32_t expect = H_POSTED; ok = __hip_atomic_compare_exchange_strong(&sl.state, &expect, (uint32_t)H_FREE, __ATOMIC_ACQ_REL, __ATOMIC_RELAXED, __HIP_MEMORY_SCOPE_WORKGROUP) ? 1u : 0u; }
 		if (uniform_u32(ok)) return false;
 	}
+	__builtin_amdgcn_s_setprio(0);
 	while (uniform_u32(W_LD_ACQ(&sl.state)) != (uint32_t)H_DONE) __builtin_amdgcn_s_sleep(2);
+	if (owner_prio(&ws.rem_flags)) __builtin_amdgcn_s_setprio(3);
 	xs = sl.ptx; ys = sl.pty; wkey = sl.best; ex0 = sl.ex; ey0 = sl.ey; steps_sum = sl.steps;
 	__builtin_amdgcn_wave_barrier();
 	if (lane == 0) W_ST_REL(&sl.state, (uint32_t)H_FREE);
@@ -518,6 +525,7 @@
 	int cur_bit = -1;
 	bool done = false, want = false, desk_valid = false;
 	WinTag wtag = {0, 0, false};
+	const uint32_t *prio_word = TEAM ? &ws.rem_flags : nullptr;
 #ifdef SMH_LSD_WDEBUG
 	unsigned long long sprof[8] = {0, 0, 0, 0, 0, 0, 0, 0}, slast = __builtin_amdgcn_s_memtime(), uprof[12] = {0, 0, 0, 0, 0, 0, 0, 0, 0, 0, 0, 0};
 	uint32_t n_units = 0, n_taken = 0;
@@ -534,6 +542,7 @@
 		__builtin_amdgcn_wave_barrier();
 		__builtin_amdgcn_fence(__ATOMIC_ACQUIRE, "workgroup");
 		SPROF(0);
+		if (owner_prio(prio_word)) __builtin_amdgcn_s_setprio(3);
 		while (true) {
 			uint32_t px = 0, py = 0;
 			if (!wave_dispatch(ws, list, survw, wy0, wwords, xorg, px, py)) break;
@@ -555,9 +564,9 @@
 #endif
 #ifdef SMH_LSD_WDEBUG
 			if (have) ++n_taken;
-			if (!have) seq_cast_candidate<MODE, REUSE, LEAN>(m, wwin, &wtag, cull_tab, cull, dirs, b.ray_off, max_gap, px, py, xs, ys, wkey, ex0, ey0, st_sum, sprof, slast, uprof, n_units);
+			if (!have) seq_cast_candidate<MODE, REUSE, LEAN>(m, wwin, &wtag, cull_tab, cull, dirs, b.ray_off, max_gap, prio_word, px, py, xs, ys, wkey, ex0, ey0, st_sum, sprof, slast, uprof, n_units);
 #else
-			if (!have) seq_cast_candidate<MODE, REUSE, LEAN>(m, wwin, &wtag, cull_tab, cull, dirs, b.ray_off, max_gap, px, py, xs, ys, wkey, ex0, ey0, st_sum);
+			if (!have) seq_cast_candidate<MODE, REUSE, LEAN>(m, wwin, &wtag, cull_tab, cull, dirs, b.ray_off, max_gap, prio_word, px, py, xs, ys, wkey, ex0, ey0, st_sum);
 #endif
 			if (lane == 0) ws.steps += st_sum;
 			if (wkey != 0ull && __uint_as_float((uint32_t)(wkey >> 32)) > SMH_LSD_ACCEPT_LEN_SQ) {
@@ -632,6 +641,7 @@
 			}
 			SPROF(4);
 		}
+		if (TEAM) __builtin_amdgcn_s_setprio(0);
 		if (segnext >= WT) break;
 		seg_start = segnext;
 	}
diff --git a/squad-mortar-helper_amd/csrc/smh_map_pass.inc b/squad-mortar-helper_amd/csrc/smh_map_pass.inc
--- a/squad-mortar-helper_amd/csrc/smh_map_pass.inc
+++ b/squad-mortar-helper_amd/csrc/smh_map_pass.inc
@@ -1,3 +1,4 @@
+	if (flags & MAP_PRIO) __builtin_amdgcn_s_setprio(3);
 	const uint32_t f = blockIdx.y;
 	if (!b.aux[f].open) return;
 	const uint32_t q = threadIdx.x, lane = q & 63u, wave = q >> 6, nwave = blockDim.x >> 6;
@@ -20,8 +21,10 @@
 
 	const uint8_t *lp = qact ? fp : fp - (size_t)q * 16;
 	uint4 nx[4];
+	if (flags & MAP_PRIO_LOADS) __builtin_amdgcn_s_setprio(3);
 #pragma unroll
 	for (int k = 0; k < 4; ++k) nx[k] = *(const uint4 *)(lp + (size_t)min(rs + k, re) * row_bytes);
+	if (flags & MAP_PRIO_LOADS) __builtin_amdgcn_s_setprio(0);
 	extern __shared__ __attribute__((aligned(16))) uint32_t s_hits[];
 	for (int r = rs; r <= re; r += 4) {
 		uint4 px[4];
@@ -29,8 +32,10 @@
 #pragma unroll
 		for (int k = 0; k < 4; ++k) px[k] = nx[k];
 		if (r + 4 <= re) {
+			if (flags & MAP_PRIO_LOADS) __builtin_amdgcn_s_setprio(3);
 #pragma unroll
 			for (int k = 0; k < 4; ++k) nx[k] = *(const uint4 *)(lp + (size_t)min(r + 4 + k, re) * row_bytes);
+			if (flags & MAP_PRIO_LOADS) __builtin_amdgcn_s_setprio(0);
 		}
 #pragma unroll
 		for (int k = 0; k < 4; ++k) {
@@ -46,12 +51,14 @@
 					else if (GRAYF) ov[c] = luma8(rr8, gg, bb) * 0x00010101u | 0xFF000000u;
 					else ov[c] = rr8 | (gg << 8) | (bb << 16) | 0xFF000000u;
 				}
+				if (flags & MAP_PRIO_MEM) __builtin_amdgcn_s_setprio(3);
 				if constexpr (GRAYF == 2) *(uint32_t *)(uip + (size_t)row * (g.ui_pitch >> 2)) = ov[0] | (ov[1] << 8) | (ov[2] << 16) | (ov[3] << 24);
 				else {
 					uint4 o;
 					o.x = ov[0]; o.y = ov[1]; o.z = ov[2]; o.w = ov[3];
 					*(uint4 *)(uip + (size_t)row * g.ui_pitch) = o;
 				}
+				if (flags & MAP_PRIO_MEM) __builtin_amdgcn_s_setprio(0);
 			}
 			if (do_mask) {
 				uint32_t pre = 0;
@@ -138,6 +145,7 @@
 		else if (lane < ntr) occp[(size_t)lane * op] = 0;
 		if (blockIdx.x == 0 && q == 0) b.aux[f].tiles = 1u;
 	}
+	if (flags & MAP_PRIO_MEM) __builtin_amdgcn_s_setprio(3);
 	if (q < quads_padded) {
 		uint8_t *mp = b.mask + (size_t)f * g.mask_stride + (size_t)q * 4;
 		uint32_t *bp = b.bits + (size_t)f * g.bits_stride_w + (q >> 3);
@@ -159,6 +167,7 @@
 			}
 		}
 	}
+	if (flags & MAP_PRIO_MEM) __builtin_amdgcn_s_setprio(0);
 	if (lanes_set) {
 		const uint64_t rows_set = wave_or64(any);
 		const uint32_t cnt = wave_sum32(__popcll(D[0]) + __popcll(D[1]) + __popcll(D[2]) + __popcll(D[3]));
diff --git a/squad-mortar-helper_amd/csrc/smh_runtime.cpp b/squad-mortar-helper_amd/csrc/smh_runtime.cpp
--- a/squad-mortar-helper_amd/csrc/smh_runtime.cpp
+++ b/squad-mortar-helper_amd/csrc/smh_runtime.cpp
@@ -1071,7 +1071,7 @@
 	if (b->probe) HIPCHK(hipEventRecord(b->ev_probe[0], s));
 	STAGE_BEGIN(1, s);
 	if (mflags && qflags) HIPCHK(launch_map_brq_pass(g, bf, n, mflags, qflags, pass_gray, 0, 1, s, &b->tune));
-	else if (mflags) HIPCHK(launch_map_pass(g, bf, n, mflags, pass_gray, s, true, b->tune.map_overlapped != 0u));
+	else if (mflags) HIPCHK(launch_map_pass(g, bf, n, mflags | map_prio_flags(b->tune.map_prio_plain), pass_gray, s, true, b->tune.map_overlapped != 0u));
 	if (mflags & MAP_MASK) {
 		std::lock_guard<std::mutex> lk(b->mask_mu);
 		if (b->mask_eager) HIPCHK(launch_mask_expand(g, b->d_bits, b->d_mask, n, s));
@@ -1317,6 +1317,7 @@
 	uint64_t submitted = 0;
 	uint64_t round_start = 0;
 	bool svc = false;
+	uint32_t prio_pass = 0, prio_plain = 0, prio_service = 0;
 	uint32_t svc_compact = 0;
 	uint32_t svc_streams = 0, svc_waves = 0, svc_part_words = 0, svc_tile_cap = 0, svc_list_cap = 0, svc_lds = 0, svc_wgs = 0, svc_ring_log2 = 0;
 	SvcCtl *d_svc_ctl = nullptr;
@@ -1400,6 +1401,15 @@
 #define SMH_ADAPT_OFF 3.5f
 #define SMH_ADAPT_ON 1.6f
 #define SMH_LATE_KC_SEARCH_BOUND 400u
+static std::atomic<uint32_t> g_prio_pass{SMHV_DEBUG_PRIORITY_RULE}, g_prio_service{SMHV_DEBUG_PRIORITY_RULE};
+static void stream_priority_for(bool compact, uint32_t pipe_flags, uint32_t *pass, uint32_t *plain, uint32_t *service) {
+	const uint32_t fp = g_prio_pass.load(std::memory_order_relaxed), fs = g_prio_service.load(std::memory_order_relaxed);
+	*pass = fp != SMHV_DEBUG_PRIORITY_RULE ? fp : 1u;
+	*plain = fp != SMHV_DEBUG_PRIORITY_RULE ? fp : 0u;
+	*service = fs != SMHV_DEBUG_PRIORITY_RULE ? fs : (compact ? 0u : 1u);
+	if (pipe_flags & SMHV_PIPE_NO_STREAM_PRIORITY) *pass = *plain = 0u;
+}
+
 static LaunchTuning pipeline_tuning(const Geom &g) {
 	LaunchTuning t{0u, 0u, 0u, 0u, 0u};
 	const uint32_t lsd = (lsd_tile_lds_bytes(g, SMH_PIPE_TILE_LIMIT(g)) + 1023u) & ~1023u;
@@ -1518,13 +1528,15 @@
 		}
 	}
 	if (e != hipSuccess) { smhv_pipeline_destroy(p); return fail(SMHV_E_HIP, "pipeline streams / events: %s", hipGetErrorString(e)); }
+	if (p->svc) stream_priority_for(p->svc_compact != 0u, opt.flags, &p->prio_pass, &p->prio_plain, &p->prio_service);
 	for (uint32_t i = 0; i < depth; ++i) {
 		int rc = smhv_batch_create(c, W, H, max_frames, &p->batch[i]);
 		if (rc) { smhv_pipeline_destroy(p); return rc; }
 		p->batch[i]->lsd_bs = depth >= 2 ? 512u : 1024u;
 		p->batch[i]->lsd_prefer_classic = depth == 2 && lsd_rows_only(p->batch[i]->g);
 		if (p->svc && !p->adaptive) {
-			p->batch[i]->tune.map_prio = (opt.flags & SMHV_PIPE_NO_STREAM_PRIORITY) ? 0u : 1u;
+			p->batch[i]->tune.map_prio = p->prio_pass;
+			p->batch[i]->tune.map_prio_plain = p->prio_plain;
 			p->batch[i]->tune.map_deep = (opt.flags & SMHV_PIPE_THREE_LOAD_SETS) ? 1u : 0u;
 			p->batch[i]->tune.map_overlapped = 1u;
 		} else if (depth >= 3) {
@@ -1567,6 +1579,7 @@
 	sp.idle_long = 50000u;
 	if (p->opt.flags & SMHV_PIPE_HELP_FIRST) sp.flags |= 16u;
 	if (p->opt.flags & SMHV_PIPE_WALK_BIT_ROWS) sp.flags |= 32u;
+	if (p->prio_service) sp.flags |= 64u;
 
 	sp.remote = p->d_svc_remote; sp.remote_store = p->d_svc_store; sp.remote_store_words = p->svc_store_words;
 	sp.remote_after = p->opt.remote_after ? p->opt.remote_after : 24u;
@@ -1622,7 +1635,7 @@
 	if (rc) return rc;
 	if (batch_check_errors(b, "pipeline_submit (the slot's previous submission, never waited for)") != SMHV_OK) logf(p->ctx, 2, "%s", t_last_error.c_str());
 	hipStream_t st = p->svc_stream[p->submitted % p->svc_streams];
-	if (p->adaptive) { b->tune = LaunchTuning{0u, 0u, 0u, (p->opt.flags & SMHV_PIPE_NO_STREAM_PRIORITY) ? 0u : 1u, (p->opt.flags & SMHV_PIPE_THREE_LOAD_SETS) ? 1u : 0u, 1u}; b->probe = false; b->lsd_late_kc = 0u; }
+	if (p->adaptive) { b->tune = LaunchTuning{0u, 0u, 0u, p->prio_pass, (p->opt.flags & SMHV_PIPE_THREE_LOAD_SETS) ? 1u : 0u, 1u, p->prio_plain}; b->probe = false; b->lsd_late_kc = 0u; }
 	Buffers probe{};
 	const bool want_cull = (stages & SMHV_STAGE_MARKERS) && !(stages & SMHV_STAGE_EXACT_STATS);
 	if (want_cull) { rc = sector_table_for(p->ctx, max_gap, st, &probe); if (rc) return rc; }
@@ -1865,7 +1878,8 @@
 	if (!p->svc) return SMHV_OK;
 	HIPCHK(hipSetDevice(p->ctx->device));
 	const unsigned long long st = __atomic_load_n(&p->h_svc->state, __ATOMIC_ACQUIRE);
-	out[0] = st >> 32; out[1] = (uint32_t)st; out[2] = p->h_svc->launches; out[3] = p->seq_counter;
+	out[0] = st >> 32; out[1] = (uint32_t)st; out[3] = p->seq_counter;
+	out[2] = p->h_svc->launches | ((uint64_t)(p->prio_pass | (p->prio_plain << 8) | (p->prio_service << 16)) << 32);
 	out[14] = ((uint64_t)p->svc_wgs << 32) | p->svc_waves; out[15] = ((uint64_t)p->svc_part_words << 32) | p->svc_lds;
 	std::lock_guard<std::mutex> lk(p->peek_mu);
 	if (!p->s_peek) HIPCHK(hipStreamCreateWithFlags(&p->s_peek, hipStreamNonBlocking));
@@ -2805,6 +2819,20 @@
 	return SMHV_OK;
 }
 
+extern "C" SMHV_API int smhv_debug_stream_priority(uint32_t pass_mode, uint32_t service_mode) {
+	if (pass_mode != SMHV_DEBUG_PRIORITY_RULE && pass_mode > 3u) return fail(SMHV_E_INVALID, "debug_stream_priority: pass mode 0..3 (or SMHV_DEBUG_PRIORITY_RULE), not %u", pass_mode);
+	if (service_mode != SMHV_DEBUG_PRIORITY_RULE && service_mode > 1u) return fail(SMHV_E_INVALID, "debug_stream_priority: service mode 0 or 1 (or SMHV_DEBUG_PRIORITY_RULE), not %u", service_mode);
+	g_prio_pass.store(pass_mode, std::memory_order_relaxed);
+	g_prio_service.store(service_mode, std::memory_order_relaxed);
+	return SMHV_OK;
+}
+
+extern "C" SMHV_API int smhv_debug_stream_priority_get(uint32_t *pass_mode, uint32_t *service_mode) {
+	if (pass_mode) *pass_mode = g_prio_pass.load(std::memory_order_relaxed);
+	if (service_mode) *service_mode = g_prio_service.load(std::memory_order_relaxed);
+	return SMHV_OK;
+}
+
 extern "C" SMHV_API int smhv_debug_band_rows(uint32_t frame_w, uint32_t frame_h, uint32_t n, int fused, uint32_t *rows, uint32_t *bands, int *tiles) {
 	Geom g;
 	int rc = compute_geom(frame_w, frame_h, &g);
diff --git a/squad-mortar-helper_amd/csrc/smh_service.inc b/squad-mortar-helper_amd/csrc/smh_service.inc
--- a/squad-mortar-helper_amd/csrc/smh_service.inc
+++ b/squad-mortar-helper_amd/csrc/smh_service.inc
@@ -69,7 +69,11 @@
 		} else svc_frame_global<COMPACT>(kargs, slot, f, part_off, cull_off, dirs_off);
 	}
 	const unsigned long long t_search_end = __builtin_amdgcn_s_memtime();
-	if (b.rec_stages & SMH_REC_ON) frame_record_tail_wave(&((const SvcKernelArgs *)kargs)->g, &((const SvcSlot *)(ka->p.slots + slot))->b, f);
+	if (b.rec_stages & SMH_REC_ON) {
+		if (ka->p.flags & 64u) __builtin_amdgcn_s_setprio(3);
+		frame_record_tail_wave(&((const SvcKernelArgs *)kargs)->g, &((const SvcSlot *)(ka->p.slots + slot))->b, f);
+		if (ka->p.flags & 64u) __builtin_amdgcn_s_setprio(0);
+	}
 	return t_search_end;
 }
 
@@ -124,9 +128,9 @@
 #ifdef SMH_LSD_WDEBUG
 		unsigned long long sprof[8] = {0, 0, 0, 0, 0, 0, 0, 0}, slast = __builtin_amdgcn_s_memtime(), uprof[12] = {0, 0, 0, 0, 0, 0, 0, 0, 0, 0, 0, 0};
 		uint32_t n_units = 0;
-		seq_cast_candidate<COMPACT ? LSD_MODE_TILEC : LSD_MODE_TILE, SVC_WIN_REUSE(COMPACT), SVC_LEAN_SAMPLER(COMPACT)>(m, wwin, &wtag, cull_tab, cull, dirs, ray_off, max_gap, px, py, xs, ys, wkey, ex0, ey0, st_sum, sprof, slast, uprof, n_units);
+		seq_cast_candidate<COMPACT ? LSD_MODE_TILEC : LSD_MODE_TILE, SVC_WIN_REUSE(COMPACT), SVC_LEAN_SAMPLER(COMPACT)>(m, wwin, &wtag, cull_tab, cull, dirs, ray_off, max_gap, nullptr, px, py, xs, ys, wkey, ex0, ey0, st_sum, sprof, slast, uprof, n_units);
 #else
-		seq_cast_candidate<COMPACT ? LSD_MODE_TILEC : LSD_MODE_TILE, SVC_WIN_REUSE(COMPACT), SVC_LEAN_SAMPLER(COMPACT)>(m, wwin, &wtag, cull_tab, cull, dirs, ray_off, max_gap, px, py, xs, ys, wkey, ex0, ey0, st_sum);
+		seq_cast_candidate<COMPACT ? LSD_MODE_TILEC : LSD_MODE_TILE, SVC_WIN_REUSE(COMPACT), SVC_LEAN_SAMPLER(COMPACT)>(m, wwin, &wtag, cull_tab, cull, dirs, ray_off, max_gap, nullptr, px, py, xs, ys, wkey, ex0, ey0, st_sum);
 #endif
 		if (lane == 0) {
 			sl.ptx = xs; sl.pty = ys; sl.best = wkey; sl.ex = ex0; sl.ey = ey0; sl.steps = st_sum;
@@ -211,9 +215,9 @@
 #ifdef SMH_LSD_WDEBUG
 		unsigned long long sprof[8] = {0, 0, 0, 0, 0, 0, 0, 0}, slast = __builtin_amdgcn_s_memtime(), uprof[12] = {0, 0, 0, 0, 0, 0, 0, 0, 0, 0, 0, 0};
 		uint32_t n_units = 0;
-		seq_cast_candidate<COMPACT ? LSD_MODE_TILEC : LSD_MODE_TILE, SVC_WIN_REUSE(COMPACT), SVC_LEAN_SAMPLER(COMPACT)>(m, wwin, &wtag, cull_tab, cull, dirs, ray_off, max_gap, px, py, xs, ys, wkey, ex0, ey0, st_sum, sprof, slast, uprof, n_units);
+		seq_cast_candidate<COMPACT ? LSD_MODE_TILEC : LSD_MODE_TILE, SVC_WIN_REUSE(COMPACT), SVC_LEAN_SAMPLER(COMPACT)>(m, wwin, &wtag, cull_tab, cull, dirs, ray_off, max_gap, nullptr, px, py, xs, ys, wkey, ex0, ey0, st_sum, sprof, slast, uprof, n_units);
 #else
-		seq_cast_candidate<COMPACT ? LSD_MODE_TILEC : LSD_MODE_TILE, SVC_WIN_REUSE(COMPACT), SVC_LEAN_SAMPLER(COMPACT)>(m, wwin, &wtag, cull_tab, cull, dirs, ray_off, max_gap, px, py, xs, ys, wkey, ex0, ey0, st_sum);
+		seq_cast_candidate<COMPACT ? LSD_MODE_TILEC : LSD_MODE_TILE, SVC_WIN_REUSE(COMPACT), SVC_LEAN_SAMPLER(COMPACT)>(m, wwin, &wtag, cull_tab, cull, dirs, ray_off, max_gap, nullptr, px, py, xs, ys, wkey, ex0, ey0, st_sum);
 #endif
 		++n_cast;
 		t_cast += __builtin_amdgcn_s_memtime() - t_c0;
@@ -346,7 +350,7 @@
 		w0.rem_ctl = (unsigned long long)(uintptr_t)p.ctl;
 		w0.rem_after = p.remote_after; w0.rem_tickets = p.remote_tickets; w0.rem_owner = owner; w0.rem_cap = p.tile_cap;
 		w0.rem_open = 0u; w0.rem_gen = 0u; w0.rem_k = 0u; w0.rem_nr = 0u;
-		w0.rem_last_div = p.remote_last_div; w0.rem_flags = (p.flags & 16u) ? 1u : 0u;
+		w0.rem_last_div = p.remote_last_div; w0.rem_flags = ((p.flags & 16u) ? 1u : 0u) | ((p.flags & 64u) ? 2u : 0u);
 	}
 	__syncthreads();
 	uint32_t *part = smem + wave * p.part_words;
diff --git a/squad-mortar-helper_amd/csrc/smh_stream.hip b/squad-mortar-helper_amd/csrc/smh_stream.hip
--- a/squad-mortar-helper_amd/csrc/smh_stream.hip
+++ b/squad-mortar-helper_amd/csrc/smh_stream.hip
@@ -371,6 +371,7 @@
 #pragma unroll
 					for (int c = 0; c < 4; ++c) lum[c] = luma_bgra(pv[c]);
 				}
+				if (flags & MAP_PRIO_MEM) __builtin_amdgcn_s_setprio(3);
 				if constexpr (GRAY == 2) {
 					if (do_ui && qact) SMH_ST32(loff >> 2, lum[0] | (lum[1] << 8) | (lum[2] << 16) | (lum[3] << 24), uibase + (size_t)row * (g.ui_pitch >> 2));
 				} else if (do_ui && qact) {
@@ -393,6 +394,7 @@
 						SMH_ST32(qoff, ones_to_bytes(nz), sp + (size_t)qrow * g.ocr_pitch);
 					}
 				}
+				if (flags & MAP_PRIO_MEM) __builtin_amdgcn_s_setprio(0);
 			}
 			if (rare(do_mask && __any(bright4(pv) != 0u))) {
 				uint32_t pre = 0;
@@ -451,12 +453,14 @@
 	{
 		const uint8_t *dummy = (const uint8_t *)&b.aux[f];
 		auto load4 = [&](u32x4 (&dst)[GR], int r) {
+			if (flags & MAP_PRIO_LOADS) __builtin_amdgcn_s_setprio(3);
 #pragma unroll
 			for (int k = 0; k < GR; ++k) {
 				const bool inside = r + k <= re;
 				const uint8_t *rowp = inside ? fbase + (size_t)(r + k) * row_bytes : dummy;
 				SMH_LD128(dst[k], inside ? loff : 0u, rowp);
 			}
+			if (flags & MAP_PRIO_LOADS) __builtin_amdgcn_s_setprio(0);
 		};
 		if constexpr (SETS == 2) {
 			u32x4 S0[GR], S1[GR];
@@ -536,6 +540,7 @@
 			else if (lane < ntr) occp[(size_t)lane * opitch] = 0;
 			if (band == 0u && q == 0u) b.aux[f].tiles = 1u;
 		}
+		if (flags & MAP_PRIO_MEM) __builtin_amdgcn_s_setprio(3);
 		if (q < quads_padded && !lanes_set) {
 			uint32_t *bbase = b.bits + (size_t)f * g.bits_stride_w;
 			const uint32_t boff = (q >> 3) * 4u;
@@ -568,6 +573,7 @@
 				}
 			}
 		}
+		if (flags & MAP_PRIO_MEM) __builtin_amdgcn_s_setprio(0);
 		if (lanes_set) {
 			const uint64_t rows_set = wave_or64(any);
 			const uint32_t cnt = wave_sum32(__popcll(D[0]) + __popcll(D[1]) + __popcll(D[2]) + __popcll(D[3]));
@@ -717,7 +723,7 @@
 			if (dev < 64) attr_devices.fetch_or(1ull << dev, std::memory_order_release);
 		}
 	}
-	if (tune && tune->map_prio) flags |= MAP_PRIO;
+	if (tune) flags |= map_prio_flags(tune->map_prio);
 	flags |= work_item_order(tune && tune->map_overlapped);
 	const uint32_t cap = tune ? tune->map_grid_cap : 0u;
 	const bool deep = tune && tune->map_deep && !(cap && cap < items);
```

Result: no change. 673,800 (median of 6 runs) (+1.0%).
